# mbhall88/drprg

Hardware: AMD Instinct MI355X
Metric: reads/sec (+ achieved HBM GB/s) predicting on mtb index, 1/2/4/8 GPUs (higher is better)
Workload: dtype u32

## Files before the change

drprg_amd/csrc/candidates.hip:

```cpp
#include "filter_common.h"
#include "verify_lane.h"
#include <algorithm>
#include <cstdint>

namespace drprg {
namespace dev {

constexpr int VS_THREADS = 512;
constexpr int VS_PER = MAX_SLICES / VS_THREADS;
template <int KC, bool PACKED>
__global__ __launch_bounds__(VS_THREADS, 8) void verify_scan_kernel(SketchArgs a, FilterWork fw, ReadClusterArgs rc)
{
    __shared__ uint32_t s_red[3][VS_THREADS / 64];
    __shared__ uint32_t s_w[VS_THREADS / 64 + 1];
    __shared__ uint32_t s_share[2];
    __shared__ __attribute__((aligned(16))) uint32_t s_pre[MAX_SLICES + 4];
    const int tid = threadIdx.x;
    static_assert(VS_PER % 4 == 0 && MAX_SLICES % (VS_THREADS * 4) == 0, "the counts are read 16 bytes at a time");
    auto my_count = [&](int i4) -> uint4 {
        return reinterpret_cast<const uint4*>(fw.super_count + (size_t)tid * VS_PER)[i4];
    };
    uint32_t run = 0;
    uint4 v[VS_PER / 4];
#pragma unroll
    for (int i = 0; i < VS_PER / 4; ++i) v[i] = my_count(i);
#pragma unroll
    for (int i = 0; i < VS_PER / 4; ++i) run += v[i].x + v[i].y + v[i].z + v[i].w;
    uint32_t total;
    const uint32_t before = block_exclusive_scan<VS_THREADS / 64>(run, s_w, &total);
    if (blockIdx.x == 0 && tid == 0) *fw.cand_count = total;
    const uint32_t per_wg = (total + gridDim.x - 1) / gridDim.x;
    const uint64_t b64 = (uint64_t)blockIdx.x * per_wg;
    const uint32_t t_begin = b64 < total ? (uint32_t)b64 : total, t_end = b64 + per_wg < total ? (uint32_t)(b64 + per_wg) : total;
    {
        const uint32_t x0 = t_begin, x1 = t_end - 1u;
        const bool own0 = t_begin < t_end && before <= x0 && x0 < before + run, own1 = t_begin < t_end && before <= x1 && x1 < before + run;
        uint32_t acc = before, n0 = 0, n1 = 0;
        uint4* dst = reinterpret_cast<uint4*>(s_pre + (size_t)tid * VS_PER);
#pragma unroll
        for (int i = 0; i < VS_PER / 4; ++i) {
            uint4 p;
            p.x = acc;
            p.y = p.x + v[i].x;
            p.z = p.y + v[i].y;
            p.w = p.z + v[i].z;
            acc = p.w + v[i].w;
            dst[i] = p;
            n0 += (p.y <= x0 ? 1u : 0u) + (p.z <= x0 ? 1u : 0u) + (p.w <= x0 ? 1u : 0u) + (acc <= x0 ? 1u : 0u);
            n1 += (p.y <= x1 ? 1u : 0u) + (p.z <= x1 ? 1u : 0u) + (p.w <= x1 ? 1u : 0u) + (acc <= x1 ? 1u : 0u);
        }
        if (tid == VS_THREADS - 1) s_pre[MAX_SLICES] = acc;
        if (own0) s_share[0] = (uint32_t)tid * VS_PER + n0;
        if (own1) s_share[1] = (uint32_t)tid * VS_PER + n1;
    }
    __syncthreads();
    const VerifyConsts c(a, fw);
    uint32_t my_hits = 0, my_nmin = 0, my_maxlen = 0;
    auto position_in = [&](uint32_t t, uint32_t lo0, uint32_t hi0, uint32_t step0) -> int64_t {
        uint32_t lo = lo0;
        for (uint32_t step = step0; step >= 1; step >>= 1)
            if (lo + step <= hi0 && s_pre[lo + step] <= t) lo += step;
        static_assert(FT_SUPER == 8, "two uint4 of slice counts per superblock");
        const uint4* __restrict__ c4 = reinterpret_cast<const uint4*>(fw.slice_count) + (size_t)lo * 2;
        const uint4* __restrict__ b4 = reinterpret_cast<const uint4*>(fw.slice_base) + (size_t)lo * 2;
        const uint4 ca = c4[0], cb = c4[1], ba = b4[0], bb = b4[1];
        const uint32_t cnt[7] = { ca.x, ca.y, ca.z, ca.w, cb.x, cb.y, cb.z }, start[8] = { ba.x, ba.y, ba.z, ba.w, bb.x, bb.y, bb.z, bb.w };
        uint32_t rest = t - s_pre[lo], sum = 0, before = 0, at = start[0];
#pragma unroll
        for (int q = 0; q < 7; ++q) {
            sum += cnt[q];
            const bool past = rest >= sum;
            at = past ? start[q + 1] : at;
            before = past ? sum : before;
        }
        return (int64_t)fw.raw_pos[(size_t)at + (rest - before)];
    };
    {
        const uint32_t s_lo = (uint32_t)__builtin_amdgcn_readfirstlane((int)s_share[0]), s_hi = (uint32_t)__builtin_amdgcn_readfirstlane((int)s_share[1]);
        const uint32_t span_step = s_hi > s_lo ? 1u << (31 - __builtin_clz(s_hi - s_lo)) : 1u;
        auto position_of = [&](uint32_t t) -> int64_t { return position_in(t, s_lo, s_hi, span_step); };
        int64_t gp_next = t_begin + tid < t_end ? position_of(t_begin + (uint32_t)tid) : 0;
        for (uint32_t t = t_begin + (uint32_t)tid; t < t_end; t += VS_THREADS) {
            const int64_t gp = gp_next;
            if (t + VS_THREADS < t_end) gp_next = position_of(t + VS_THREADS);
            VerifyOut o;
            verify_one_lane<KC, PACKED>(a, rc, c, gp, o, my_hits, my_nmin, my_maxlen);
            fw.cand_pos1[t] = o.pos1;
            fw.cand_info[t] = ((uint64_t)o.slot << 32) | ((uint64_t)o.strand << 31) | (uint64_t)o.read;
            fw.cand_rec[t] = o.crec;
        }
    }
    const uint32_t wh = wave_inclusive_scan(my_hits), wn = wave_inclusive_scan(my_nmin), wm = wave_max(my_maxlen);
    if ((tid & 63) == 63) {
        s_red[0][tid >> 6] = wh;
        s_red[1][tid >> 6] = wn;
        s_red[2][tid >> 6] = wm;
    }
    __syncthreads();
    if (tid == 0) {
        uint32_t h = 0, n = 0, mx = 0;
        for (int i = 0; i < VS_THREADS / 64; ++i) {
            h += s_red[0][i];
            n += s_red[1][i];
            mx = s_red[2][i] > mx ? s_red[2][i] : mx;
        }
        fw.wg_hits[blockIdx.x] = h;
        fw.wg_nmin[blockIdx.x] = n;
        fw.wg_maxlen[blockIdx.x] = mx;
    }
}



__global__ __launch_bounds__(SCAN_THREADS) void hit_scan_kernel(SketchArgs a, FilterWork fw, int recount, uint32_t n_wg)
{
    __shared__ uint32_t s_w[SCAN_THREADS / 64 + 1];
    __shared__ uint32_t s_n[SCAN_THREADS / 64], s_m[SCAN_THREADS / 64];
    constexpr int PER = MAX_EX_WG / SCAN_THREADS;
    const int tid = threadIdx.x;
    uint32_t v[PER], h[PER], nm[PER], ml[PER], run = 0, nmin = 0, mx = 0;
#pragma unroll
    for (int i = 0; i < PER; ++i) {
        const uint32_t g = (uint32_t)tid * PER + i, gc = g < n_wg ? g : 0u;
        h[i] = fw.wg_hits[gc];
        nm[i] = fw.wg_nmin[gc];
        ml[i] = fw.wg_maxlen[gc];
    }
#pragma unroll
    for (int i = 0; i < PER; ++i) {
        const uint32_t g = (uint32_t)tid * PER + i;
        v[i] = run;
        if (g < n_wg) {
            run += h[i];
            nmin += nm[i];
            mx = ml[i] > mx ? ml[i] : mx;
        }
    }
    uint32_t total;
    const uint32_t before = block_exclusive_scan<SCAN_THREADS / 64>(run, s_w, &total);
#pragma unroll
    for (int i = 0; i < PER; ++i) {
        const uint32_t g = (uint32_t)tid * PER + i;
        if (g < n_wg) fw.wg_base[g] = before + v[i];
    }
    const uint32_t wn = wave_inclusive_scan(nmin), wm = wave_max(mx);
    if ((tid & 63) == 63) {
        s_n[tid >> 6] = wn;
        s_m[tid >> 6] = wm;
    }
    __syncthreads();
    if (tid == 0) {
        uint32_t n = 0, m = 0;
        for (int i = 0; i < SCAN_THREADS / 64; ++i) {
            n += s_n[i];
            m = s_m[i] > m ? s_m[i] : m;
        }
        *a.n_hits = (unsigned long long)total;
        if (n && !recount && !(*reinterpret_cast<volatile uint32_t*>(a.overflow) & 4u)) atomicAdd(a.n_minimizers, (unsigned long long)n);
        *fw.max_len = (unsigned long long)m;
    }
}

__global__ __launch_bounds__(EX_THREADS) void expand_kernel(SketchArgs a, FilterWork fw)
{
    __shared__ uint32_t s_w[EX_THREADS / 64 + 1];
    const int tid = threadIdx.x;
    uint32_t t_begin, t_end;
    candidate_range(fw, blockIdx.x, gridDim.x, t_begin, t_end);
    uint64_t base = fw.wg_base[blockIdx.x];
    for (uint32_t t0 = t_begin; t0 < t_end; t0 += EX_THREADS) {
        const uint32_t t = t0 + tid;
        const uint32_t pos1 = t < t_end ? fw.cand_pos1[t] : 0u;
        uint64_t info = 0;
        uint2 rec = make_uint2(0, 0);
        if (pos1) {
            info = fw.cand_info[t];
            rec = a.slot_rec[(uint32_t)(info >> 32)];
        }
        uint32_t total;
        const uint32_t off = block_exclusive_scan<EX_THREADS / 64>(rec.y, s_w, &total);
        const uint64_t at = base + off;
        if (pos1 && at + rec.y <= a.hit_capacity) {
            const uint32_t read = (uint32_t)info & 0x7FFFFFFFu, strand = ((uint32_t)info >> 31) & 1u;
            for (uint32_t q = 0; q < rec.y; ++q) {
                const uint32_t kn = a.rec_knode[rec.x + q];
                const uint32_t prg = a.rec_prg[rec.x + q];
                const uint32_t rev = ((kn & 1u) == strand) ? 0u : 1u;
                a.hit_key[at + q] = pack_hit_key(read, prg, rev, pos1 - 1);
                a.hit_val[at + q] = kn >> 1;
            }
        }
        base += total;
    }
}

__global__ void read_inversion_kernel(const uint64_t* __restrict__ key, uint32_t n, uint2* __restrict__ list, uint32_t cap,
    unsigned long long* __restrict__ count)
{
    const uint32_t i = blockIdx.x * blockDim.x + threadIdx.x;
    if (i + 1 >= n) return;
    const uint64_t a = key[i], b = key[i + 1];
    const uint32_t read = hit_read(a);
    if (hit_read(b) != read || a <= b) return;
    uint32_t s = i;
    while (s > 0 && hit_read(key[s - 1]) == read) {
        if (key[s - 1] > key[s]) return;
        --s;
    }
    uint32_t e = i + 2;
    while (e < n && hit_read(key[e]) == read) ++e;
    const unsigned long long at = atomicAdd(count, 1ull);
    if (at < cap) list[at] = make_uint2(s, e - s);
}

constexpr int RS_THREADS = 256, RS_MAX = 1024;
__global__ __launch_bounds__(RS_THREADS) void read_fix_kernel(uint64_t* __restrict__ key, uint32_t* __restrict__ val,
    uint64_t* __restrict__ key_tmp, uint32_t* __restrict__ val_tmp, const uint2* __restrict__ list, const unsigned long long* __restrict__ count)
{
    __shared__ uint64_t s_key[RS_MAX];
    __shared__ uint32_t s_val[RS_MAX];
    const uint32_t n_list = (uint32_t)*count;
    for (uint32_t r = blockIdx.x; r < n_list; r += gridDim.x) {
        const uint32_t start = list[r].x, len = list[r].y;
        if (len > RS_MAX) {
            for (uint32_t t0 = 0; t0 < len; t0 += RS_THREADS) {
                const uint32_t t = t0 + threadIdx.x;
                const bool mine = t < len;
                const uint64_t kt = mine ? key[start + t] : 0;
                uint32_t before = 0;
                for (uint32_t j0 = 0; j0 < len; j0 += RS_MAX) {
                    const uint32_t nj = len - j0 < (uint32_t)RS_MAX ? len - j0 : (uint32_t)RS_MAX;
                    __syncthreads();
                    for (uint32_t j = threadIdx.x; j < nj; j += RS_THREADS) s_key[j] = key[start + j0 + j];
                    __syncthreads();
                    if (!mine) continue;
                    if (j0 + nj <= t) {
                        for (uint32_t j = 0; j < nj; ++j) before += s_key[j] <= kt ? 1u : 0u;
                    } else if (j0 > t) {
                        for (uint32_t j = 0; j < nj; ++j) before += s_key[j] < kt ? 1u : 0u;
                    } else {
                        const uint32_t tj = t - j0;
                        for (uint32_t j = 0; j < tj; ++j) before += s_key[j] <= kt ? 1u : 0u;
                        for (uint32_t j = tj + 1; j < nj; ++j) before += s_key[j] < kt ? 1u : 0u;
                    }
                }
                if (mine) {
                    key_tmp[start + before] = kt;
                    val_tmp[start + before] = val[start + t];
                }
            }
            __syncthreads();
            for (uint32_t t = threadIdx.x; t < len; t += RS_THREADS) {
                key[start + t] = key_tmp[start + t];
                val[start + t] = val_tmp[start + t];
            }
            __syncthreads();
            continue;
        }
        for (uint32_t t = threadIdx.x; t < len; t += RS_THREADS) {
            s_key[t] = key[start + t];
            s_val[t] = val[start + t];
        }
        __syncthreads();
        for (uint32_t t = threadIdx.x; t < len; t += RS_THREADS) {
            const uint64_t kt = s_key[t];
            uint32_t before = 0;
            for (uint32_t j = 0; j < t; ++j) before += s_key[j] <= kt ? 1u : 0u;
            for (uint32_t j = t + 1; j < len; ++j) before += s_key[j] < kt ? 1u : 0u;
            key[start + before] = kt;
            val[start + before] = s_val[t];
        }
        __syncthreads();
    }
}

__global__ __launch_bounds__(EX_THREADS) void recount_kernel(SketchArgs a, FilterWork fw)
{
    __shared__ uint32_t s_red[2][EX_THREADS / 64];
    const int tid = threadIdx.x;
    uint32_t t_begin, t_end;
    candidate_range(fw, blockIdx.x, gridDim.x, t_begin, t_end);
    uint32_t my_hits = 0, my_maxlen = 0;
    for (uint32_t t = t_begin + tid; t < t_end; t += EX_THREADS) {
        if (!fw.cand_pos1[t]) continue;
        const uint64_t info = fw.cand_info[t];
        my_hits += a.slot_rec[(uint32_t)(info >> 32)].y;
        const uint32_t read = (uint32_t)info & 0x7FFFFFFFu;
        const uint64_t len64 = a.offsets[read + 1] - a.offsets[read];
        const uint32_t len = len64 > 0xFFFFFFFFull ? 0xFFFFFFFFu : (uint32_t)len64;
        my_maxlen = len > my_maxlen ? len : my_maxlen;
    }
    const uint32_t wh = wave_inclusive_scan(my_hits), wm = wave_max(my_maxlen);
    if ((tid & 63) == 63) {
        s_red[0][tid >> 6] = wh;
        s_red[1][tid >> 6] = wm;
    }
    __syncthreads();
    if (tid == 0) {
        uint32_t h = 0, mx = 0;
        for (int i = 0; i < EX_THREADS / 64; ++i) {
            h += s_red[0][i];
            mx = s_red[1][i] > mx ? s_red[1][i] : mx;
        }
        fw.wg_hits[blockIdx.x] = h;
        fw.wg_nmin[blockIdx.x] = 0;
        fw.wg_maxlen[blockIdx.x] = mx;
    }
}

constexpr int TG_THREADS = 1024, TG_TILES = 64;
__device__ __forceinline__ bool tile_overflow(const SketchArgs& a, const uint32_t* tile_prefix, uint32_t n_tiles, uint64_t dense_capacity)
{
    return (*reinterpret_cast<volatile uint32_t*>(a.overflow) & 4u) != 0 || (uint64_t)tile_prefix[n_tiles] > dense_capacity;
}

__global__ __launch_bounds__(TG_THREADS) void tile_totals_kernel(SketchArgs a, const uint32_t* __restrict__ tile_prefix, uint32_t n_tiles,
    uint64_t dense_capacity, uint32_t* __restrict__ block_first)
{
    __shared__ uint32_t s_w[TG_THREADS / 64 + 1];
    const int tid = threadIdx.x;
    if (tile_overflow(a, tile_prefix, n_tiles, dense_capacity)) {
        if (blockIdx.x == 0 && tid == 0) atomicOr(a.overflow, 4u);
        return;
    }
    uint32_t my_hits = 0, my_nmin = 0;
    for (uint32_t t = blockIdx.x * TG_THREADS + (uint32_t)tid; t < n_tiles; t += gridDim.x * TG_THREADS) {
        my_hits += a.tile_hits[t];
        my_nmin += a.tile_nmin[t];
        if (block_first) {
            const uint32_t lo = tile_prefix[t], hi = tile_prefix[t + 1];
            for (uint32_t m = (lo + 63u) >> 6; lo < hi && (uint64_t)m << 6 < hi; ++m) block_first[m] = t;
        }
    }
    uint32_t hits, nmin;
    (void)block_exclusive_scan<TG_THREADS / 64>(my_hits, s_w, &hits);
    (void)block_exclusive_scan<TG_THREADS / 64>(my_nmin, s_w, &nmin);
    if (tid == 0) {
        if (hits) atomicAdd(a.n_hits, (unsigned long long)hits);
        if (nmin) atomicAdd(a.n_minimizers, (unsigned long long)nmin);
    }
}

__global__ __launch_bounds__(TG_THREADS) void tile_gather_kernel(SketchArgs a, FilterWork fw, const uint32_t* __restrict__ tile_prefix,
    uint32_t n_tiles, uint64_t dense_capacity, uint32_t mark)
{
    const int tid = threadIdx.x, lane = tid & 63, wave = tid >> 6;
    if (tile_overflow(a, tile_prefix, n_tiles, dense_capacity)) return;
    const uint32_t t0 = blockIdx.x * TG_TILES, t1 = t0 + TG_TILES < n_tiles ? t0 + TG_TILES : n_tiles;
    for (uint32_t t = t0 + (uint32_t)wave; t < t1; t += TG_THREADS / 64) {
        const uint32_t n = a.tile_count[t], dst = tile_prefix[t];
        const size_t src = (size_t)t * a.tile_cap;
        for (uint32_t i0 = 0; i0 < n; i0 += 256) {
            uint64_t ci[4];
            uint32_t cp[4];
            uint4 cr[4];
#pragma unroll
            for (int u = 0; u < 4; ++u) {
                const uint32_t i = i0 + 64u * (uint32_t)u + (uint32_t)lane;
                const size_t at = src + (i < n ? i : 0u);
                ci[u] = a.tile_info[at];
                cp[u] = a.tile_pos1[at];
                cr[u] = a.tile_rec[at];
            }
#pragma unroll
            for (int u = 0; u < 4; ++u) {
                const uint32_t i = i0 + 64u * (uint32_t)u + (uint32_t)lane;
                if (i < n) {
                    fw.cand_info[dst + i] = ci[u];
                    fw.cand_pos1[dst + i] = fw.cand_pos1[dst + i] == mark ? 0u : cp[u];
                    fw.cand_rec[dst + i] = cr[u];
                }
            }
        }
    }
}

hipError_t launch_candidate_stage(const SketchArgs& a, FilterWork& fw, const ReadClusterArgs& rc, int n_cus, hipStream_t stream, bool with_totals)
{
    fw.verify_grid = std::min<uint32_t>((uint32_t)n_cus * (uint32_t)(2048 / VS_THREADS), MAX_EX_WG);
    const dim3 grid(fw.verify_grid);
    if (a.packed) {
        if (a.k == 15) hipLaunchKernelGGL((verify_scan_kernel<15, true>), grid, dim3(VS_THREADS), 0, stream, a, fw, rc);
        else hipLaunchKernelGGL((verify_scan_kernel<0, true>), grid, dim3(VS_THREADS), 0, stream, a, fw, rc);
    } else if (a.k == 15) hipLaunchKernelGGL((verify_scan_kernel<15, false>), grid, dim3(VS_THREADS), 0, stream, a, fw, rc);
    else hipLaunchKernelGGL((verify_scan_kernel<0, false>), grid, dim3(VS_THREADS), 0, stream, a, fw, rc);
    if (with_totals) hipLaunchKernelGGL(hit_scan_kernel, dim3(1), dim3(SCAN_THREADS), 0, stream, a, fw, 0, fw.verify_grid);
    return hipGetLastError();
}

bool direct_uses_wave_form(int k, int w, bool wide_hash, bool force_lds) { return !wide_hash && !force_lds && wave_kernel_applies(k, w); }

uint32_t direct_candidate_tiles(uint64_t n_bases, int halo, int k, int w, bool wide_hash, bool force_lds)
{
    return direct_uses_wave_form(k, w, wide_hash, force_lds) ? wave_n_slices(n_bases) : sketch_n_tiles(n_bases, halo);
}

uint32_t direct_first_read_tiles(uint64_t n_bases, int halo, int k, int w, bool wide_hash, bool force_lds)
{
    return direct_uses_wave_form(k, w, wide_hash, force_lds) ? wave_n_tiles(n_bases) : sketch_n_tiles(n_bases, halo);
}

hipError_t launch_direct_candidates(const SketchArgs& a, bool wide_hash, bool force_lds, uint32_t* tile_prefix, void* temp, size_t temp_bytes,
    uint64_t dense_capacity, const ReadClusterArgs& rc, int n_cus, FilterWork& fw, hipStream_t stream, KernelTimer timer, uint32_t slices_mark)
{
    if (a.n_bases == 0 || !a.tile_cap || !slices_mark) return hipErrorInvalidValue;
    const uint32_t n_tiles = direct_candidate_tiles(a.n_bases, a.halo, a.k, a.w, wide_hash, force_lds);
    if (direct_uses_wave_form(a.k, a.w, wide_hash, force_lds)) HIP_TRY(launch_sketch_wave(a, stream, timer));
    else HIP_TRY(launch_sketch_probe(a, wide_hash, stream, timer));
    HIP_TRY(exclusive_scan_u32(temp, temp_bytes, a.tile_count, tile_prefix, n_tiles + 1, stream));
    fw.cand_total = tile_prefix + n_tiles;
    uint32_t* const block_first = dense_capacity ? reinterpret_cast<uint32_t*>(fw.cand_info) : nullptr;
    hipLaunchKernelGGL(tile_totals_kernel, dim3(std::min<uint32_t>((n_tiles + TG_THREADS - 1) / TG_THREADS, (uint32_t)n_cus)), dim3(TG_THREADS), 0, stream, a,
        tile_prefix, n_tiles, dense_capacity, block_first);
    HIP_TRY(hipGetLastError());
    ReadClusterArgs rcs = rc;
    rcs.block_first = block_first;
    rcs.slice_prefix = tile_prefix;
    rcs.n_slices = n_tiles;
    rcs.mark_epoch = slices_mark;
    return launch_read_cluster(a, fw, rcs, n_cus, false, stream);
}

hipError_t launch_tile_gather_marked(const SketchArgs& a, const FilterWork& fw, const uint32_t* tile_prefix, uint32_t n_tiles, uint64_t dense_capacity,
    uint32_t mark, hipStream_t stream)
{
    hipLaunchKernelGGL(tile_gather_kernel, dim3((n_tiles + TG_TILES - 1) / TG_TILES), dim3(TG_THREADS), 0, stream, a, fw, tile_prefix, n_tiles,
        dense_capacity, mark);
    return hipGetLastError();
}

hipError_t launch_filter_recount(const SketchArgs& a, const FilterWork& fw, hipStream_t stream)
{
    hipLaunchKernelGGL(recount_kernel, dim3(fw.ex_grid), dim3(EX_THREADS), 0, stream, a, fw);
    HIP_TRY(hipGetLastError());
    hipLaunchKernelGGL(hit_scan_kernel, dim3(1), dim3(SCAN_THREADS), 0, stream, a, fw, 1, fw.ex_grid);
    return hipGetLastError();
}

hipError_t launch_filter_expand(const SketchArgs& a, const FilterWork& fw, hipStream_t stream)
{
    hipLaunchKernelGGL(expand_kernel, dim3(fw.ex_grid), dim3(EX_THREADS), 0, stream, a, fw);
    return hipGetLastError();
}

hipError_t launch_read_sort(uint64_t* key, uint32_t* val, uint64_t* key_tmp, uint32_t* val_tmp, uint32_t n, uint32_t* scratch, uint64_t scratch_words,
    unsigned long long* count, hipStream_t stream)
{
    if (n < 2) return hipSuccess;
    uint2* list = reinterpret_cast<uint2*>(scratch);
    hipLaunchKernelGGL(read_inversion_kernel, dim3((n + 255) / 256), dim3(256), 0, stream, key, n, list, (uint32_t)(scratch_words / 2), count);
    HIP_TRY(hipGetLastError());
    hipLaunchKernelGGL(read_fix_kernel, dim3(1024), dim3(RS_THREADS), 0, stream, key, val, key_tmp, val_tmp, list, count);
    return hipGetLastError();
}

}
}
```

drprg_amd/csrc/capi.cpp:

```cpp
#include <set>
#include <atomic>
#include <mutex>
#include <thread>
#include <fstream>
#include <cstdio>
#include "../../include/drprg_hip.h"
#include "fastx.h"
#include "genotype.h"
#include "bam.h"
#include "ingest.h"
#include "pgunzip.h"
#include "denovo.h"
#include "mapper.h"
#include "rccl_dyn.h"
#include "pack.h"
#include <algorithm>
#include <cstdlib>
#include <cstring>
#include <fcntl.h>
#include <functional>
#include <sys/mman.h>
#include <sys/stat.h>
#include <unistd.h>
#include <memory>
// ... 1169 lines not shown
    const std::vector<uint32_t> p = find_max_path(kg, std::vector<float>(logp, logp + kg.nodes.size()), thresh, max_kmers_to_average);
    *n_path = p.size();
    for (size_t i = 0; i < p.size() && i < cap; ++i) path[i] = p[i];
    return DRPRG_OK;
}

int drprg_hip_path_base_coverage(const drprg_hip_ctx* ctx, uint32_t prg, const uint32_t* path, uint64_t n_path, const uint32_t* covg2, uint32_t* out,
    uint64_t cap, uint64_t* n_out)
{
    if (!ctx || (n_path && !path) || !covg2 || !n_out || prg >= ctx->index.kgs.size()) return DRPRG_EINVAL;
    const KmerGraph& kg = ctx->index.kgs[prg];
    for (uint64_t i = 0; i < n_path; ++i)
        if (path[i] >= kg.nodes.size()) return DRPRG_EINVAL;
    const std::vector<uint32_t> b = base_coverage_along_path(ctx->index.prgs[prg], kg, std::vector<uint32_t>(path, path + n_path), covg2);
    *n_out = b.size();
    for (size_t i = 0; i < b.size() && i < cap; ++i) out[i] = b[i];
    return DRPRG_OK;
}

int drprg_hip_path_coverage_too_low(const uint32_t* base_covg, uint64_t n, uint32_t global_covg)
{
    if (n && !base_covg) return DRPRG_EINVAL;
    return path_coverage_too_low(std::vector<uint32_t>(base_covg, base_covg + n), global_covg) ? 1 : 0;
}

int drprg_hip_coverage_model(const drprg_hip_ctx* ctx, double out[12])
{
    if (!ctx || !out) return DRPRG_EINVAL;
    const CoverageModel& m = ctx->last_model;
    out[0] = m.exp_depth_covg; out[1] = m.bin ? 1 : 0; out[2] = m.e_rate; out[3] = m.nb_p; out[4] = m.nb_r; out[5] = m.branch;
    out[6] = m.mean; out[7] = m.var; out[8] = m.num_reads; out[9] = m.bin_p; out[10] = m.thresh; out[11] = (double)ctx->last_dropped;
    return DRPRG_OK;
}

int drprg_hip_allele_stats(const uint32_t* fwd, const uint32_t* rev, uint32_t n, uint32_t min_kmer_covg, uint32_t out[6], double* gaps)
{
    if ((n && (!fwd || !rev)) || !out || !gaps) return DRPRG_EINVAL;
    const AlleleStats s = allele_stats(std::vector<uint32_t>(fwd, fwd + n), std::vector<uint32_t>(rev, rev + n), min_kmer_covg);
    out[0] = s.mean_fwd; out[1] = s.mean_rev; out[2] = s.med_fwd; out[3] = s.med_rev; out[4] = s.sum_fwd; out[5] = s.sum_rev;
    *gaps = s.gaps;
    return DRPRG_OK;
}

int drprg_hip_genotype_site(const uint32_t* mean_fwd, const uint32_t* mean_rev, const double* gaps, uint32_t n_alleles, double e,
    double eps, double* likelihood, int32_t* gt, double* gt_conf)
{
    if (!n_alleles || !mean_fwd || !mean_rev || !gaps || !likelihood || !gt || !gt_conf) return DRPRG_EINVAL;
    std::vector<AlleleStats> al(n_alleles);
    for (uint32_t a = 0; a < n_alleles; ++a) {
        al[a].mean_fwd = mean_fwd[a];
        al[a].mean_rev = mean_rev[a];
        al[a].gaps = gaps[a];
    }
    int g = 0;
    genotype_site(al, e, eps, g, *gt_conf);
    *gt = g;
    for (uint32_t a = 0; a < n_alleles; ++a) likelihood[a] = al[a].likelihood;
    return DRPRG_OK;
}

int drprg_hip_genotype_info(const drprg_hip_ctx* ctx, uint32_t out[4])
{
    if (!ctx || !out) return DRPRG_EINVAL;
    std::memcpy(out, ctx->ginfo, sizeof ctx->ginfo);
    return DRPRG_OK;
}

int drprg_hip_filter_selfcheck(const drprg_hip_ctx* ctx, uint64_t out[8])
{
    if (!ctx || !out) return DRPRG_EINVAL;
    ctx->index.filter_selfcheck(out);
    return DRPRG_OK;
}

int drprg_hip_index_sizes(const drprg_hip_ctx* ctx, uint64_t sizes[5])
{
    if (!ctx || !sizes) return DRPRG_EINVAL;
    const FlatIndex& f = ctx->index.flat;
    sizes[0] = f.keys.size();
    sizes[1] = f.rec_prg.size();
    sizes[2] = ctx->index.prgs.size();
    sizes[3] = f.total_knodes();
    sizes[4] = f.slot_key.size();
    return DRPRG_OK;
}

int drprg_hip_index_export(const drprg_hip_ctx* ctx, uint64_t* keys, uint32_t* rec_off, uint32_t* rec_prg, uint32_t* rec_knode,
    uint8_t* rec_strand, uint32_t* prg_min_path_len, uint32_t* prg_knode_base)
{
    if (!ctx) return DRPRG_EINVAL;
    const FlatIndex& f = ctx->index.flat;
    if (keys) std::memcpy(keys, f.keys.data(), f.keys.size() * sizeof(uint64_t));
    if (rec_off) std::memcpy(rec_off, f.rec_off.data(), f.rec_off.size() * sizeof(uint32_t));
    if (rec_prg) std::memcpy(rec_prg, f.rec_prg.data(), f.rec_prg.size() * sizeof(uint32_t));
    if (rec_knode) std::memcpy(rec_knode, f.rec_knode_global.data(), f.rec_knode_global.size() * sizeof(uint32_t));
    if (rec_strand) std::memcpy(rec_strand, f.rec_strand.data(), f.rec_strand.size());
    if (prg_min_path_len) std::memcpy(prg_min_path_len, f.min_path_len.data(), f.min_path_len.size() * sizeof(uint32_t));
    if (prg_knode_base) std::memcpy(prg_knode_base, f.knode_base.data(), f.knode_base.size() * sizeof(uint32_t));
    return DRPRG_OK;
}

int drprg_hip_prg_nodes(const drprg_hip_ctx* ctx, uint32_t prg, uint32_t* starts, uint32_t* ends, uint32_t cap, uint32_t* n_nodes,
    uint32_t* n_sites)
{
    if (!ctx || prg >= ctx->index.prgs.size()) return DRPRG_EINVAL;
    const LocalGraph& g = ctx->index.prgs[prg];
    for (uint32_t i = 0; i < g.nodes.size() && i < cap; ++i) {
        if (starts) starts[i] = g.nodes[i].start;
        if (ends) ends[i] = g.nodes[i].end;
    }
    if (n_nodes) *n_nodes = (uint32_t)g.nodes.size();
    if (n_sites) *n_sites = (uint32_t)g.sites.size();
    return DRPRG_OK;
}

int drprg_hip_device_tables(drprg_hip_ctx* ctx, uint64_t out[6])
{
    API_BEGIN(ctx)
    need_mapper(ctx).device_tables(out);
    API_END(ctx)
}

int drprg_hip_kernel_timing(drprg_hip_ctx* ctx, int enable, int reset, double* ms_total, uint64_t* launches)
{
    API_BEGIN(ctx)
    Mapper& m = need_mapper(ctx);
    m.sync();
    m.enable_kernel_timing(enable != 0);
    if (ms_total) *ms_total = m.sketch_ms_total();
    if (launches) *launches = m.sketch_launches();
    if (reset) m.reset_kernel_timing();
    API_END(ctx)
}

int drprg_hip_filter_schedule(drprg_hip_ctx* ctx, uint64_t out[20])
{
    API_BEGIN(ctx)
    if (!out) throw Error(DRPRG_EINVAL, "null pointer");
    need_mapper(ctx).filter_schedule(out);
    API_END(ctx)
}

int drprg_hip_buffer_info(drprg_hip_ctx* ctx, uint64_t out[6])
{
    API_BEGIN(ctx)
    if (!out) throw Error(DRPRG_EINVAL, "null pointer");
    need_mapper(ctx);
    std::memset(out, 0, 6 * sizeof(uint64_t));
    for (Mapper* m : mappers_of(ctx)) {
        uint64_t v[6];
        m->buffer_info(v);
        for (int i = 0; i < 3; ++i) out[i] += v[i];
        for (int i = 3; i < 5; ++i) out[i] = std::max(out[i], v[i]);
    }
    API_END(ctx)
}

}

#include "report.h"

static int report_guard(char* err, size_t err_len, const std::function<void()>& fn)
{
    auto put = [&](const char* m) {
        if (err && err_len) {
            std::strncpy(err, m, err_len - 1);
            err[err_len - 1] = 0;
        }
    };
    try {
        fn();
    } catch (const Error& e) {
        put(e.what());
        return e.code;
    } catch (const std::exception& e) {
        put(e.what());
        return DRPRG_EIO;
    }
    return DRPRG_OK;
}

extern "C" {

int drprg_hip_annotate(const char* index_dir, const char* pandora_vcf, const char* out_vcf, const drprg_hip_annotate_opts* o,
    char* err, size_t err_len)
{
    if (!index_dir || !pandora_vcf || !out_vcf || !o) return DRPRG_EINVAL;
    return report_guard(err, err_len, [&]() {
        report::AnnotateOpts a;
        a.filter.min_covg = o->min_covg;
        a.filter.max_covg = o->max_covg;
        a.filter.min_strand_bias = o->min_strand_bias;
        a.filter.min_gt_conf = o->min_gt_conf;
        a.filter.min_frs = o->min_frs;
        a.filter.has_max_indel = o->max_indel >= 0;
        a.filter.max_indel = o->max_indel;
        a.minor.maf = o->maf;
        a.minor.max_gaps = o->max_gaps;
        a.minor.max_called_gaps = o->max_called_gaps;
        a.minor.max_gaps_diff = o->max_gaps_diff;
        a.minor.minor_min_covg = o->minor_min_covg;
        a.minor.minor_min_strand_bias = o->minor_min_strand_bias;
        a.ignore_synonymous = o->ignore_synonymous != 0;
        a.id_seed = o->id_seed;
        report::annotate_vcf(report::IndexFiles { index_dir }, pandora_vcf, out_vcf, a);
    });
}

int drprg_hip_report_json(const char* index_dir, const char* annotated_vcf, const char* out_json, const char* sample, int padding,
    const char* index_version, char* err, size_t err_len)
{
    if (!index_dir || !annotated_vcf || !out_json) return DRPRG_EINVAL;
    return report_guard(err, err_len, [&]() {
        report::IndexFiles idx { index_dir };
        std::string version = index_version ? index_version : "";
        if (padding < 0 || !index_version) {
            report::IndexConfig c = report::read_config(idx.config());
            if (padding < 0) padding = c.padding;
            if (!index_version) version = c.version;
        }
        report::vcf_to_json(idx, annotated_vcf, out_json, sample ? sample : "sample", padding, version);
    });
}

}

extern "C" int drprg_hip_vcf_to_bcf(const char* vcf_path, const char* bcf_path, char* err, size_t err_len)
{
    if (!vcf_path || !bcf_path) return DRPRG_EINVAL;
    return report_guard(err, err_len, [&]() { report::vcf_to_bcf(vcf_path, bcf_path); });
}

extern "C" int drprg_hip_gunzip_file(const char* gz_path, int threads, uint64_t chunk_bytes, const char* out_path, uint64_t out[3], char* err, size_t err_len)
{
    if (!gz_path || !out_path || !out) return DRPRG_EINVAL;
    return report_guard(err, err_len, [&]() {
        const int fd = open(gz_path, O_RDONLY);
        if (fd < 0) throw Error(DRPRG_ENOENT, std::string("cannot open ") + gz_path);
        struct stat sb;
        void* map = fstat(fd, &sb) == 0 && sb.st_size > 0 ? mmap(nullptr, (size_t)sb.st_size, PROT_READ, MAP_PRIVATE, fd, 0) : MAP_FAILED;
        close(fd);
        if (map == MAP_FAILED) throw Error(DRPRG_EIO, std::string("cannot map ") + gz_path);
        struct Unmap {
            void* p;
            size_t n;
            ~Unmap() { munmap(p, n); }
        } unmap { map, (size_t)sb.st_size };
        FILE* o = std::fopen(out_path, "wb");
        if (!o) throw Error(DRPRG_EIO, std::string("cannot write ") + out_path);
        struct Close {
            FILE* f;
            ~Close() { std::fclose(f); }
        } close_o { o };
        ParallelGunzip pg((const unsigned char*)map, (size_t)sb.st_size, threads, (size_t)chunk_bytes);
        std::vector<char> buf(size_t(8) << 20);
        uint64_t total = 0;
        for (size_t n; (n = pg.read(buf.data(), buf.size())) > 0; total += n)
            if (std::fwrite(buf.data(), 1, n, o) != n) throw Error(DRPRG_EIO, std::string("cannot write ") + out_path);
        out[0] = total;
        out[1] = pg.chunks_accepted();
        out[2] = pg.chunks_redone();
    });
}

extern "C" int drprg_hip_parse_fastx_ordered(const char* reads_path, int threads, uint64_t max_reads, uint64_t out[6], char* err, size_t err_len)
{
    if (!reads_path || !out) return DRPRG_EINVAL;
    return report_guard(err, err_len, [&]() {
        uint64_t sum = 0, n_reads = 0, n_bases = 0, batches = 0;
        IngestHooks hooks;
        hooks.submit_in_order = [&](const PinnedBatch& b) -> bool {
            const uint64_t n = std::min<uint64_t>(b.n_reads, max_reads - n_reads);
            for (uint64_t i = 0; i < n; ++i) {
                uint64_t h = 1469598103934665603ull;
                for (uint64_t j = b.offsets[i]; j < b.offsets[i + 1]; ++j) h = (h ^ b.bases[j]) * 1099511628211ull;
                sum += (n_reads + i + 1) * h;
            }
            n_reads += n;
            n_bases += b.offsets[n];
            ++batches;
            return n_reads < max_reads;
        };
        const IngestStats st = ingest_fastx(reads_path, threads, hooks);
        out[0] = n_reads; out[1] = n_bases; out[2] = sum; out[3] = batches; out[4] = (uint64_t)st.gz_mode; out[5] = st.discarded_reads;
    });
}

extern "C" int drprg_hip_parse_fastx(const char* reads_path, int threads, uint64_t out[5], char* err, size_t err_len)
{
    if (!reads_path || !out) return DRPRG_EINVAL;
    return report_guard(err, err_len, [&]() {
        uint64_t sum = 0, n_reads = 0, n_bases = 0, batches = 0;
        const bool no_digest = std::getenv("DRPRG_PARSE_NO_DIGEST") != nullptr;
        auto digest = [&](const uint8_t* bases, const uint64_t* offsets, uint64_t n) {
            for (uint64_t i = 0; i < n && !no_digest; ++i) {
                uint64_t h = 1469598103934665603ull;
                for (uint64_t j = offsets[i]; j < offsets[i + 1]; ++j) h = (h ^ bases[j]) * 1099511628211ull;
                sum += h;
            }
            n_reads += n;
            n_bases += offsets[n];
            ++batches;
        };
        const char* fmt = std::getenv("DRPRG_PARSE_FORMAT");
        const bool packed = fmt && std::string(fmt) == "packed", normalized = fmt && std::string(fmt) == "normalized";
        std::vector<uint8_t> tmp;
// ... 37 lines not shown
```

drprg_amd/csrc/device_common.h:

```cpp
#pragma once
#include "kernels.h"
#include <hip/hip_runtime.h>
#include <hip/hip_ext.h>

namespace drprg {
namespace dev {

#define HIP_TRY(x)                                                                                   \
    do {                                                                                             \
        hipError_t e_ = (x);                                                                         \
        if (e_ != hipSuccess) return e_;                                                             \
    } while (0)

constexpr int MAX_HIP_DEVICES = 64;
inline hipError_t ensure_dynamic_lds(const void* kernel, size_t bytes, size_t (&cache)[MAX_HIP_DEVICES])
{
    int dev = 0;
    hipError_t e = hipGetDevice(&dev);
    if (e != hipSuccess) return e;
    if (dev >= 0 && dev < MAX_HIP_DEVICES && bytes <= cache[dev]) return hipSuccess;
    e = hipFuncSetAttribute(kernel, hipFuncAttributeMaxDynamicSharedMemorySize, (int)bytes);
    if (e == hipSuccess && dev >= 0 && dev < MAX_HIP_DEVICES) cache[dev] = bytes;
    return e;
}
// ... 57 lines not shown
    static constexpr uint64_t EMPTY = ~0ULL;
    __device__ static inline uint64_t mix(uint64_t key, uint64_t mask)
    {
        key = (~key + (key << 21)) & mask;
        key = key ^ (key >> 24);
        key = (key + (key << 3) + (key << 8)) & mask;
        key = key ^ (key >> 14);
        key = (key + (key << 2) + (key << 4)) & mask;
        key = key ^ (key >> 28);
        key = (key + (key << 31)) & mask;
        return key;
    }
};

__device__ inline uint32_t table_slot_dev(uint32_t key, uint32_t bits) { return (key * 0x9E3779B1u) >> (32 - bits); }
__device__ inline uint32_t table_slot_dev(uint64_t key, uint32_t bits)
{
    return (uint32_t)((key * 0x9E3779B97F4A7C15ULL) >> (64 - bits));
}

__device__ __forceinline__ bool table_find4(const uint32_t* __restrict__ slot_key, uint32_t tmask, uint32_t h, uint32_t& sl)
{
    constexpr uint32_t EMPTY = HashTraits<uint32_t>::EMPTY;
    uint32_t base = sl & ~3u, from = 0xFu << (sl & 3u);
    while (true) {
        const uint4 q = *reinterpret_cast<const uint4*>(slot_key + base);
        const uint32_t hit = (q.x == h ? 1u : 0u) | (q.y == h ? 2u : 0u) | (q.z == h ? 4u : 0u) | (q.w == h ? 8u : 0u);
        const uint32_t end = hit | (q.x == EMPTY ? 1u : 0u) | (q.y == EMPTY ? 2u : 0u) | (q.z == EMPTY ? 4u : 0u) | (q.w == EMPTY ? 8u : 0u);
        const uint32_t m = end & from;
        if (m) {
            const uint32_t i = (uint32_t)__builtin_ctz(m);
            sl = base + i;
            return (hit >> i) & 1u;
        }
        base = (base + 4u) & tmask;
        from = 0xFu;
    }
}

__device__ inline uint32_t encode_base(uint32_t c)
{
    uint32_t u = c & 0xDFu;
    uint32_t x = (u >> 1) & 3u;
    x ^= x >> 1;
    bool ok = (u == 'A') | (u == 'C') | (u == 'G') | (u == 'T');
    return ok ? x : 4u;
}
__device__ inline uint32_t encode4(uint32_t word)
{
    const uint32_t u = word & 0xDFDFDFDFu;
    const uint32_t sel = (u >> 1) & 0x03030303u;
    const uint32_t code = __builtin_amdgcn_perm(0u, 0x02030100u, sel);
    const uint32_t expect = __builtin_amdgcn_perm(0u, 0x47544341u, sel);
    const uint32_t diff = u ^ expect;
    const uint32_t bad = (((diff & 0x7F7F7F7Fu) + 0x7F7F7F7Fu) | diff) & 0x80808080u;
    return code | (bad >> 5);
}

__device__ inline uint32_t find_read_from(const uint64_t* __restrict__ offsets, uint32_t n_reads, uint32_t lo, uint64_t gp)
{
    uint32_t step = 1, hi = lo + 1;
    while (hi < n_reads && offsets[hi] <= gp) {
        lo = hi;
        step <<= 1;
        hi = (n_reads - lo > step) ? lo + step : n_reads;
    }
    while (hi - lo > 1) {
        uint32_t mid = lo + ((hi - lo) >> 1);
        if (offsets[mid] <= gp) lo = mid; else hi = mid;
    }
    return lo;
}

__device__ inline uint32_t find_read_guess(const uint64_t* __restrict__ offsets, uint32_t n_reads, uint32_t guess, uint32_t lo, uint64_t gp)
{
    if (guess >= n_reads) guess = n_reads - 1;
    if (offsets[guess] <= gp && gp < offsets[guess + 1]) return guess;
    return find_read_from(offsets, n_reads, lo, gp);
}

__device__ inline uint32_t find_read_near(const uint64_t* __restrict__ offsets, uint32_t n_reads, uint32_t guess, uint64_t gp)
{
    uint32_t lo = guess < n_reads ? guess : n_reads - 1, hi;
    if (offsets[lo] <= gp) {
        uint32_t step = 1;
        hi = lo + 1;
        while (hi < n_reads && offsets[hi] <= gp) {
            lo = hi;
            step <<= 1;
            hi = (n_reads - lo > step) ? lo + step : n_reads;
        }
    } else {
        uint32_t step = 1;
        hi = lo;
        while (true) {
            lo = hi > step ? hi - step : 0;
            if (offsets[lo] <= gp) break;
            hi = lo;
            step <<= 1;
        }
    }
    while (hi - lo > 1) {
        uint32_t mid = lo + ((hi - lo) >> 1);
        if (offsets[mid] <= gp) lo = mid; else hi = mid;
    }
    return lo;
}

__device__ inline uint32_t w1_reciprocal(int w) { return (uint32_t)(0x100000000ull / (uint32_t)(w + 1)) + 1u; }
__device__ inline uint64_t expected_minimizers(uint64_t len, int w, uint32_t magic)
{
    if (w < 200 && len < (1ull << 23)) return (uint64_t)__umulhi((uint32_t)len * 2u, magic);
    return len * 2 / (uint64_t)(w + 1);
}

__device__ inline uint32_t wave_inclusive_scan(uint32_t v)
{
    const int lane = threadIdx.x & 63;
#pragma unroll
    for (int off = 1; off < 64; off <<= 1) {
        const uint32_t n = __shfl_up(v, off);
        if (lane >= off) v += n;
    }
    return v;
}
__device__ inline uint32_t wave_max(uint32_t v)
{
#pragma unroll
    for (int off = 32; off > 0; off >>= 1) {
        const uint32_t n = __shfl_xor(v, off);
        v = n > v ? n : v;
    }
    return v;
}

template <int NW> __device__ inline uint32_t block_exclusive_scan(uint32_t v, uint32_t* s_w, uint32_t* total)
{
    const int lane = threadIdx.x & 63, wave = threadIdx.x >> 6;
    const uint32_t incl = wave_inclusive_scan(v);
    __syncthreads();
    if (lane == 63) s_w[wave] = incl;
    __syncthreads();
    uint32_t base = 0, sum = 0;
#pragma unroll
    for (int i = 0; i < NW; ++i) {
        const uint32_t x = s_w[i];
        if (i < wave) base += x;
        sum += x;
    }
    *total = sum;
    return base + incl - v;
}

}
}
```

drprg_amd/csrc/filter_common.h:

```cpp
#pragma once
#include "common.h"
#include "device_common.h"

namespace drprg {
namespace dev {

constexpr int FT_THREADS = 1024;
constexpr int FT_WAVES = FT_THREADS / 64;
constexpr int FT_G = 32;
constexpr int FT_WPOS = 63 * FT_G;
DRPRG_HD constexpr int filter_positions_per_lane(bool level0, bool packed) { return level0 && packed ? 64 : 32; }
constexpr int FT_BLOOM_WORDS = 1 << 14;
constexpr int FT_L0_WORDS = 1 << 15;
constexpr int EX_THREADS = 256;
constexpr int SCAN_THREADS = 1024;
constexpr int MAX_SLICES = SCAN_THREADS * 8;
constexpr int FT_DEPTH = 3;
constexpr int FT_SUPER = 8;
constexpr int MAX_CHUNKS = MAX_SLICES * FT_SUPER;
constexpr int MAX_EX_WG = SCAN_THREADS * 4;

__device__ inline void candidate_range(const FilterWork& fw, uint32_t wg, uint32_t n_wg, uint32_t& t_begin, uint32_t& t_end)
{
    const uint32_t total = *fw.cand_total;
    const uint32_t per_wg = (total + n_wg - 1) / n_wg;
    const uint64_t b = (uint64_t)wg * per_wg;
    t_begin = b < total ? (uint32_t)b : total;
    t_end = b + per_wg < total ? (uint32_t)(b + per_wg) : total;
}

hipError_t launch_candidate_stage(const SketchArgs& a, FilterWork& fw, const ReadClusterArgs& rc, int n_cus, hipStream_t stream, bool with_totals = true);
hipError_t launch_read_cluster(const SketchArgs& a, const FilterWork& fw, const ReadClusterArgs& rc, int n_cus, bool skip, hipStream_t stream);

}
}
```

drprg_amd/csrc/kernels.h:

```cpp
#pragma once
#include <cstddef>
#include <cstdint>
#include <hip/hip_runtime_api.h>
#include "switches.h"

#if defined(__HIPCC__)
#define DRPRG_HD __host__ __device__
#else
#define DRPRG_HD
#endif

namespace drprg {
namespace dev {

constexpr int HIT_POS_BITS = 23;
constexpr int HIT_PRG_BITS = 12;
constexpr int HIT_READ_BITS = 28;
constexpr uint64_t HIT_POS_MASK = (1ull << HIT_POS_BITS) - 1;
constexpr uint32_t MAX_BATCH_READS = 1u << HIT_READ_BITS;
constexpr uint32_t MAX_PRGS = 1u << HIT_PRG_BITS;

DRPRG_HD inline uint64_t pack_hit_key(uint32_t read, uint32_t prg, uint32_t rev, uint32_t pos)
{
    return ((uint64_t)read << (HIT_PRG_BITS + 1 + HIT_POS_BITS)) | ((uint64_t)prg << (1 + HIT_POS_BITS))
        | ((uint64_t)rev << HIT_POS_BITS) | (uint64_t)pos;
}
DRPRG_HD inline uint32_t hit_read(uint64_t k) { return (uint32_t)(k >> (HIT_PRG_BITS + 1 + HIT_POS_BITS)); }
DRPRG_HD inline uint32_t hit_prg(uint64_t k) { return (uint32_t)(k >> (1 + HIT_POS_BITS)) & (MAX_PRGS - 1); }
DRPRG_HD inline uint32_t hit_rev(uint64_t k) { return (uint32_t)(k >> HIT_POS_BITS) & 1u; }

DRPRG_HD inline uint32_t pbloom_mix(uint64_t key) { return ((uint32_t)key ^ (uint32_t)(key >> 32)) * 0x9E3779B1u; }
DRPRG_HD inline uint32_t pbloom_word(uint32_t m, uint32_t wbits) { return m >> (32 - wbits); }
DRPRG_HD inline uint32_t pbloom_bits(uint32_t m) { return (1u << (m & 31)) | (1u << ((m >> 5) & 31)); }

struct SketchArgs {
    const uint8_t* bases;
    const uint64_t* offsets;
    uint64_t n_bases;
    uint32_t n_reads;
    int w, k, halo;
    int packed;
    const uint64_t* npos;
    uint64_t n_npos;
    const uint16_t* nbits;
    const void* slot_key;
    const uint2* slot_rec;
    const uint4* slot_first;
    uint32_t table_bits;
    const uint32_t* rec_knode;
    const uint16_t* rec_prg;
    uint32_t* tile_first_read;
    uint64_t* hit_key;
    uint32_t* hit_val;
    uint64_t hit_capacity;
    unsigned long long* n_hits;
    unsigned long long* n_minimizers;
    const uint32_t* pbloom;
    uint32_t pbloom_wbits;
    uint32_t* overflow;
    uint32_t tile_cap;
    uint64_t* tile_info;
    uint32_t* tile_pos1;
    uint4* tile_rec;
    uint32_t *tile_count, *tile_hits, *tile_nmin;
    const uint32_t* prg_min_path_len;
    const uint32_t* prg_thr;
    double fraction;
    uint32_t min_cluster_size;
};

struct ClusterRec {
    uint32_t read, prg_rev, first_pos, last_pos, n, state;
};

struct ClusterArgs {
    const uint64_t* key;
    const uint32_t* val;
    const uint32_t* scan;
    const uint32_t* cstart;
    const uint32_t* d_n_clusters;
    const uint64_t* offsets;
    const uint32_t* prg_min_path_len;
    ClusterRec* clusters;
    uint32_t* order;
    int w;
    double fraction;
    uint32_t min_cluster_size;
    uint32_t* covg;
    uint32_t* prg_reads;
    unsigned long long* n_clusters_kept;
    unsigned long long* n_hits_kept;
};

struct KernelTimer {
    hipEvent_t begin = nullptr, end = nullptr;
};

uint32_t sketch_tile_eval(int halo);
uint32_t sketch_n_tiles(uint64_t n_bases, int halo);
hipError_t launch_sketch_probe(const SketchArgs& a, bool wide_hash, hipStream_t stream, KernelTimer timer = {});
bool probe_compile_time_window(int k, int w);
hipError_t launch_tile_first_read(const uint64_t* offsets, uint32_t n_reads, int t_eval, int halo, uint32_t n_tiles, uint32_t* out,
    hipStream_t stream);
bool wave_kernel_applies(int k, int w);
uint32_t wave_tile_eval();
uint32_t wave_n_tiles(uint64_t n_bases);
uint32_t wave_n_slices(uint64_t n_bases);
hipError_t launch_sketch_wave(const SketchArgs& a, hipStream_t stream, KernelTimer timer = {});
uint32_t direct_candidate_tiles(uint64_t n_bases, int halo, int k, int w, bool wide_hash, bool force_lds);
bool direct_uses_wave_form(int k, int w, bool wide_hash, bool force_lds);
uint32_t direct_first_read_tiles(uint64_t n_bases, int halo, int k, int w, bool wide_hash, bool force_lds);
uint32_t filter_n_tiles(uint64_t n_bases, int positions_per_lane = 32);
uint32_t filter_grid(bool level0, int n_cus, uint32_t n_tiles, uint32_t cap);
struct BloomTables {
    const uint32_t* bloom;
    uint32_t bloom_wbits;
    const uint32_t* bloom0;
    uint32_t bloom0_wbits;
    const uint32_t* bloomr;
    const uint32_t* bloom0f;
    const uint32_t* mid0 = nullptr;
    const uint32_t* mid_bitmap = nullptr;
    const uint32_t* midc = nullptr;
    uint32_t midc_wbits = 0, mid0_bits = 0;
    const uint32_t* blkc = nullptr;
    uint32_t blkc_wbits = 0;
};
struct FilterBuffers {
    uint64_t* raw_pos;
    uint64_t* cand_info;
    uint32_t* cand_pos1;
    uint4* cand_rec;
    uint64_t raw_capacity;
    uint32_t* small;
    unsigned long long* max_len;
    const uint32_t* wave_share = nullptr;
    unsigned long long* class_clock = nullptr;
};
constexpr int FT_MAX_ROUNDS = 8;
struct FilterSched {
    uint32_t tpw0;
    uint32_t per_wg;
    uint32_t n_tiles;
    uint32_t first_ticket[FT_MAX_ROUNDS], first_tile[FT_MAX_ROUNDS], size[FT_MAX_ROUNDS];
    uint32_t n_rounds;
    uint32_t lds_word;
};
FilterSched make_filter_sched(uint32_t n_tiles, uint32_t n_wg, const uint32_t share[4], const FilterSchedKnobs& knobs);
const uint32_t* filter_builtin_shares(bool mid, bool packed);
struct FilterWork {
    const uint32_t* bloom;
    uint32_t bloom_wbits;
    const uint32_t* bloom0;
    uint32_t bloom0_wbits;
    const uint32_t* mid_bitmap;
    const uint32_t* midc;
    uint32_t midc_wbits;
    uint32_t read_begin, read_end;
    uint32_t n_slices;
    uint32_t slice_budget, slice_cpt, slice_slack;
    uint32_t slice_extra, slice_extra_from;
    uint64_t* raw_pos;
    uint32_t* slice_count;
    uint32_t* slice_base;
    uint32_t* slice_cap;
    uint32_t* super_count;
    FilterSched sched;
    uint32_t* cand_count;
    const uint32_t* cand_total;
    uint64_t* cand_info;
    uint32_t* cand_pos1;
    uint4* cand_rec;
    uint32_t ex_grid;
    uint32_t verify_grid;
    uint32_t *wg_hits, *wg_nmin, *wg_maxlen, *wg_base;
    unsigned long long* max_len;
    unsigned long long* class_clock;
    uint32_t wave_share[4];
};
constexpr uint32_t READ_NONE = 0x7FFFFFFFu;

struct ReadClusterArgs {
    const uint32_t* prg_min_path_len;
    double fraction;
    uint32_t min_cluster_size;
    int max_diff;
    uint32_t n_prgs;
    uint32_t* covg;
    uint32_t* prg_reads;
    unsigned long long* n_clusters_kept;
    unsigned long long* n_hits_kept;
    unsigned long long* n_complex;
    uint32_t* chunk_counter;
    const uint32_t* slice_prefix;
    uint32_t n_slices, mark_epoch;
    const uint32_t* block_first;
    const uint32_t *wg_hits, *wg_nmin, *wg_maxlen;
    uint32_t n_wg;
    unsigned long long *tot_hits, *tot_minimizers, *tot_max_len;
    const uint32_t* overflow_word;
    uint32_t minpath_in_lds;
};
hipError_t launch_counters_home(unsigned long long* from, unsigned long long* to, uint32_t n, hipStream_t stream, uint32_t* zero = nullptr, uint32_t n_zero = 0);
uint32_t* filter_super_counts(uint32_t* small);
uint32_t filter_super_words();
size_t filter_small_words();
void init_candidate_work(FilterWork& fw, const FilterBuffers& b, int n_cus);
hipError_t launch_sketch_filter(const SketchArgs& a, const BloomTables& bt, int n_cus, const FilterBuffers& b, const ReadClusterArgs& rc, FilterWork& fw,
    const Switches& sw, hipStream_t stream, KernelTimer timer = {});
hipError_t launch_filter_recount(const SketchArgs& a, const FilterWork& fw, hipStream_t stream);
hipError_t launch_filter_expand(const SketchArgs& a, const FilterWork& fw, hipStream_t stream);
hipError_t launch_direct_candidates(const SketchArgs& a, bool wide_hash, bool force_lds, uint32_t* tile_prefix, void* temp, size_t temp_bytes,
    uint64_t dense_capacity, const ReadClusterArgs& rc, int n_cus, FilterWork& fw, hipStream_t stream, KernelTimer timer, uint32_t slices_mark);
hipError_t launch_tile_gather_marked(const SketchArgs& a, const FilterWork& fw, const uint32_t* tile_prefix, uint32_t n_tiles, uint64_t dense_capacity,
    uint32_t mark, hipStream_t stream);
hipError_t exclusive_scan_u32(void* temp, size_t temp_bytes, const uint32_t* in, uint32_t* out, uint32_t n, hipStream_t stream);
hipError_t launch_read_sort(uint64_t* key, uint32_t* val, uint64_t* key_tmp, uint32_t* val_tmp, uint32_t n, uint32_t* scratch, uint64_t scratch_words,
    unsigned long long* count, hipStream_t stream);
size_t sort_temp_bytes(uint32_t n);
size_t scan_temp_bytes(uint32_t n);
hipError_t sort_hits(void* temp, size_t temp_bytes, const uint64_t* key_in, uint64_t* key_out, const uint32_t* val_in,
    uint32_t* val_out, uint32_t n, hipStream_t stream);
hipError_t launch_cluster_flags(const uint64_t* key, uint32_t n, int max_diff, uint32_t* head, uint32_t* scan, void* temp,
    size_t temp_bytes, hipStream_t stream);
hipError_t launch_cluster_starts(const uint32_t* head, const uint32_t* scan, uint32_t n, uint32_t* cstart, hipStream_t stream);
hipError_t launch_cluster_pipeline(const ClusterArgs& a, uint32_t n_hits, uint32_t n_prgs, hipStream_t stream);
hipError_t launch_vector_add_u32(uint32_t* dst, const uint32_t* src, uint64_t n, hipStream_t stream);
hipError_t launch_unpack(const uint32_t* words, uint64_t n_bases, const uint64_t* npos, uint64_t n_npos, uint8_t* out, hipStream_t stream);
hipError_t launch_mark_npos(const uint64_t* npos, uint64_t n_npos, uint64_t n_bases, uint16_t* bits, hipStream_t stream);
hipError_t launch_pack(const uint8_t* bases, uint64_t n_bases, uint32_t* words, uint64_t* npos, uint64_t npos_cap, unsigned long long* n_npos,
    hipStream_t stream);

uint32_t bam_pack_chunks(uint64_t n_bases);
hipError_t launch_bam_pack(const uint8_t* seq, const uint64_t* seq_start, const uint64_t* offsets, const uint8_t* reverse, uint64_t n_reads, uint64_t n_bases,
    uint32_t* words, uint64_t* npos, uint64_t npos_cap, bool list, uint32_t* chunk_count, uint32_t* chunk_prefix, void* temp, size_t temp_bytes, hipStream_t stream);

hipError_t launch_covg_cut(const uint64_t* offsets, uint64_t n_reads, uint64_t target, const uint64_t* npos, uint64_t n_npos, unsigned long long* out,
    hipStream_t stream);

struct SelectedRead {
    uint64_t offset;
    uint32_t len, read, batch, pad;
};
hipError_t launch_anchor_scan(const uint8_t* bases, const uint64_t* offsets, uint32_t n_reads, uint64_t n_bases, const uint64_t* anchors,
    uint32_t n_anchors, uint32_t A, const uint32_t* prefilter, uint32_t batch, uint32_t* flags, unsigned long long* count, SelectedRead* list,
    uint64_t list_cap, int n_cus, hipStream_t stream);
struct GatherEntry {
    const uint8_t* src;
    uint64_t dst;
    uint32_t len, pad;
};
hipError_t launch_gather_reads(const GatherEntry* table, uint32_t n, uint8_t* out, hipStream_t stream);

}
}
```

drprg_amd/csrc/mapper.cpp:

```cpp
#include "mapper.h"
#include <algorithm>
#include <cmath>
#include <atomic>
#include <cstdio>
#include <cstdlib>
#include <cstring>
#include <mutex>
#include <set>
#include <hip/hip_runtime.h>
#include <sys/mman.h>

namespace drprg {

enum { C_HITS = 0, C_MINIMIZERS = 1, C_CLUSTERS_KEPT = 2, C_HITS_KEPT = 3, C_OVERFLOW = 4, C_MAXLEN = 5, C_UNSORTED = 6, C_COMPLEX = 7, C_N = 8 };
constexpr uint64_t READ_SORT_MAX_LEN = 512;
constexpr uint64_t FILTER_BASES_PER_ENTRY = 48;

void Mapper::IndexTables::fill(const FlatIndex& idx, bool wide_hash, uint64_t mid_max_records)
{
    const size_t nslot = idx.slot_key.size(), nrec = idx.rec_prg.size();
    if (idx.min_path_len.size() > dev::MAX_PRGS) throw Error(DRPRG_EOVERFLOW, "more than " + std::to_string(dev::MAX_PRGS) + " PRGs");
    for (size_t i = 0; i < nslot; ++i)
        if (idx.slot_cnt[i] && idx.min_path_len[idx.rec_prg[idx.slot_off[i]]] >= (1u << 20))
            throw Error(DRPRG_EOVERFLOW, "a PRG's shortest k-mer path has 2^20 nodes or more");
// ... 152 lines not shown
            (void)hipHostFree(p);
            return;
        }
    }
    (void)hipHostUnregister(p);
    std::free(p);
}

void Mapper::warm_device(int device)
{
    if (hipSetDevice(device) == hipSuccess) (void)hipFree(nullptr);
}

void Mapper::set_params(const MapParams& p)
{
    sync();
    PrgIndex::check_wk(p.w, p.k);
    const bool filter_ok = (tables_.bloom_wbits != 0 || tables_.midc_wbits != 0) && p.k <= 15 && p.w <= 16;
    if (p.kernel_mode < 0 || p.kernel_mode > 3) throw Error(DRPRG_EINVAL, "kernel must be 0 (auto), 1, 2 or 3");
    if (p.kernel_mode == 2 && !filter_ok)
        throw Error(DRPRG_EINVAL, "the Bloom-prefiltered kernel needs k <= 15, w <= 16 and an index small enough for its filter tiers");
    params_ = p;
    wide_hash_ = p.k > 15;
    halo_ = std::max(16, ((p.w - 1 + 15) / 16) * 16);
    {
        std::vector<uint32_t> thr(n_prgs_);
        const double fraction = params_.cluster_fraction();
        for (uint32_t i = 0; i < n_prgs_; ++i) thr[i] = (uint32_t)((double)tables_.h_min_path_len[i] * fraction);
        HIPCHK(hipSetDevice(device_));
        HIPCHK(hipMemcpy(tables_.prg_thr.data(), thr.data(), n_prgs_ * sizeof(uint32_t), hipMemcpyHostToDevice));
        HIPCHK(hipStreamSynchronize(nullptr));
    }
    use_filter_ = p.kernel_mode == 2 || (p.kernel_mode == 0 && filter_ok);
    use_mid_ = use_filter_ && tables_.bloom_wbits == 0;
    use_direct_cands_ = p.kernel_mode == 3 || (p.kernel_mode == 0 && !filter_ok);
}

void Mapper::reset_coverage(bool new_sample)
{
    sync();
    HIPCHK(hipSetDevice(device_));
    HIPCHK(hipMemsetAsync(d_covg_.data(), 0, d_covg_.bytes(), stream_));
    HIPCHK(hipMemsetAsync(d_counters_.data(), 0, d_counters_.bytes(), stream_));
    HIPCHK(hipStreamSynchronize(stream_));
    tot_reads_ = tot_bases_ = tot_hits_ = tot_leftover_ = tot_minimizers_ = 0;
    bam_blocks_ = 0;
    for (auto& sh : ft_share_)
        for (uint32_t& v : sh) v = 0;
    sw_ = read_switches();
    if (new_sample) drop_kept();
}

void Mapper::ensure_workspace(uint64_t cap)
{
    if (cap <= hit_capacity()) return;
    if (cap >= (1ull << 31)) throw Error(DRPRG_EOVERFLOW, "more than 2^31 minimizer hits in one batch; map smaller batches");
    d_key_a_.alloc(cap); d_key_b_.alloc(cap); d_val_a_.alloc(cap); d_val_b_.alloc(cap);
    d_head_.alloc(cap); d_scan_.alloc(cap); d_cstart_.alloc(cap + 1); d_order_.alloc(cap);
    d_clusters_.alloc(cap);
    d_temp_.alloc(std::max(dev::sort_temp_bytes((uint32_t)cap), dev::scan_temp_bytes((uint32_t)cap)));
}

void Mapper::grow_lane(Lane& lane, uint64_t cap)
{
    if (cap <= lane.capacity()) return;
    if (cap >= (1ull << 31)) throw Error(DRPRG_EOVERFLOW, "more than 2^31 candidate k-mers in one batch; map smaller batches");
    lane.raw_pos.alloc(cap); lane.cand_info.alloc(cap); lane.cand_pos1.alloc(cap); lane.cand_rec.alloc(cap);
    zero_now(lane.cand_pos1.data(), lane.cand_pos1.bytes());
}

void Mapper::ensure_lanes()
{
    for (Lane& lane : lanes_) {
        if (lane.h_scratch) continue;
        lane.done.create(false);
        lane.t0.create(true);
        lane.t1.create(true);
        lane.small.alloc(dev::filter_small_words());
        zero_now(lane.small.data(), lane.small.bytes());
        lane.d_scratch.alloc(L_N);
        zero_now(lane.d_scratch.data(), lane.d_scratch.bytes());
        lane.scratch_zero = true;
        lane.h_scratch.alloc(L_N);
    }
}

Mapper::Batch Mapper::make_batch(int lane, const DeviceBatch& batch, uint32_t* covg, uint32_t* prg_reads, hipStream_t stream) const
{
    Batch b;
    b.batch = batch;
    b.active = true;
    b.direct = !use_filter_;
    b.lane = lane;
    b.covg = covg;
    b.prg_reads = prg_reads;
    b.stream = stream;
    return b;
}

void Mapper::launch(const Batch& b)
{
    ensure_lanes();
    if (b.direct) direct_launch(b);
    else filter_launch(b);
    HIPCHK(hipEventRecord(lanes_[b.lane].done, b.stream));
}

void Mapper::count_on_lane(dev::SketchArgs& a, const Lane& lane) const
{
    a.n_hits = lane.d_scratch.data() + L_HITS;
    a.n_minimizers = lane.d_scratch.data() + L_MINIMIZERS;
    a.overflow = reinterpret_cast<uint32_t*>(lane.d_scratch.data() + L_OVERFLOW);
}

dev::FilterBuffers Mapper::filter_buffers(const Lane& lane) const
{
    return dev::FilterBuffers { lane.raw_pos.data(), lane.cand_info.data(), lane.cand_pos1.data(), lane.cand_rec.data(), lane.capacity(), lane.small.data(),
        lane.d_scratch.data() + L_MAXLEN };
}

dev::ReadClusterArgs Mapper::read_cluster_args(const Batch& b) const
{
    const Lane& lane = lanes_[b.lane];
    dev::ReadClusterArgs rc {};
    rc.prg_min_path_len = tables_.min_path_len.data();
    rc.fraction = params_.cluster_fraction();
    rc.min_cluster_size = params_.min_cluster_size;
    rc.max_diff = params_.max_diff;
    rc.n_prgs = n_prgs_;
    rc.covg = b.covg;
    rc.prg_reads = b.prg_reads;
    rc.n_clusters_kept = d_counters_.data() + C_CLUSTERS_KEPT;
    rc.n_hits_kept = d_counters_.data() + C_HITS_KEPT;
    rc.n_complex = lane.d_scratch.data() + L_COMPLEX;
    rc.chunk_counter = reinterpret_cast<uint32_t*>(lane.d_scratch.data() + L_CHUNK);
    return rc;
}

dev::KernelTimer Mapper::kernel_timer(hipEvent_t t0, hipEvent_t t1) const
{
    dev::KernelTimer timer;
    if (timing_) {
        timer.begin = t0;
        timer.end = t1;
    }
    return timer;
}

void Mapper::filter_launch(const Batch& b)
{
    Lane& lane = lanes_[b.lane];
    grow_lane(lane, std::max<uint64_t>(min_capacity_, b.batch.n_bases / FILTER_BASES_PER_ENTRY));
    if (!lane.scratch_zero) HIPCHK(hipMemsetAsync(lane.d_scratch.data(), 0, lane.d_scratch.bytes(), b.stream));
    lane.scratch_zero = false;
    dev::SketchArgs a = sketch_args(b.batch, nullptr);
    count_on_lane(a, lane);
    dev::FilterBuffers fb = filter_buffers(lane);
    fb.class_clock = lane.d_scratch.data() + L_FT_CLOCK;
    if (ft_share_[b.batch.packed ? 1 : 0][0]) fb.wave_share = ft_share_[b.batch.packed ? 1 : 0];
    HIPCHK(dev::launch_sketch_filter(a, tables_.bloom_tables(use_mid_), n_cus_, fb, read_cluster_args(b), lane.fw, sw_, b.stream, kernel_timer(lane.t0, lane.t1)));
    HIPCHK(dev::launch_counters_home(lane.d_scratch.data(), lane.h_scratch.device_ptr(), L_N, b.stream, dev::filter_super_counts(lane.small.data()), dev::filter_super_words()));
    lane.scratch_zero = true;
}

static void wait_stream(hipStream_t stream, hipEvent_t event = nullptr)
{
    for (int spins = 0; spins < 2048; ++spins) {
        const hipError_t e = event ? hipEventQuery(event) : hipStreamQuery(stream);
        if (e == hipSuccess) return;
        if (e != hipErrorNotReady) HIPCHK(e);
    }
    HIPCHK(event ? hipEventSynchronize(event) : hipStreamSynchronize(stream));
}

void Mapper::cluster_hits(const uint64_t* d_offsets, uint32_t n_hits, bool ordered, unsigned long long* d_unsorted, uint32_t* covg,
    uint32_t* prg_reads, hipStream_t stream)
{
    if (n_hits == 0) return;
    const uint64_t* s_key = d_key_b_.data();
    const uint32_t* s_val = d_val_b_.data();
    if (ordered) {
        HIPCHK(dev::launch_read_sort(d_key_a_.data(), d_val_a_.data(), d_key_b_.data(), d_val_b_.data(), n_hits, d_order_.data(), hit_capacity(), d_unsorted, stream));
        s_key = d_key_a_.data();
        s_val = d_val_a_.data();
    } else HIPCHK(dev::sort_hits(d_temp_.data(), d_temp_.size(), d_key_a_.data(), d_key_b_.data(), d_val_a_.data(), d_val_b_.data(), n_hits, stream));
    HIPCHK(dev::launch_cluster_flags(s_key, n_hits, params_.max_diff, d_head_.data(), d_scan_.data(), d_temp_.data(), d_temp_.size(), stream));
    HIPCHK(dev::launch_cluster_starts(d_head_.data(), d_scan_.data(), n_hits, d_cstart_.data(), stream));
    dev::ClusterArgs c {};
    c.key = s_key;
    c.val = s_val;
    c.scan = d_scan_.data();
    c.cstart = d_cstart_.data();
    c.d_n_clusters = d_scan_.data() + (n_hits - 1);
    c.offsets = d_offsets;
    c.prg_min_path_len = tables_.min_path_len.data();
    c.clusters = d_clusters_.data();
    c.order = d_order_.data();
    c.w = params_.w;
    c.fraction = params_.cluster_fraction();
    c.min_cluster_size = params_.min_cluster_size;
    c.covg = covg;
    c.prg_reads = prg_reads;
    c.n_clusters_kept = d_counters_.data() + C_CLUSTERS_KEPT;
    c.n_hits_kept = d_counters_.data() + C_HITS_KEPT;
    HIPCHK(dev::launch_cluster_pipeline(c, n_hits, n_prgs_, stream));
}

dev::SketchArgs Mapper::sketch_args(const DeviceBatch& batch, const TileSet* tiles) const
{
    dev::SketchArgs a {};
    a.bases = batch.d_bases;
    a.offsets = batch.d_offsets;
    a.n_bases = batch.n_bases;
    a.n_reads = (uint32_t)batch.n_reads;
    a.w = params_.w;
    a.k = params_.k;
    a.halo = halo_;
    a.slot_key = tables_.slot_key.data();
    a.slot_rec = tables_.slot_rec.data();
    a.slot_first = tables_.slot_first.data();
    a.table_bits = tables_.table_bits;
    a.rec_knode = tables_.rec_knode.data();
    a.rec_prg = tables_.rec_prg.data();
    a.tile_first_read = tiles ? tiles->d_tile_first.data() : nullptr;
    a.pbloom = tables_.pbloom.data();
    a.pbloom_wbits = tables_.pbloom_wbits;
    a.hit_key = d_key_a_.data();
    a.hit_val = d_val_a_.data();
    a.hit_capacity = hit_capacity();
    a.n_hits = d_counters_.data() + C_HITS;
    a.n_minimizers = d_counters_.data() + C_MINIMIZERS;
    a.overflow = reinterpret_cast<uint32_t*>(d_counters_.data() + C_OVERFLOW);
    a.packed = batch.packed ? 1 : 0;
    a.npos = batch.d_npos;
    a.n_npos = batch.n_npos;
    return a;
}

Mapper::DeviceBatch Mapper::ascii_view(int slot, const DeviceBatch& batch, hipStream_t stream)
{
    if (!batch.packed) return batch;
    const uint64_t need = (batch.n_bases + 15) / 16 * 16 + 64;
    if (need > d_unpacked_[slot].size()) {
        sync();
        HIPCHK(hipStreamSynchronize(stream));
        d_unpacked_[slot].alloc(need + need / 4);
    }
    HIPCHK(dev::launch_unpack(reinterpret_cast<const uint32_t*>(batch.d_bases), batch.n_bases, batch.d_npos, batch.n_npos, d_unpacked_[slot].data(), stream));
    DeviceBatch ascii;
    ascii.d_bases = d_unpacked_[slot].data();
    ascii.d_offsets = batch.d_offsets;
    ascii.n_reads = batch.n_reads;
    ascii.n_bases = batch.n_bases;
    return ascii;
}

void Mapper::read_counters(hipStream_t stream)
{
    HIPCHK(hipMemcpyAsync(h_counters_.data(), d_counters_.data(), d_counters_.bytes(), hipMemcpyDeviceToHost, stream));
    wait_stream(stream);
}

void Mapper::note_kernel_time(hipEvent_t t0, hipEvent_t t1)
{
    if (!timing_) return;
    float ms = 0;
    HIPCHK(hipEventElapsedTime(&ms, t0, t1));
    sketch_ms_ += ms;
    sketch_launches_ += 1;
}

void Mapper::leftovers(const Batch& b)
{
    Lane& lane = lanes_[b.lane];
    if (lane.h_scratch[L_COMPLEX] == 0) return;
    const hipStream_t stream = b.stream;
    dev::SketchArgs a = sketch_args(b.batch, b.direct ? &tsets_[b.lane] : nullptr);
    count_on_lane(a, lane);
    lane.scratch_zero = false;
    HIPCHK(dev::launch_filter_recount(a, lane.fw, stream));
    HIPCHK(hipMemcpyAsync(lane.h_scratch.data(), lane.d_scratch.data(), lane.d_scratch.bytes(), hipMemcpyDeviceToHost, stream));
    wait_stream(stream);
    const uint64_t n_left = lane.h_scratch[L_HITS];
    if (n_left == 0) return;
    ensure_workspace(std::max<uint64_t>(min_capacity_, n_left + n_left / 8));
    a.hit_key = d_key_a_.data();
    a.hit_val = d_val_a_.data();
    a.hit_capacity = hit_capacity();
    HIPCHK(dev::launch_filter_expand(a, lane.fw, stream));
    cluster_hits(b.batch.d_offsets, (uint32_t)n_left, lane.h_scratch[L_MAXLEN] <= READ_SORT_MAX_LEN, lane.d_scratch.data() + L_UNSORTED, b.covg, b.prg_reads, stream);
}

void Mapper::ensure_tile_workspace(TileSet& t, uint32_t n_tiles, uint32_t tile_cap)
{
    if (n_tiles <= t.ws_tiles && tile_cap <= t.ws_cap) return;
    const uint32_t ws_tiles = std::max(t.ws_tiles, n_tiles + n_tiles / 8 + 32), ws_cap = std::max(t.ws_cap, tile_cap);
    const size_t n = (size_t)ws_tiles * ws_cap, per_tile = (size_t)ws_tiles + 1;
    t.d_tile_info.alloc(n); t.d_tile_pos1.alloc(n); t.d_tile_rec.alloc(n);
    t.d_tile_count.alloc(per_tile); t.d_tile_hits.alloc(per_tile); t.d_tile_nmin.alloc(per_tile); t.d_tile_prefix.alloc(per_tile);
    t.d_tile_temp.alloc(dev::scan_temp_bytes(ws_tiles + 1));
    t.ws_tiles = ws_tiles;
    t.ws_cap = ws_cap;
}

void Mapper::reserve_tile_first(TileSet& t, uint32_t n_tiles)
{
    t.d_tile_first.reserve(n_tiles, n_tiles + n_tiles / 4 + 16);
}

void Mapper::direct_launch(const Batch& b)
{
    const int set = b.lane;
    const uint64_t n_bases = b.batch.n_bases;
    const hipStream_t stream = b.stream;
    TileSet& t = tsets_[set];
    const uint32_t n_tiles = dev::direct_candidate_tiles(n_bases, halo_, params_.k, params_.w, wide_hash_, sw_.direct_lds);
    reserve_tile_first(t, dev::direct_first_read_tiles(n_bases, halo_, params_.k, params_.w, wide_hash_, sw_.direct_lds));
    Lane& lane = lanes_[set];
    grow_lane(lane, std::min<uint64_t>(std::max<uint64_t>(min_capacity_, n_bases / 16), (1ull << 31) - 1));
    static std::atomic<uint32_t> process_epoch { 0x80000000u };
    slices_epoch_ = process_epoch.fetch_add(1) + 1;
    if (slices_epoch_ < 0x80000000u) {
        HIPCHK(hipMemsetAsync(lane.cand_pos1.data(), 0, lane.cand_pos1.bytes(), stream));
        process_epoch.store(0x80000001u);
        slices_epoch_ = 0x80000001u;
    }
    const uint32_t mark = slices_epoch_;
    ensure_tile_workspace(t, n_tiles, t.slice_cap);
    if (!lane.scratch_zero) HIPCHK(hipMemsetAsync(lane.d_scratch.data(), 0, lane.d_scratch.bytes(), stream));
    lane.scratch_zero = false;
    HIPCHK(hipMemsetAsync(t.d_tile_count.data() + n_tiles, 0, sizeof(uint32_t), stream));
    const bool native_packed = b.batch.packed && dev::direct_uses_wave_form(params_.k, params_.w, wide_hash_, sw_.direct_lds);
    dev::SketchArgs a = sketch_args(native_packed ? b.batch : ascii_view(set, b.batch, stream), &t);
    if (native_packed && a.n_npos) {
        const uint64_t words16 = ((n_bases + 15) / 16 + 1) & ~1ull;
        const uint64_t grown = words16 + words16 / 4;
        if (t.d_nbits.reserve(words16, grown + (grown & 1))) t.nbits_dirty = true;
        if (t.nbits_dirty) HIPCHK(hipMemsetAsync(t.d_nbits.data(), 0, t.d_nbits.bytes(), stream));
        HIPCHK(dev::launch_mark_npos(a.npos, a.n_npos, n_bases, t.d_nbits.data(), stream));
        t.nbits_dirty = true;
        a.nbits = t.d_nbits.data();
    }
    count_on_lane(a, lane);
    a.tile_cap = t.ws_cap;
    a.tile_info = t.d_tile_info.data();
    a.tile_pos1 = t.d_tile_pos1.data();
    a.tile_rec = t.d_tile_rec.data();
    a.tile_count = t.d_tile_count.data();
    a.tile_hits = t.d_tile_hits.data();
    a.tile_nmin = t.d_tile_nmin.data();
    a.prg_min_path_len = tables_.min_path_len.data();
    a.prg_thr = tables_.prg_thr.data();
    a.fraction = params_.cluster_fraction();
    a.min_cluster_size = params_.min_cluster_size;
    lane.fw = dev::FilterWork {};
    lane.fw.read_begin = 0;
    lane.fw.read_end = (uint32_t)b.batch.n_reads;
    dev::init_candidate_work(lane.fw, filter_buffers(lane), n_cus_);
    HIPCHK(dev::launch_direct_candidates(a, wide_hash_, sw_.direct_lds, t.d_tile_prefix.data(), t.d_tile_temp.data(), t.d_tile_temp.size(), lane.capacity(),
        read_cluster_args(b), n_cus_, lane.fw, stream, kernel_timer(lane.t0, lane.t1), mark));
    t.a_done = a;
    t.mark = mark;
    t.n_tiles = n_tiles;
    HIPCHK(hipMemcpyAsync(lane.h_scratch.data(), lane.d_scratch.data(), lane.d_scratch.bytes(), hipMemcpyDeviceToHost, stream));
    HIPCHK(hipMemsetAsync(lane.d_scratch.data(), 0, lane.d_scratch.bytes(), stream));
    lane.scratch_zero = true;
}

bool Mapper::direct_finish(const Batch& b, int attempt)
{
    TileSet& t = tsets_[b.lane];
    Lane& lane = lanes_[b.lane];
    const uint32_t ovf = (uint32_t)lane.h_scratch[L_OVERFLOW];
    if (ovf & 2u) throw Error(DRPRG_EOVERFLOW, "a read is longer than 2^" + std::to_string(dev::HIT_POS_BITS) + " bases");
    if (ovf & 4u) {
        if (attempt > 6) throw Error(DRPRG_EOVERFLOW, "candidate buffer overflow after regrow");
        HIPCHK(hipStreamSynchronize(b.stream));
        ++reruns_direct_;
        t.slice_cap = std::min<uint32_t>(t.slice_cap * 2, 4096);
        grow_lane(lane, std::min<uint64_t>(lane.capacity() * 2, (1ull << 31) - 1));
        return false;
    }
    tot_minimizers_ += lane.h_scratch[L_MINIMIZERS];
    tot_hits_ += lane.h_scratch[L_HITS];
    tot_leftover_ += lane.h_scratch[L_COMPLEX];
    if (lane.h_scratch[L_COMPLEX])
        HIPCHK(dev::launch_tile_gather_marked(t.a_done, lane.fw, t.d_tile_prefix.data(), t.n_tiles, lane.capacity(), t.mark, b.stream));
    leftovers(b);
    return true;
}

bool Mapper::filter_finish(const Batch& b, int attempt)
{
    Lane& lane = lanes_[b.lane];
    const uint32_t ovf = (uint32_t)lane.h_scratch[L_OVERFLOW];
    if (ovf & 8u) throw Error(DRPRG_EIO, "sketch_filter_kernel: dynamic LDS does not start at address 0");
    if (ovf & 16u) throw Error(DRPRG_EIO, "sketch_filter_kernel: a chunk of its schedule holds too few whole tiles");
    if (ovf & 32u) throw Error(DRPRG_EINVAL, "the batch's read offsets do not span its bases: offsets[0] must be 0 and offsets[n_reads] must be n_bases");
    if (ovf & 2u) throw Error(DRPRG_EOVERFLOW, "a read is longer than 2^" + std::to_string(dev::HIT_POS_BITS) + " bases");
    if (ovf & 4u) {
        if (attempt > 8) throw Error(DRPRG_EOVERFLOW, "candidate buffer overflow after regrow");
        grow_lane(lane, lane.capacity() * 4);
        ++reruns_filter_;
        return false;
    }
    tot_minimizers_ += lane.h_scratch[L_MINIMIZERS];
    tot_hits_ += lane.h_scratch[L_HITS];
    tot_leftover_ += lane.h_scratch[L_COMPLEX];
    tune_filter_shares(lane, b.batch.packed, b.batch.n_bases);
    leftovers(b);
    return true;
}

void Mapper::filter_schedule(uint64_t out[20])
{
    sync();
    for (int i = 0; i < 20; ++i) out[i] = ft_last_[i];
}

void Mapper::buffer_info(uint64_t out[6])
{
    sync();
    uint64_t raw = 0;
    for (const Lane& lane : lanes_) raw = std::max(raw, lane.capacity());
    out[0] = reruns_filter_;
    out[1] = reruns_direct_;
    out[2] = regrows_hits_;
    out[3] = raw;
    out[4] = hit_capacity();
    out[5] = sketch_form();
}

int Mapper::sketch_form() const
{
    if (use_filter_) return use_mid_ ? 12 : (tables_.bloom0_wbits ? 10 : 11);
    if (use_direct_cands_ && dev::direct_uses_wave_form(params_.k, params_.w, wide_hash_, sw_.direct_lds)) return 1;
    return wide_hash_ ? 4 : (dev::probe_compile_time_window(params_.k, params_.w) ? 2 : 3);
}

void Mapper::tune_filter_shares(const Lane& lane, bool packed, uint64_t n_bases)
{
    {
        const dev::FilterSched& sc = lane.fw.sched;
        const unsigned long long* ck = &lane.h_scratch[L_FT_CLOCK];
        ft_last_[0] = sc.n_rounds;
        ft_last_[1] = lane.fw.n_slices;
        ft_last_[2] = sc.tpw0;
        for (int c = 0; c < 4; ++c) {
            ft_last_[3 + c] = lane.fw.wave_share[c];
            ft_last_[7 + c] = ck[0] && ck[1 + c] > ~ck[0] ? ck[1 + c] - ~ck[0] : 0;
        }
        ft_last_[11] = sc.per_wg;
        for (int r = 0; r < dev::FT_MAX_ROUNDS; ++r) ft_last_[12 + r] = r && r < (int)sc.n_rounds ? sc.size[r] : 0;
    }
    if (lane.fw.sched.n_rounds > 1) return;
    if (n_bases < (64ull << 20)) return;
    const unsigned long long* ck = &lane.h_scratch[L_FT_CLOCK];
    if (!ck[0] || !ck[1] || !ck[2] || !ck[3] || !ck[4]) return;
    const unsigned long long t0 = ~ck[0];
    double end[4], mean = 0;
    for (int c = 0; c < 4; ++c) {
        if (ck[1 + c] <= t0) return;
        end[c] = (double)(ck[1 + c] - t0);
        mean += end[c] / 4;
    }
    uint32_t* s = ft_share_[packed ? 1 : 0];
    if (!s[0]) {
        const uint32_t* from = dev::filter_builtin_shares(use_mid_, packed);
        for (int c = 0; c < 4; ++c) s[c] = from[c];
    }
    double v[4], sum = 0;
    for (int c = 0; c < 4; ++c) {
        v[c] = (double)s[c] * std::pow(mean / end[c], 0.6);
        v[c] = std::min(std::max(v[c], 0.35 * 256), 2.2 * 256);
        sum += v[c];
    }
    uint32_t acc = 0;
    for (int c = 0; c < 3; ++c) acc += s[c] = (uint32_t)(1024.0 * v[c] / sum + 0.5);
    s[3] = 1024u - acc;
}

void Mapper::check(const DeviceBatch& b)
{
    if (b.n_npos && !b.d_npos) throw Error(DRPRG_EINVAL, "n_npos > 0 without the positions");
    if (b.n_reads == 0) return;
    if (!b.d_bases || !b.d_offsets) throw Error(DRPRG_EINVAL, "null device pointer");
    if ((reinterpret_cast<uintptr_t>(b.d_bases) & 15u) != 0)
        throw Error(DRPRG_EINVAL, std::string(b.packed ? "d_words" : "d_bases") + " must be 16-byte aligned");
    if (b.n_reads > dev::MAX_BATCH_READS) throw Error(DRPRG_EOVERFLOW, "at most " + std::to_string(dev::MAX_BATCH_READS) + " reads per batch");
}

void Mapper::map(const DeviceBatch& batch, uint32_t* covg, uint32_t* prg_reads, hipStream_t stream, bool deferred)
{
    check(batch);
    if (batch.n_reads == 0) return;
    HIPCHK(hipSetDevice(device_));
    if (kept_cap_ && !in_keep_call_) kept_broken_ = true;
    if (!covg) covg = d_covg();
    if (!prg_reads) prg_reads = d_prg_reads();
    if (!stream) stream = stream_;
    if (!deferred || (!use_filter_ && !use_direct_cands_) || batch.n_bases == 0) {
        complete_pending();
        run_batch(batch, covg, prg_reads, stream);
        tot_reads_ += batch.n_reads;
        tot_bases_ += batch.n_bases;
        if (deferred) wait_stream(stream);
        return;
    }
    const Batch cur = make_batch(pipe_next_, batch, covg, prg_reads, stream);
    launch(cur);
    const Batch prev = pending_;
    pending_ = cur;
    pipe_next_ ^= 1;
    tot_reads_ += batch.n_reads;
    tot_bases_ += batch.n_bases;
    if (prev.active) complete_batch(prev);
}

void Mapper::complete_pending()
{
    if (!pending_.active) return;
    const Batch b = pending_;
    pending_.active = false;
    complete_batch(b);
}

void Mapper::complete_batch(const Batch& b)
{
    HIPCHK(hipSetDevice(device_));
    const Lane& lane = lanes_[b.lane];
    const uint64_t leftover_before = tot_leftover_;
    for (int attempt = 0;; ++attempt) {
        if (attempt) launch(b);
        wait_stream(b.stream, lane.done);
        if (attempt == 0) note_kernel_time(lane.t0, lane.t1);
        if (b.direct ? direct_finish(b, attempt) : filter_finish(b, attempt)) {
            if (attempt || tot_leftover_ != leftover_before) wait_stream(b.stream);
            return;
        }
    }
}

void Mapper::sync()
{
    const hipStream_t last = pending_.active ? pending_.stream : nullptr;
    complete_pending();
    if (last) HIPCHK(hipStreamSynchronize(last));
}

void Mapper::run_batch(const DeviceBatch& batch, uint32_t* covg, uint32_t* prg_reads, hipStream_t stream)
{
    const uint64_t n_bases = batch.n_bases;
    if (n_bases == 0) return;
    if (use_filter_ || use_direct_cands_) {
        const Batch b = make_batch(0, batch, covg, prg_reads, stream);
        launch(b);
        complete_batch(b);
        return;
    }
    ensure_workspace(std::max<uint64_t>(min_capacity_, n_bases / 64));
    reserve_tile_first(tsets_[0], dev::sketch_n_tiles(n_bases, halo_));
// ... 457 lines not shown
```

drprg_amd/csrc/mapper.h:

```cpp
#pragma once
#include "device_mem.h"
#include "index.h"
#include "kernels.h"
#include <vector>

namespace drprg {

struct MapCounters {
    uint64_t reads = 0, bases = 0, minimizers = 0, hits = 0, clusters_kept = 0, hits_kept = 0;
    uint64_t kernel = 0;
    uint64_t leftover_reads = 0;
};

class Mapper {
public:
    Mapper(const FlatIndex& idx, const MapParams& p, int device);
    ~Mapper();
    Mapper(const Mapper&) = delete;
    Mapper& operator=(const Mapper&) = delete;

    int device() const { return device_; }
    uint32_t n_knodes() const { return n_knodes_; }
    uint32_t n_prgs() const { return n_prgs_; }
    hipStream_t stream() const { return stream_; }
    void set_params(const MapParams& p);

    struct DeviceBatch {
        const uint8_t* d_bases = nullptr;
        const uint64_t* d_offsets = nullptr;
        uint64_t n_reads = 0, n_bases = 0;
        bool packed = false;
        const uint64_t* d_npos = nullptr;
        uint64_t n_npos = 0;
    };
    void map(const DeviceBatch& b, uint32_t* d_covg, uint32_t* d_prg_reads, hipStream_t stream, bool deferred);
    void sync();
    static void check(const DeviceBatch& b);

    struct CutPoint {
        uint64_t n_reads, n_bases, n_npos;
    };
    CutPoint find_cut(const DeviceBatch& b, uint64_t target, hipStream_t stream);

    uint64_t pack_on_device(const uint8_t* d_bases, uint64_t n_bases, uint32_t* d_words, uint64_t* d_npos, uint64_t npos_cap, hipStream_t stream);
    uint64_t pack_bam_on_device(const uint8_t* d_seq, const uint64_t* d_seq_start, const uint64_t* d_offsets, const uint8_t* d_reverse, uint64_t n_reads,
        uint64_t n_bases, uint32_t* d_words, uint64_t* d_npos, uint64_t npos_cap, hipStream_t stream);
    struct HostBatch {
        const uint8_t* bases = nullptr;
        const uint64_t* offsets = nullptr;
        uint64_t n_reads = 0;
        bool packed = false;
        const uint64_t* npos = nullptr;
        uint64_t n_npos = 0;
        bool bam = false;
        const uint64_t* seq_start = nullptr;
        const uint8_t* reverse = nullptr;
        uint64_t seq_bytes = 0;
        uint64_t n_bases() const { return offsets[n_reads]; }
        uint64_t payload_bytes() const { return packed || bam ? ((n_bases() + 15) / 16) * 4 : n_bases(); }
    };
    uint64_t bam_blocks() const { return bam_blocks_; }
    void map_host(const HostBatch& b);
    void map_host_async(const HostBatch& b);
    void keep_reads(uint64_t max_bytes);
    bool kept_complete() const { return kept_cap_ > 0 && !kept_broken_; }
    const std::vector<DeviceBatch>& kept() const { return kept_; }
    uint64_t kept_bytes() const { return kept_bytes_; }
    void drop_kept();
    static constexpr uint64_t SELECT_WINDOW_BYTES = 1ull << 30;
    void select_reads_with_anchors(std::vector<uint64_t> anchors, uint32_t A, std::vector<uint8_t>& bases, std::vector<uint64_t>& offsets,
        std::vector<uint64_t>* ids = nullptr, uint64_t window_bytes = 0);
    uint64_t map_kept_from(const Mapper& other);

    void add_vectors_from(Mapper& other);

    static void* pinned_alloc(size_t bytes);
    static void pinned_free(void* p);
    static void warm_device(int device);

    void reset_coverage(bool new_sample = true);
    uint32_t* d_covg() const { return d_covg_.data(); }
    uint32_t* d_prg_reads() const { return d_covg_.data() + 2 * (size_t)n_knodes_; }
    void download(std::vector<uint32_t>& covg, std::vector<uint32_t>& prg_reads);
    void upload(const std::vector<uint32_t>& covg, const std::vector<uint32_t>& prg_reads);
    MapCounters counters();
    void device_tables(uint64_t out[6]) const;

    bool pending_writes_to(const uint32_t* covg, const uint32_t* prg_reads) const
    {
        return pending_.active && ((covg && pending_.covg == covg) || (prg_reads && pending_.prg_reads == prg_reads));
    }
    void filter_schedule(uint64_t out[20]);
    void buffer_info(uint64_t out[6]);
    void enable_kernel_timing(bool on) { timing_ = on; }
    double sketch_ms_total() const { return sketch_ms_; }
    uint64_t sketch_launches() const { return sketch_launches_; }
    void reset_kernel_timing() { sketch_ms_ = 0; sketch_launches_ = 0; }

private:
    Stream stream_, copy_stream_;
    void zero_now(void* p, size_t bytes);
    void ensure_workspace(uint64_t hit_capacity);
    struct Lane {
        Event done, t0, t1;
        DeviceBuffer<uint64_t> raw_pos, cand_info;
        DeviceBuffer<uint4> cand_rec;
        DeviceBuffer<uint32_t> cand_pos1, small;
        DeviceBuffer<unsigned long long> d_scratch;
        PinnedBuffer<unsigned long long> h_scratch;
        bool scratch_zero = false;
        dev::FilterWork fw {};
        uint64_t capacity() const { return raw_pos.size(); }
    };
    enum { L_HITS = 0, L_OVERFLOW = 1, L_MAXLEN = 2, L_UNSORTED = 3, L_COMPLEX = 4, L_CHUNK = 5, L_MINIMIZERS = 6, L_FT_CLOCK = 7 , L_N = 12 };
    struct Batch {
        DeviceBatch batch;
        bool active = false;
        bool direct = false;
        int lane = 0;
        uint32_t *covg = nullptr, *prg_reads = nullptr;
        hipStream_t stream = nullptr;
    };
    Batch make_batch(int lane, const DeviceBatch& batch, uint32_t* covg, uint32_t* prg_reads, hipStream_t stream) const;
    void ensure_lanes();
    void grow_lane(Lane& lane, uint64_t capacity);
    void launch(const Batch& b);
    void filter_launch(const Batch& b);
    bool filter_finish(const Batch& b, int attempt);
    void direct_launch(const Batch& b);
    bool direct_finish(const Batch& b, int attempt);
    void leftovers(const Batch& b);
    void run_batch(const DeviceBatch& batch, uint32_t* d_covg, uint32_t* d_prg_reads, hipStream_t stream);
    void cluster_hits(const uint64_t* d_offsets, uint32_t n_hits, bool ordered, unsigned long long* d_unsorted, uint32_t* d_covg,
        uint32_t* d_prg_reads, hipStream_t stream);
    void count_on_lane(dev::SketchArgs& a, const Lane& lane) const;
    dev::FilterBuffers filter_buffers(const Lane& lane) const;
    dev::ReadClusterArgs read_cluster_args(const Batch& b) const;
    dev::KernelTimer kernel_timer(hipEvent_t t0, hipEvent_t t1) const;
    DeviceBatch ascii_view(int slot, const DeviceBatch& batch, hipStream_t stream);
    DeviceBuffer<uint8_t> d_unpacked_[3];
    DeviceBuffer<unsigned long long> d_pack_count_;
    PinnedBuffer<unsigned long long> h_cut_;
    void read_counters(hipStream_t stream);
    void note_kernel_time(hipEvent_t t0, hipEvent_t t1);
    void complete_pending();
    void complete_batch(const Batch& b);
    Batch pending_;
    int pipe_next_ = 0;

    int device_ = 0;
    Switches sw_ = read_switches();
    MapParams params_;
    bool wide_hash_ = false;
    int halo_ = 16;
    uint32_t n_knodes_ = 0, n_prgs_ = 0;
    struct IndexTables {
        uint32_t table_bits = 0;
        DeviceBuffer<unsigned char> slot_key;
        DeviceBuffer<uint2> slot_rec;
        DeviceBuffer<uint4> slot_first;
        DeviceBuffer<uint32_t> rec_knode;
        DeviceBuffer<uint16_t> rec_prg;
        DeviceBuffer<uint32_t> min_path_len;
        DeviceBuffer<uint32_t> prg_thr;
        std::vector<uint32_t> h_min_path_len;
        DeviceBuffer<uint32_t> bloom;
        uint32_t bloom_wbits = 0;
        DeviceBuffer<uint32_t> pbloom;
        uint32_t pbloom_wbits = 0;
        DeviceBuffer<uint32_t> bloom0;
        DeviceBuffer<uint32_t> bloom0f;
        uint32_t bloom0_wbits = 0;
        DeviceBuffer<uint32_t> bloomr;
        DeviceBuffer<uint32_t> mid0, mid_bitmap, midc;
        uint32_t midc_wbits = 0, mid0_bits = 0;
        DeviceBuffer<uint32_t> blkc;
        uint32_t blkc_wbits = 0;
        void fill(const FlatIndex& idx, bool wide_hash, uint64_t mid_max_records);
        dev::BloomTables bloom_tables(bool mid) const;
    };
    IndexTables tables_;
    bool use_mid_ = false;
    int n_cus_ = 256;
    bool use_filter_ = false;
    bool use_direct_cands_ = false;
    int sketch_form() const;
    DeviceBuffer<uint32_t> d_covg_;
    DeviceBuffer<unsigned long long> d_counters_;
    PinnedBuffer<unsigned long long> h_counters_;
    uint64_t tot_reads_ = 0, tot_bases_ = 0, tot_hits_ = 0, tot_leftover_ = 0, tot_minimizers_ = 0;
    DeviceBuffer<uint64_t> d_key_a_, d_key_b_;
    DeviceBuffer<uint32_t> d_val_a_, d_val_b_;
    DeviceBuffer<uint32_t> d_head_, d_scan_, d_cstart_, d_order_;
    DeviceBuffer<dev::ClusterRec> d_clusters_;
    DeviceBuffer<unsigned char> d_temp_;
    uint64_t hit_capacity() const { return d_key_a_.size(); }
    Lane lanes_[2];
    static constexpr uint64_t MIN_CAPACITY_CLAMP = 4096;
    uint64_t min_capacity_ = 1u << 20;
    uint64_t reruns_filter_ = 0, reruns_direct_ = 0, regrows_hits_ = 0;
    struct TileSet {
        uint32_t slice_cap = 256, ws_tiles = 0, ws_cap = 0;
        DeviceBuffer<uint64_t> d_tile_info;
        DeviceBuffer<uint32_t> d_tile_pos1, d_tile_count, d_tile_hits, d_tile_nmin, d_tile_prefix;
        DeviceBuffer<uint4> d_tile_rec;
        DeviceBuffer<unsigned char> d_tile_temp;
        DeviceBuffer<uint32_t> d_tile_first;
        DeviceBuffer<uint16_t> d_nbits;
        bool nbits_dirty = false;
        uint32_t mark = 0, n_tiles = 0;
        dev::SketchArgs a_done {};
    };
    TileSet tsets_[2];
    dev::SketchArgs sketch_args(const DeviceBatch& batch, const TileSet* tiles) const;
    uint32_t slices_epoch_ = 0x80000000u;
    void ensure_tile_workspace(TileSet& t, uint32_t n_tiles, uint32_t tile_cap);
    void reserve_tile_first(TileSet& t, uint32_t n_tiles);
    struct BamScratch {
        DeviceBuffer<uint32_t> d_count, d_prefix;
        DeviceBuffer<unsigned char> d_temp;
    };
    struct Stage {
        DeviceBuffer<uint8_t> d_bases;
        DeviceBuffer<uint64_t> d_offsets, d_npos;
        Event copied;
        DeviceBuffer<uint8_t> d_seq, d_reverse;
        DeviceBuffer<uint64_t> d_seq_start;
        BamScratch bam;
    };
    void ensure_bam_scratch(BamScratch& s, uint64_t n_bases);
    DeviceBatch copy_in_bam(const HostBatch& hb, Stage& st, uint8_t* d_words, uint64_t* d_offsets, uint64_t* d_npos, hipStream_t copy_stream, hipStream_t stream);
    BamScratch bam_api_;
    uint64_t bam_blocks_ = 0;
    void ensure_stage(Stage& st, uint64_t payload_bytes, uint64_t n_reads, uint64_t n_npos);
    Stage stage_[2], stage_sync_;
    DeviceBatch copy_in(const HostBatch& hb, uint8_t* d_bases, uint64_t* d_offsets, uint64_t* d_npos, hipStream_t stream);
    int stage_next_ = 0;
    uint32_t ft_share_[2][4] = { { 0, 0, 0, 0 }, { 0, 0, 0, 0 } };
    uint64_t ft_last_[20] = {};
    void tune_filter_shares(const Lane& lane, bool packed, uint64_t n_bases);
    std::vector<DeviceBuffer<uint8_t>> kept_arenas_;
    uint8_t* arena_at_ = nullptr;
    size_t arena_left_ = 0;
    std::vector<DeviceBatch> kept_;
    uint64_t kept_cap_ = 0, kept_bytes_ = 0;
    bool kept_broken_ = false, in_keep_call_ = false;
    Event kept_copied_;
    void* arena_take(size_t bytes);
    DeviceBuffer<uint32_t> d_peer_tmp_;
    bool timing_ = false;
    double sketch_ms_ = 0;
    uint64_t sketch_launches_ = 0;
    Event ev0_, ev1_;
};

}
```

drprg_amd/csrc/read_cluster.hip:

```cpp
#include "filter_common.h"
#include <algorithm>
#include <cstdint>

namespace drprg {
namespace dev {

constexpr int RC_THREADS = 1024;
constexpr int RC_WAVES = RC_THREADS / 64;
constexpr int RC_PER = 2;
constexpr int RC_WG_PER_CU = 2;
constexpr int RC_SLOTS = RC_THREADS * RC_PER;
constexpr int RC_HCAP = 3072;
constexpr int RC_POOL = 512;
constexpr uint32_t RC_IRREGULAR = 2u, RC_COMPLEX = 1u;

__device__ __forceinline__ uint32_t pack_max(uint32_t earlier, uint32_t later)
{
    const uint32_t lead = (later >> 16) > (earlier >> 16) ? (later >> 16) : (earlier >> 16);
    const uint32_t seg = (later & 0xFFFFu) > (earlier & 0xFFFFu) ? (later & 0xFFFFu) : (earlier & 0xFFFFu);
    return (lead << 16) | seg;
}
__device__ __forceinline__ void lds_barrier() { asm volatile("s_waitcnt lgkmcnt(0)\n\ts_barrier" ::: "memory"); }
__device__ __forceinline__ void lds_barrier(int& t) { asm volatile("s_waitcnt lgkmcnt(0)\n\ts_barrier" : "+v"(t) : : "memory"); }

template <bool SLICES, int AHEAD>
__global__ __launch_bounds__(RC_THREADS, 4 * RC_WG_PER_CU) void read_cluster_kernel(SketchArgs a, FilterWork fw, ReadClusterArgs rc)
{
    constexpr int RC_AHEAD = AHEAD, RC_OWN = RC_SLOTS - AHEAD;
    static_assert(RC_OWN % 64 == 0, "the slices form locates 64 entries from a multiple of 64 per wave");
    (void)RC_AHEAD;
    extern __shared__ uint32_t s_hist[];
    __shared__ uint32_t s_read[RC_SLOTS + 1], s_hstart[RC_SLOTS + 1];
    __shared__ uint16_t s_pos1[RC_SLOTS];
    __shared__ uint32_t s_gt[RC_SLOTS];
    __shared__ uint16_t s_lead[RC_SLOTS];
    __shared__ uint16_t s_seg[RC_SLOTS];
    __shared__ uint16_t s_end[RC_SLOTS];
    __shared__ uint16_t s_g0[RC_SLOTS];
    __shared__ uint8_t s_dec[RC_SLOTS];
    __shared__ uint8_t s_cplx[RC_SLOTS], s_irrf[RC_SLOTS];
    __shared__ uint16_t s_grp[RC_HCAP];
    __shared__ uint16_t s_hpos[RC_HCAP];
    __shared__ uint32_t s_cov[RC_HCAP];
    __shared__ uint32_t s_w[2][RC_WAVES];
    __shared__ uint32_t s_irr[RC_POOL];
    __shared__ uint32_t s_prev_read, s_n_irr, s_chunk;
    __shared__ unsigned long long s_tot[3];

    int tid = threadIdx.x;
#define lane (tid & 63)
#define wave (tid >> 6)
    if (rc.n_wg && blockIdx.x == 0) {
        uint32_t h = 0, nm = 0, ml = 0;
        for (uint32_t g = (uint32_t)tid; g < rc.n_wg; g += RC_THREADS) {
            h += rc.wg_hits[g];
            nm += rc.wg_nmin[g];
            const uint32_t m = rc.wg_maxlen[g];
            ml = m > ml ? m : ml;
        }
        const uint32_t wh = wave_inclusive_scan(h), wn = wave_inclusive_scan(nm), wm = wave_max(ml);
        if (lane == 63) {
            s_w[0][wave] = wh;
            s_w[1][wave] = wn;
            s_irr[wave] = wm;
        }
        __syncthreads();
        if (tid == 0) {
            unsigned long long th = 0, tn = 0;
            uint32_t tm = 0;
            for (int i = 0; i < RC_WAVES; ++i) {
                th += s_w[0][i];
                tn += s_w[1][i];
                tm = s_irr[i] > tm ? s_irr[i] : tm;
            }
            *rc.tot_hits = th;
            if (tn && !(*reinterpret_cast<volatile const uint32_t*>(rc.overflow_word) & 4u)) atomicAdd(rc.tot_minimizers, tn);
            *rc.tot_max_len = (unsigned long long)tm;
        }
        __syncthreads();
    }
    if (*reinterpret_cast<volatile uint32_t*>(a.overflow) & 4u) return;
    const uint32_t total = SLICES ? rc.slice_prefix[rc.n_slices] : *fw.cand_total;
    const uint32_t handled_mark = SLICES ? rc.mark_epoch : 0u;
    uint16_t* const s_minpath = reinterpret_cast<uint16_t*>(s_hist + rc.n_prgs);
    for (uint32_t i = tid; i < rc.n_prgs; i += RC_THREADS) {
        s_hist[i] = 0;
        if (rc.minpath_in_lds) {
            const uint32_t m = rc.prg_min_path_len[i];
            s_minpath[i] = (uint16_t)(m < 0xFFFFu ? m : 0xFFFFu);
        }
    }
    if (tid < 3) s_tot[tid] = 0;
    unsigned long long my_kept_hits = 0;
    uint32_t my_kept = 0, my_complex = 0;
    const uint32_t w1_magic = w1_reciprocal(a.w);

    struct Staged {
        uint4 rec[RC_PER];
        uint32_t info[RC_PER], pos1[RC_PER], edge_prev, edge_next;
    };
    auto request = [&](uint32_t chunk) {
        Staged st;
        const uint64_t b64 = (uint64_t)chunk * RC_OWN;
        const bool live = b64 < total;
        const uint32_t b = live ? (uint32_t)b64 : 0u;
        const uint32_t n_in = total - b < (uint32_t)RC_SLOTS ? total - b : (uint32_t)RC_SLOTS;
        if constexpr (!SLICES) {
#pragma unroll
            for (int q = 0; q < RC_PER; ++q) {
                const uint32_t i = (uint32_t)tid + (uint32_t)q * RC_THREADS;
                const uint32_t src = b + (i < n_in ? i : 0u);
                st.info[q] = live ? (uint32_t)fw.cand_info[src] : 0u;
                st.pos1[q] = live ? fw.cand_pos1[src] : 0u;
                st.rec[q] = live ? fw.cand_rec[src] : make_uint4(0, 0, 0, 0);
            }
            const bool nxt = n_in == (uint32_t)RC_SLOTS && b + n_in < total;
            st.edge_prev = live ? (uint32_t)fw.cand_info[b ? b - 1 : 0u] : 0u;
            st.edge_next = live ? (uint32_t)fw.cand_info[nxt ? b + n_in : b] : 0u;
        } else {
            const uint32_t* __restrict__ P = rc.slice_prefix;
            uint32_t* const s_mine = s_gt + (wave << 6);
            const uint32_t d_last = b + n_in - 1;
            const bool nxt = n_in == (uint32_t)RC_SLOTS && b + n_in < total;
            uint32_t d0[RC_PER + 1], s0[RC_PER + 1], pj[RC_PER + 1], p0[RC_PER + 1], sn = 0, pn0 = 0;
            bool some[RC_PER + 1];
#pragma unroll
            for (int q = 0; q <= RC_PER; ++q) {
                d0[q] = q < RC_PER ? b + ((uint32_t)(wave << 6) + (uint32_t)q * RC_THREADS) : b - 64u;
                some[q] = q < RC_PER ? live && d0[q] <= d_last : live && b && wave == 0;
                s0[q] = some[q] ? rc.block_first[__builtin_amdgcn_readfirstlane(d0[q] >> 6)] : 0u;
            }
            const bool edge_n = live && nxt && wave == 0;
            if (edge_n) sn = rc.block_first[__builtin_amdgcn_readfirstlane((b + n_in) >> 6)];
#pragma unroll
            for (int q = 0; q <= RC_PER; ++q) {
                s0[q] = __builtin_amdgcn_readfirstlane(s0[q]);
                const uint32_t j1 = s0[q] + 1u + (uint32_t)lane;
                pj[q] = some[q] ? P[j1 < rc.n_slices ? j1 : rc.n_slices] : 0u;
                p0[q] = some[q] ? P[s0[q]] : 0u;
            }
            if (edge_n) pn0 = P[sn];
            auto locate = [&](int q, uint32_t d_hi) -> size_t {
                const uint32_t x = d0[q] + (uint32_t)lane <= d_hi ? (uint32_t)lane : d_hi - d0[q];
                if (__builtin_amdgcn_readlane(pj[q], 63) > d_hi) {
                    s_mine[lane] = 0;
                    const uint32_t pn = __shfl_down(pj[q], 1);
                    const uint32_t rel = pj[q] - d0[q];
                    if ((lane == 63 || pn != pj[q]) && rel < 64u) s_mine[rel] = (uint32_t)lane + 1u;
                    __builtin_amdgcn_wave_barrier();
                    uint32_t c = s_mine[lane];
                    __builtin_amdgcn_wave_barrier();
#pragma unroll
                    for (int off = 1; off < 64; off <<= 1) {
                        const uint32_t n = __shfl_up(c, off);
                        if (lane >= off) c = n > c ? n : c;
                    }
                    c = __shfl(c, (int)x);
                    const uint32_t before = __shfl(pj[q], (int)(c ? c - 1u : 0u));
                    return (size_t)(s0[q] + c) * a.tile_cap + (d0[q] + x - (c ? before : p0[q]));
                }
                const uint32_t d = d0[q] + x;
                uint32_t lo = s0[q], hi = rc.n_slices;
                while (hi - lo > 1) {
                    const uint32_t mid = (lo + hi) >> 1;
                    if (P[mid] <= d) lo = mid;
                    else hi = mid;
                }
                return (size_t)lo * a.tile_cap + (d - P[lo]);
            };
#pragma unroll
            for (int q = 0; q < RC_PER; ++q) {
                const size_t src = some[q] ? locate(q, d_last) : 0;
                st.info[q] = live ? (uint32_t)a.tile_info[src] : 0u;
                st.pos1[q] = live ? a.tile_pos1[src] : 0u;
                st.rec[q] = live ? a.tile_rec[src] : make_uint4(0, 0, 0, 0);
            }
            st.edge_prev = 0u;
            st.edge_next = 0u;
            if (wave == 0) {
                size_t e_prev = 0;
                if (some[RC_PER]) e_prev = (size_t)__shfl((unsigned long long)locate(RC_PER, b - 1u), 63);
                const size_t e_next = edge_n ? (size_t)sn * a.tile_cap + (b + n_in - pn0) : 0;
                st.edge_prev = some[RC_PER] ? (uint32_t)a.tile_info[e_prev] : 0u;
                st.edge_next = edge_n ? (uint32_t)a.tile_info[e_next] : 0u;
            }
        }
        return st;
    };
    auto take_ticket = [&]() -> uint32_t { return atomicAdd(rc.chunk_counter, 1u) + gridDim.x; };
    uint32_t cur = blockIdx.x;
    Staged nx = request(cur);
    for (;;) {
        lds_barrier(tid);
        const uint64_t base64 = (uint64_t)cur * RC_OWN;
        if (base64 >= total) break;
        const uint32_t base = (uint32_t)base64;
        const uint32_t n_loaded = total - base < (uint32_t)RC_SLOTS ? total - base : (uint32_t)RC_SLOTS;
        const uint32_t n_own = total - base < (uint32_t)RC_OWN ? total - base : (uint32_t)RC_OWN;
        uint32_t ticket = 0;
        if (tid == 0) ticket = take_ticket();
        uint4 crec[RC_PER];
        uint32_t st_read[RC_PER], st_pos1[RC_PER];
#pragma unroll
        for (int q = 0; q < RC_PER; ++q) {
            st_read[q] = nx.info[q];
            st_pos1[q] = nx.pos1[q];
            crec[q] = nx.rec[q];
        }
        const bool has_next = n_loaded == (uint32_t)RC_SLOTS && base + n_loaded < total;
        const uint32_t edge_prev = nx.edge_prev, edge_next = nx.edge_next;
#pragma unroll
        for (int q = 0; q < RC_PER; ++q) {
            const uint32_t i = (uint32_t)tid + (uint32_t)q * RC_THREADS;
            const bool in = i < n_loaded;
            st_read[q] = in ? st_read[q] & 0x7FFFFFFFu : READ_NONE;
            st_pos1[q] = in ? st_pos1[q] : 0u;
            if (!in) crec[q] = make_uint4(0, 0, 0, 0);
        }
#pragma unroll
        for (int q = 0; q < RC_PER; ++q) {
            const uint32_t i = (uint32_t)tid + (uint32_t)q * RC_THREADS;
            const uint32_t read = st_read[q], pos1 = st_pos1[q];
            if (!pos1) crec[q].y = 0;
            s_read[i] = read;
            s_pos1[i] = (uint16_t)(pos1 < 0xFFFFu ? pos1 : 0xFFFFu);
            s_hstart[i] = crec[q].y;
            s_g0[i] = (uint16_t)((crec[q].z >> 16) & 0x7FFFu);
            s_cplx[i] = 0;
            s_irrf[i] = 0;
        }
        if (tid == 0) {
            s_prev_read = base ? (edge_prev & 0x7FFFFFFFu) : 0xFFFFFFFFu;
            s_read[RC_SLOTS] = has_next ? (edge_next & 0x7FFFFFFFu) : 0xFFFFFFFFu;
            s_n_irr = 0;
// ... 153 lines not shown
                const uint32_t decision = s_dec[(uint32_t)s_seg[i] - 1];
                if (!decision) continue;
                fw.cand_pos1[base + i] = handled_mark;
                if (decision == 2) {
                    atomicAdd(&rc.covg[crec[q].w], 1u);
                    const uint32_t h0 = s_hstart[i];
                    for (uint32_t r = 1; r < cnt; ++r) atomicAdd(&rc.covg[s_cov[h0 + r]], 1u);
                }
            }
        }
        cur = s_chunk;
        nx = request(cur);
        const uint32_t n_irr = s_n_irr < (uint32_t)RC_POOL ? s_n_irr : (uint32_t)RC_POOL;
        for (uint32_t r = wave; r < n_irr; r += RC_WAVES) {
            const uint32_t i = s_irr[r] & 0xFFFFu, e = s_irr[r] >> 16;
            const uint32_t read = s_read[i], hb = s_hstart[i], he = s_hstart[e];
            const uint64_t len = a.offsets[read + 1] - a.offsets[read];
            uint32_t cl_g = 0, cl_n = 0, cl_first = 0, cl_last = 0;
            int nc = 0;
            bool complex = false;
            for (uint32_t b = hb; b < he && !complex; b += 64) {
                const uint32_t h = b + lane;
                const uint32_t hg = h < he ? s_grp[h] : 0u, hp = h < he ? s_hpos[h] : 0u;
                const bool valid = h < he;
                const uint64_t lt = (1ull << lane) - 1ull;
                uint64_t todo = __ballot(valid);
                while (todo) {
                    const uint32_t G = (uint32_t)__builtin_amdgcn_readlane((int)hg, __ffsll((long long)todo) - 1);
                    const uint64_t m = __ballot(valid && hg == G);
                    todo &= ~m;
                    const uint64_t open = __ballot(lane < nc && cl_g == G);
                    const int fo = open ? 63 - __clzll((long long)open) : -1;
                    const uint32_t open_last = fo >= 0 ? (uint32_t)__builtin_amdgcn_readlane((int)cl_last, fo) : 0u;
                    const uint64_t below = m & lt;
                    const int prev = below ? 63 - __clzll((long long)below) : -1;
                    const uint32_t prev_pos = __shfl(hp, prev < 0 ? lane : prev);
                    const bool member = ((m >> lane) & 1ull) != 0;
                    const bool start = member
                        && (prev >= 0 ? (int)(hp - prev_pos) > rc.max_diff : (fo < 0 || (int)(hp - open_last) > rc.max_diff));
                    const uint64_t starts = __ballot(start);
                    const int n_new = __popcll(starts);
                    if (nc + n_new > 64) {
                        complex = true;
                        break;
                    }
                    const uint64_t cont = m & (starts ? (1ull << (__ffsll((long long)starts) - 1)) - 1ull : ~0ull);
                    if (cont) {
                        const uint32_t lp = (uint32_t)__builtin_amdgcn_readlane((int)hp, 63 - __clzll((long long)cont));
                        if (lane == fo) {
                            cl_n += (uint32_t)__popcll(cont);
                            cl_last = lp;
                        }
                    }
                    const int c = lane - nc;
                    const bool mine = c >= 0 && c < n_new;
                    int first_lane = lane, last_lane = lane;
                    uint32_t span_n = 0;
                    if (mine) {
                        uint64_t mm = starts;
                        for (int k = 0; k < c; ++k) mm &= mm - 1;
                        first_lane = __ffsll((long long)mm) - 1;
                        const uint64_t rest = mm & (mm - 1);
                        const uint64_t upto = rest ? (1ull << (__ffsll((long long)rest) - 1)) - 1ull : ~0ull;
                        const uint64_t span = m & upto & ~((1ull << first_lane) - 1ull);
                        last_lane = 63 - __clzll((long long)span);
                        span_n = (uint32_t)__popcll(span);
                    }
                    const uint32_t fpos = __shfl(hp, first_lane), lpos = __shfl(hp, last_lane);
                    if (mine) {
                        cl_g = G;
                        cl_n = span_n;
                        cl_first = fpos;
                        cl_last = lpos;
                    }
                    nc += n_new;
                }
            }
            if (complex) {
                if (lane == 0) ++my_complex;
                continue;
            }
            const uint64_t expected = expected_minimizers(len, a.w, w1_magic);
            bool kept = false;
            if (lane < nc) {
                uint64_t m = rc.minpath_in_lds ? s_minpath[cl_g >> 1] : 0xFFFFu;
                if (m == 0xFFFFu) m = rc.prg_min_path_len[cl_g >> 1];
                if (expected < m) m = expected;
                const uint32_t length_based = (uint32_t)((double)m * rc.fraction);
                const uint32_t thr = length_based > rc.min_cluster_size ? length_based : rc.min_cluster_size;
                kept = cl_n > thr;
            }
            uint64_t alive = __ballot(kept);
            if (alive & (alive - 1)) {
                uint32_t rank = 0;
                for (uint64_t mm = alive; mm; mm &= mm - 1) {
                    const int o = __ffsll((long long)mm) - 1;
                    const uint32_t of = (uint32_t)__builtin_amdgcn_readlane((int)cl_first, o), on = (uint32_t)__builtin_amdgcn_readlane((int)cl_n, o),
                                   og = (uint32_t)__builtin_amdgcn_readlane((int)cl_g, o);
                    rank += (of < cl_first || (of == cl_first && (on > cl_n || (on == cl_n && og < cl_g)))) ? 1u : 0u;
                }
                const int nk = __popcll(alive);
                int prev = -1;
                uint32_t pg = 0, pn = 0, p_last = 0;
                for (int o = 0; o < nk; ++o) {
                    const int cur = __ffsll((long long)__ballot(kept && rank == (uint32_t)o)) - 1;
                    const uint32_t cg = (uint32_t)__builtin_amdgcn_readlane((int)cl_g, cur), cn = (uint32_t)__builtin_amdgcn_readlane((int)cl_n, cur),
                                   c_last = (uint32_t)__builtin_amdgcn_readlane((int)cl_last, cur);
                    if (prev >= 0) {
                        const bool same_prg_other_strand = (pg >> 1) == (cg >> 1) && (pg & 1u) != (cg & 1u);
                        if (same_prg_other_strand || c_last <= p_last) {
                            if (pn >= cn) {
                                alive &= ~(1ull << cur);
                                continue;
                            }
                            alive &= ~(1ull << prev);
                        }
                    }
                    prev = cur;
                    pg = cg;
                    pn = cn;
                    p_last = c_last;
                }
            }
            if ((alive >> lane) & 1ull) {
                atomicAdd(&s_hist[cl_g >> 1], 1u);
                ++my_kept;
                my_kept_hits += cl_n;
            }
            for (uint32_t b = hb; b < he; b += 64) {
                const uint32_t h = b + lane;
                const uint32_t hg = h < he ? s_grp[h] : 0xFFFFFFFFu, hp = h < he ? s_hpos[h] : 0u;
                for (uint64_t mm = alive; mm; mm &= mm - 1) {
                    const int o = __ffsll((long long)mm) - 1;
                    const uint32_t og = (uint32_t)__builtin_amdgcn_readlane((int)cl_g, o), of = (uint32_t)__builtin_amdgcn_readlane((int)cl_first, o),
                                   ol = (uint32_t)__builtin_amdgcn_readlane((int)cl_last, o);
                    if (hg == og && hp >= of && hp <= ol) atomicAdd(&rc.covg[s_cov[h]], 1u);
                }
            }
            for (uint32_t c = i + lane; c < e; c += 64)
                if (s_pos1[c]) fw.cand_pos1[base + c] = handled_mark;
        }
    }
    if (my_kept) atomicAdd(&s_tot[0], (unsigned long long)my_kept);
    if (my_kept_hits) atomicAdd(&s_tot[1], my_kept_hits);
    if (my_complex) atomicAdd(&s_tot[2], (unsigned long long)my_complex);
    __syncthreads();
    for (uint32_t i = tid; i < rc.n_prgs; i += RC_THREADS)
        if (s_hist[i]) atomicAdd(&rc.prg_reads[i], s_hist[i]);
    if (tid == 0) {
        if (s_tot[0]) atomicAdd(rc.n_clusters_kept, s_tot[0]);
        if (s_tot[1]) atomicAdd(rc.n_hits_kept, s_tot[1]);
        if (s_tot[2]) atomicAdd(rc.n_complex, s_tot[2]);
    }
}
#undef lane
#undef wave

constexpr int CH_THREADS = 256;
__global__ __launch_bounds__(CH_THREADS) void counters_home_kernel(unsigned long long* from, unsigned long long* to, uint32_t n, uint4* zero, uint32_t n_zero4)
{
    const uint32_t i = threadIdx.x;
    if (i < n) {
        to[i] = from[i];
        from[i] = 0;
    }
    for (uint32_t j = i; j < n_zero4; j += CH_THREADS) zero[j] = make_uint4(0, 0, 0, 0);
}
hipError_t launch_counters_home(unsigned long long* from, unsigned long long* to, uint32_t n, hipStream_t stream, uint32_t* zero, uint32_t n_zero)
{
    if (n > CH_THREADS || (n_zero & 3u) || (reinterpret_cast<uintptr_t>(zero) & 15u)) return hipErrorInvalidValue;
    hipLaunchKernelGGL(counters_home_kernel, dim3(1), dim3(CH_THREADS), 0, stream, from, to, n, reinterpret_cast<uint4*>(zero), zero ? n_zero / 4 : 0u);
    return hipGetLastError();
}

__global__ void flag_complex_kernel(const unsigned long long* n_hits, unsigned long long* n_complex)
{
    if (*n_hits) *n_complex = 1;
}

hipError_t launch_read_cluster(const SketchArgs& a, const FilterWork& fw, const ReadClusterArgs& rc, int n_cus, bool skip, hipStream_t stream)
{
    if (skip) {
        hipLaunchKernelGGL(flag_complex_kernel, dim3(1), dim3(1), 0, stream, a.n_hits, rc.n_complex);
        return hipGetLastError();
    }
    ReadClusterArgs rcd = rc;
    size_t dyn = (size_t)rc.n_prgs * sizeof(uint32_t);
    {
        static size_t static_lds = 0;
        if (!static_lds) {
            size_t most = 0;
            for (const void* k : { reinterpret_cast<const void*>(&read_cluster_kernel<false, 128>), reinterpret_cast<const void*>(&read_cluster_kernel<false, 256>),
                     reinterpret_cast<const void*>(&read_cluster_kernel<false, 512>), reinterpret_cast<const void*>(&read_cluster_kernel<true, 128>),
                     reinterpret_cast<const void*>(&read_cluster_kernel<true, 256>), reinterpret_cast<const void*>(&read_cluster_kernel<true, 512>) }) {
                hipFuncAttributes at {};
                HIP_TRY(hipFuncGetAttributes(&at, k));
                most = std::max<size_t>(most, at.sharedSizeBytes);
            }
            static_lds = most;
        }
        const size_t lds_cu = 160 * 1024, with = dyn + (size_t)rc.n_prgs * sizeof(uint16_t);
        const size_t fit_without = std::min<size_t>(lds_cu / (static_lds + dyn), RC_WG_PER_CU), fit_with = std::min<size_t>(lds_cu / (static_lds + with), RC_WG_PER_CU);
        rcd.minpath_in_lds = fit_with == fit_without ? 1u : 0u;
        if (rcd.minpath_in_lds) dyn = with;
    }
    const uint64_t mean_len = a.n_bases / (a.n_reads ? a.n_reads : 1u);
    const int ahead = mean_len <= 300 ? 128 : mean_len <= 600 ? 256 : 512;
    static size_t configured[6][MAX_HIP_DEVICES] = {};
    auto launch = [&](auto kernel, size_t (&conf)[MAX_HIP_DEVICES]) -> hipError_t {
        HIP_TRY(ensure_dynamic_lds(reinterpret_cast<const void*>(kernel), dyn, conf));
        hipLaunchKernelGGL(kernel, dim3((uint32_t)n_cus * RC_WG_PER_CU), dim3(RC_THREADS), dyn, stream, a, fw, rcd);
        return hipGetLastError();
    };
    if (rcd.slice_prefix) {
        if (ahead == 128) HIP_TRY(launch(&read_cluster_kernel<true, 128>, configured[0]));
        else if (ahead == 256) HIP_TRY(launch(&read_cluster_kernel<true, 256>, configured[1]));
        else HIP_TRY(launch(&read_cluster_kernel<true, 512>, configured[2]));
    } else {
        if (ahead == 128) HIP_TRY(launch(&read_cluster_kernel<false, 128>, configured[3]));
        else if (ahead == 256) HIP_TRY(launch(&read_cluster_kernel<false, 256>, configured[4]));
        else HIP_TRY(launch(&read_cluster_kernel<false, 512>, configured[5]));
    }
    return hipGetLastError();
}

}
}
```

drprg_amd/csrc/sketch_filter.hip:

```cpp
#include "filter_common.h"
#include <algorithm>
#include <cstdint>
#include <type_traits>

namespace drprg {
namespace dev {

__device__ inline uint32_t pack16le(const uint4& in)
{
    constexpr uint32_t W = 0x40100401u;
    const uint32_t p0 = __builtin_amdgcn_udot4(in.x & 0x06060606u, W, 0u, false), p1 = __builtin_amdgcn_udot4(in.y & 0x06060606u, W, 0u, false);
    const uint32_t p2 = __builtin_amdgcn_udot4(in.z & 0x06060606u, W, 0u, false), p3 = __builtin_amdgcn_udot4(in.w & 0x06060606u, W, 0u, false);
    return ((p0 | (p1 << 8) | (p2 << 16)) >> 1) | (p3 << 23);
}


typedef __attribute__((address_space(3))) const uint32_t lds_cu32;
__device__ __forceinline__ uint32_t lds_at(uint32_t byte_addr) { return *(lds_cu32*)(uintptr_t)byte_addr; }
__device__ __forceinline__ uint32_t bloom_test(uint32_t word, uint32_t h, uint32_t x)
{
    uint32_t t2;
    asm("v_lshlrev_b32_sdwa %0, %1, %2 dst_sel:DWORD dst_unused:UNUSED_PAD src0_sel:BYTE_1 src1_sel:DWORD" : "=v"(t2) : "v"(h), "v"(word));
    return (word << (h & 31)) & t2 & (word << ((x >> 16) & 0xFF));
}

__device__ __forceinline__ uint32_t canon12_dev(uint32_t x)
{
    const uint32_t m = x & 0xFFFFFFu;
    const uint32_t r = __builtin_bitreverse32(x);
    const uint32_t rc = ((r >> 9) & 0x555555u) | (~(r >> 7) & 0xAAAAAAu);
    return m < rc ? m : rc;
}

template <bool SHORT_K, bool LEVEL0, bool FUSED = false, int MID = 0, bool PACKED = false>
__global__ __launch_bounds__(FT_THREADS) void sketch_filter_kernel(SketchArgs a, FilterWork fw)
{
    static_assert(FUSED == LEVEL0, "the level-0 form runs its second stage in this kernel");
    static_assert(MID == 0 || (LEVEL0 && FUSED), "the middle tier is a variant of the level-0 form with the second stage inside");
    extern __shared__ uint32_t s_dyn[];
    constexpr int G = filter_positions_per_lane(LEVEL0, PACKED), WPOS = 63 * G, NW = G / 16, NG = G / 4;
    constexpr uint32_t L12_BASE = LEVEL0 ? FT_L0_WORDS * 4u : 0u;
    constexpr bool CANON = MID == 1 || MID == 3;
    auto group_key = [](uint32_t x) -> uint32_t {
        if constexpr (CANON) return canon12_dev(x);
        else return x;
    };
    (void)group_key;
    constexpr uint32_t STAGE_RECORDS = 128, STAGE_CAP = STAGE_RECORDS - 1, STAGE_BASE_WORDS = FT_L0_WORDS;

    const int tid = threadIdx.x, lane = tid & 63;
    const int k = a.k;
    const int64_t n_bases = (int64_t)a.n_bases;
    const uint32_t n_words = 1u << fw.bloom_wbits;
    const uint32_t amask = (n_words - 1) << 2;
    const uint32_t amask0 = ((1u << fw.bloom0_wbits) - 1) << 2;
    const uint32_t kmask = (k < 16) ? ((1u << (2 * k)) - 1) : 0xFFFFFFFFu;
    const uint32_t kmask24 = kmask & 0xFFFFFFu;
    const int sh_w = 32 - (int)fw.bloom_wbits;
    const uint32_t sh_c = 32u - fw.midc_wbits;
    (void)sh_c;

    auto fill = [&](uint32_t lds_word0, const uint32_t* __restrict__ from, uint32_t n) {
        const uint4* __restrict__ src = reinterpret_cast<const uint4*>(from);
        uint4* dst = reinterpret_cast<uint4*>(s_dyn + lds_word0);
        for (uint32_t i = tid; i < n / 4; i += FT_THREADS) dst[i] = src[i];
    };
    if constexpr (LEVEL0) {
        constexpr int ROUNDS = FT_L0_WORDS / 4 / FT_THREADS;
        const uint4* __restrict__ src = reinterpret_cast<const uint4*>(fw.bloom0);
        uint4* dst = reinterpret_cast<uint4*>(s_dyn);
        uint4 v[ROUNDS];
#pragma unroll
        for (int r = 0; r < ROUNDS; ++r) v[r] = src[tid + r * FT_THREADS];
#pragma unroll
        for (int r = 0; r < ROUNDS; ++r) dst[tid + r * FT_THREADS] = v[r];
    }
    if (!LEVEL0) fill(L12_BASE / 4, fw.bloom, n_words);
    if (tid == 0 && (uint32_t)(uintptr_t)(__attribute__((address_space(3))) uint32_t*)s_dyn != 0u) atomicOr(a.overflow, 8u);

    const uint32_t wv = (uint32_t)(tid >> 6);
    const uint64_t win_lo = a.offsets[fw.read_begin], win_hi = a.offsets[fw.read_end];
    const uint32_t t_lo = (uint32_t)(win_lo / WPOS), t_hi = (uint32_t)((win_hi + WPOS - 1) / WPOS);
    const uint32_t n_waves = gridDim.x * FT_WAVES;
    const uint32_t per_wg = fw.sched.per_wg;
    const bool dynamic = per_wg > FT_WAVES;
    if (dynamic && (t_lo != 0 || t_hi != fw.sched.n_tiles)) {
        if (tid == 0) atomicOr(a.overflow, 32u);
        return;
    }
    const uint32_t tiles_per_wave = fw.sched.tpw0 ? fw.sched.tpw0 : (t_hi - t_lo + n_waves - 1) / n_waves;
    const uint32_t wg_lo = dynamic ? t_lo + (uint32_t)((uint64_t)blockIdx.x * (t_hi - t_lo) / gridDim.x) : (uint32_t)std::min<uint64_t>((uint64_t)t_lo + (uint64_t)blockIdx.x * FT_WAVES * tiles_per_wave, t_hi);
    const uint32_t wg_hi = dynamic ? t_lo + (uint32_t)((uint64_t)(blockIdx.x + 1) * (t_hi - t_lo) / gridDim.x) : (uint32_t)std::min<uint64_t>((uint64_t)wg_lo + (uint64_t)FT_WAVES * tiles_per_wave, t_hi);
    if (fw.class_clock && tid == 0) atomicMax(&fw.class_clock[0], ~(unsigned long long)wall_clock64());
    auto bound = [&](uint32_t i) -> uint32_t {
        uint32_t cum = (i & 3u) * fw.wave_share[(i >> 2) & 3u];
        for (uint32_t c = 0; c < (i >> 2); ++c) cum += 4u * fw.wave_share[c];
        const uint64_t t = (uint64_t)wg_lo + ((uint64_t)tiles_per_wave * FT_WAVES * cum) / 4096u;
        return t < (uint64_t)wg_hi ? (uint32_t)t : wg_hi;
    };
    auto chunk_of_ticket = [&](uint32_t kt, uint32_t& b, uint32_t& e) {
        uint32_t ft = fw.sched.first_ticket[1], tl = fw.sched.first_tile[1], sz = fw.sched.size[1];
#pragma unroll
        for (int q = 2; q < FT_MAX_ROUNDS; ++q)
            if (kt >= fw.sched.first_ticket[q]) {
                ft = fw.sched.first_ticket[q];
                tl = fw.sched.first_tile[q];
                sz = fw.sched.size[q];
            }
        b = wg_lo + tl + (kt - ft) * sz;
        e = kt + 1u == per_wg ? wg_hi : b + sz;
    };
    uint32_t tile = (uint32_t)__builtin_amdgcn_readfirstlane((int)bound(wv));
    uint32_t c_all = (uint32_t)__builtin_amdgcn_readfirstlane((int)bound(wv + 1));
    const uint32_t slice0 = blockIdx.x * per_wg;
    uint32_t slice = (uint32_t)__builtin_amdgcn_readfirstlane((int)(slice0 + wv));
    bool decoded = !dynamic, has_next = false;
    uint32_t n_k = 0, n_begin = 0, n_all = 0;
    auto slice_geometry = [&](uint32_t kt, uint32_t b, uint32_t e, uint32_t& base, uint32_t& cap) {
        base = blockIdx.x * fw.slice_budget + (b - wg_lo) * fw.slice_cpt + kt * fw.slice_slack;
        cap = (e - b) * fw.slice_cpt + fw.slice_slack;
        if (kt >= fw.slice_extra_from) {
            base += (kt - fw.slice_extra_from) * fw.slice_extra;
            cap += fw.slice_extra;
        }
    };
    uint32_t base_cur, cap_cur;
    slice_geometry(wv, tile, c_all, base_cur, cap_cur);
    base_cur = (uint32_t)__builtin_amdgcn_readfirstlane((int)base_cur);
    cap_cur = (uint32_t)__builtin_amdgcn_readfirstlane((int)cap_cur);
    if (tid == 0) s_dyn[fw.sched.lds_word] = 0;

    auto load16 = [&](int64_t g) -> uint4 {
        if (g + 16 <= n_bases) return *reinterpret_cast<const uint4*>(a.bases + g);
        uint32_t t4[4];
        for (int q = 0; q < 4; ++q) {
            uint32_t wd = 0;
            for (int b = 0; b < 4; ++b) {
                const int64_t gg = g + q * 4 + b;
                wd |= (uint32_t)(gg < n_bases ? a.bases[gg] : (uint8_t)'N') << (8 * b);
            }
            t4[q] = wd;
        }
        return make_uint4(t4[0], t4[1], t4[2], t4[3]);
    };
    (void)load16;
    struct PairAscii {
        uint4 a, b;
    };
    using Pair = typename std::conditional<PACKED, typename std::conditional<NW == 4, uint4, uint2>::type, PairAscii>::type;
    const uint32_t* const words = reinterpret_cast<const uint32_t*>(a.bases);
    const int64_t n_pwords = (n_bases + 15) >> 4;
    (void)words; (void)n_pwords;
    const uint32_t n_full = PACKED ? (n_pwords >= NW * 64 ? (uint32_t)((n_pwords - NW * 64) / (WPOS / 16)) + 1 : 0u)
                                   : (n_bases >= 64 * G ? (uint32_t)((n_bases - 64 * G) / WPOS) + 1 : 0u);
    uint32_t c_end = c_all < n_full ? c_all : n_full;
    auto fetch = [&](uint32_t t, Pair& p) {
        if constexpr (PACKED) {
            p = *reinterpret_cast<const Pair*>(words + (int64_t)t * (WPOS / 16) + (int64_t)lane * NW);
        } else {
            const uint8_t* g = a.bases + (int64_t)t * WPOS + (int64_t)lane * G;
            p.a = *reinterpret_cast<const uint4*>(g);
            p.b = *reinterpret_cast<const uint4*>(g + 16);
        }
    };
    uint64_t* out = fw.raw_pos + base_cur;
    uint32_t lane_keep = lane == 63 ? 0u : 0xFFFFFFFFu;
    asm volatile("" : "+v"(lane_keep));
    uint32_t wcur = 0;
    uint4* const stage = FUSED ? reinterpret_cast<uint4*>(s_dyn + STAGE_BASE_WORDS) + (tid >> 6) * STAGE_RECORDS : nullptr;
    uint32_t lcnt = 0;
    (void)stage;
    auto mb_below = [](uint64_t m) { return __builtin_amdgcn_mbcnt_hi((uint32_t)(m >> 32), __builtin_amdgcn_mbcnt_lo((uint32_t)m, 0u)); };
    (void)mb_below;
#define DRPRG_STAGE2_APPEND(r, cand2_in)                                                                                              \
    do {                                                                                                                              \
        uint32_t cand2 = (cand2_in);                                                                                                  \
                                               \
        const uint32_t c2 = (uint32_t)__popc(cand2);                                                                                  \
        const uint64_t e0 = __ballot(c2 & 1u), e1 = __ballot(c2 & 2u), e2 = __ballot(c2 & 4u);                                        \
        if (e0 | e1 | e2) {                                                                                                           \
            uint32_t at2 = wcur + mb_below(e0) + 2u * mb_below(e1) + 4u * mb_below(e2);                                               \
            const uint64_t pos2 = ((uint64_t)(r).y << 32) | (r).x;                                                                    \
            while (cand2) {                                                                                                           \
                const int q2 = __ffs(cand2) - 1;                                                                                      \
                cand2 &= cand2 - 1;                                                                                                   \
                if (at2 < cap_cur) out[at2] = pos2 + (uint64_t)q2;                                                                    \
                ++at2;                                                                                                                \
            }                                                                                                                         \
            wcur += (uint32_t)(__popcll(e0) + 2 * __popcll(e1) + 4 * __popcll(e2));                                                   \
        }                                                                                                                             \
    } while (0)
#define DRPRG_BLOCK_TEST(r, b, dst)                                                                                                   \
    do {                                                                                                                              \
        _Pragma("unroll") for (int q = 0; q < 4; ++q) {                                                                               \
            const uint32_t f = (q ? __funnelshift_r((r).z, (r).w, 2 * q) : (r).z) & kmask;                                            \
            const uint32_t h = f * BLOOM_CR;                                                                                          \
            dst |= (((b).x >> (h >> 27)) & ((b).y >> ((h >> 22) & 31)) & ((b).z >> ((h >> 17) & 31)) & ((b).w >> ((h >> 12) & 31)) & 1u) << q; \
        }                                                                                                                             \
    } while (0)
#define DRPRG_SECOND_STAGE()                                                                                                          \
    do {                                                                                                                              \
        if (lcnt) {                                                                                                                   \
            __builtin_amdgcn_wave_barrier();                  \
            if constexpr (MID != 0) {                                                                                                 \
                                             \
                for (uint32_t c0 = 0; c0 < lcnt; c0 += 128) {                                                                         \
                    const uint32_t ia = c0 + (uint32_t)lane, ib = ia + 64;                                                            \
                    uint4 ra = make_uint4(0, 0, 0, 0), rb = ra, ba = ra, bb = ra;                                                     \
                    if (ia < lcnt) {                                                                                                  \
                        ra = stage[ia];                                                                                               \
                        ba = reinterpret_cast<const uint4*>(fw.midc)[(uint32_t)__umul24(group_key(__funnelshift_r(ra.z, ra.w, 6)), BLOOM_C0) >> sh_c];  \
                    }                                                                                                                 \
                    if (ib < lcnt) {                                                                                                  \
                        rb = stage[ib];                                                                                               \
                        bb = reinterpret_cast<const uint4*>(fw.midc)[(uint32_t)__umul24(group_key(__funnelshift_r(rb.z, rb.w, 6)), BLOOM_C0) >> sh_c]; \
                    }                                                                                                                 \
                    uint32_t ca = 0, cb = 0;                                                                                          \
                    DRPRG_BLOCK_TEST(ra, ba, ca);                            \
                    DRPRG_STAGE2_APPEND(ra, ca);                                                                                      \
                    if (c0 + 64 < lcnt) {                                                                           \
                        DRPRG_BLOCK_TEST(rb, bb, cb);                                                                                 \
                        DRPRG_STAGE2_APPEND(rb, cb);                                                                                  \
                    }                                                                                                                 \
                }                                                                                                                     \
            } else {                                                                                                                  \
                for (uint32_t c0 = 0; c0 < lcnt; c0 += 64) {                                                                          \
                    const uint32_t ri = c0 + (uint32_t)lane;                                                                          \
                    uint32_t cs = 0;                                                                                                  \
                    uint4 r = make_uint4(0, 0, 0, 0);                                                                                 \
                    if (ri < lcnt) {                                                                                                  \
                        r = stage[ri];                                                                                                \
                                                                     \
                        uint32_t hq[4], h2q[4], wq[4];                                                                                \
                        _Pragma("unroll") for (int q = 0; q < 4; ++q) {                                                               \
                            const uint32_t f = (q ? __funnelshift_r(r.z, r.w, 2 * q) : r.z) & kmask;                                  \
                            hq[q] = f * BLOOM_CR;                                                                                     \
                            h2q[q] = f * BLOOM_C2;                                                                                    \
                            wq[q] = lds_at((hq[q] >> 17) << 2);                                                                       \
                        }                                                                                                             \
                        __builtin_amdgcn_sched_barrier(0);      \
// ... 84 lines not shown
                    return make_uint4((uint32_t)pos, (uint32_t)(pos >> 32), __funnelshift_r(lo, hi, sh), hi >> sh);
                };
                if (lcnt + total > STAGE_CAP) DRPRG_SECOND_STAGE();
                if (total <= STAGE_CAP) {
                    uint32_t at = lcnt + lanes_below();
                    while (grp) {
                        const int g = __ffs(grp) - 1;
                        grp &= grp - 1;
                        stage[at++] = record(g);
                    }
                    lcnt += total;
                } else {
                    constexpr int PART_LANES = (int)STAGE_CAP / NG;
                    for (int part = 0; part < (64 + PART_LANES - 1) / PART_LANES; ++part) {
                        uint32_t gq = (lane / PART_LANES) == part ? grp : 0u;
                        const uint32_t cq = (uint32_t)__popc(gq);
                        const uint64_t q0 = __ballot(cq & 1u), q1 = __ballot(cq & 2u), q2 = __ballot(cq & 4u), q3 = __ballot(cq & 8u);
                        const uint64_t q4 = NG > 8 ? __ballot(cq & 16u) : 0ull;
                        uint32_t at = below(q0) + 2u * below(q1) + 4u * below(q2) + 8u * below(q3) + (NG > 8 ? 16u * below(q4) : 0u);
                        while (gq) {
                            const int g = __ffs(gq) - 1;
                            gq &= gq - 1;
                            stage[at++] = record(g);
                        }
                        lcnt = (uint32_t)(__popcll(q0) + 2 * __popcll(q1) + 4 * __popcll(q2) + 8 * __popcll(q3) + (NG > 8 ? 16 * __popcll(q4) : 0));
                        DRPRG_SECOND_STAGE();
                    }
                }
            }
            return;
        }
        uint32_t cand = 0;
        uint32_t c1 = 0;
        {
#pragma unroll
            for (int j = FT_G - 1; j >= 0; --j) {
                const uint32_t lo = j < 16 ? wa : wb, hi = j < 16 ? wb : wc;
                uint32_t x = (j & 15) ? __builtin_amdgcn_alignbit(hi, lo, 2 * (j & 15)) : lo;
                if (SHORT_K) x &= kmask24;
                const uint32_t h = __umul24(x, BLOOM_C1);
                c1 = __builtin_amdgcn_alignbit(c1, bloom_test(lds_at(L12_BASE + ((h >> 16) & amask)), h, x), 31);
            }
            if (lane == 63) c1 = 0;
        }
        while (c1) {
            const int j = __ffs(c1) - 1;
            c1 &= c1 - 1;
            const uint32_t lo = j < 16 ? wa : wb, hi = j < 16 ? wb : wc;
            const uint32_t f = __funnelshift_r(lo, hi, 2 * (j & 15)) & kmask;
            const uint32_t h2 = f * BLOOM_C2;
            const uint32_t word = lds_at(L12_BASE + ((h2 >> sh_w) << 2));
            cand |= ((word >> (h2 & 31)) & (word >> ((h2 >> 5) & 31)) & (word >> ((h2 >> 10) & 31)) & 1u) << j;
        }
        uint64_t m = __ballot(cand != 0);
        while (m) {
            const int l = __ffsll((unsigned long long)m) - 1;
            m &= m - 1;
            const uint32_t c = (uint32_t)__builtin_amdgcn_readlane((int)cand, l);
            if (lane == l) {
                const uint64_t base = (uint64_t)t * WPOS + (uint64_t)lane * G;
                uint32_t cc = c, at = wcur;
                while (cc) {
                    const int j = __ffs(cc) - 1;
                    cc &= cc - 1;
                    if (at < cap_cur) out[at] = base + (uint64_t)j;
                    ++at;
                }
            }
            wcur += (uint32_t)__popc(c);
        }
    };

    auto decode_next = [&]() {
        uint32_t drawn = 0;
        if (lane == 0) drawn = atomicAdd(&s_dyn[fw.sched.lds_word], 1u);
        const uint32_t kt = (uint32_t)FT_WAVES + (uint32_t)__builtin_amdgcn_readfirstlane((int)drawn);
        has_next = kt < per_wg;
        if (has_next) {
            n_k = kt;
            chunk_of_ticket(kt, n_begin, n_all);
            if (lane == 0 && n_begin + FT_DEPTH > (n_all < n_full ? n_all : n_full)) atomicOr(a.overflow, 16u);
        }
        decoded = true;
    };
    auto ahead2 = [&]() -> uint32_t {
        uint32_t ft = tile + FT_DEPTH;
        if (ft >= c_end) {
            if (!decoded) decode_next();
            ft = has_next ? n_begin + (ft - c_end) : c_end - 1;
        }
        return ft;
    };
    auto advance = [&]() {
        ++tile;
        if (tile >= c_end && has_next) {
            close_slice();
            slice = slice0 + n_k;
            slice_geometry(n_k, n_begin, n_all, base_cur, cap_cur);
            out = fw.raw_pos + base_cur;
            wcur = 0;
            tile = n_begin;
            c_all = n_all;
            c_end = n_all < n_full ? n_all : n_full;
            has_next = false;
            decoded = false;
        }
    };
    Pair r0 {}, r1 {}, r2 {}, r3 {};
    const bool pipelined = tile < c_end;
    if (pipelined) {
        fetch(tile, r0);
        fetch(tile + 1 < c_end ? tile + 1 : tile, r1);
        fetch(tile + 2 < c_end ? tile + 2 : tile, r2);
    }
    __syncthreads();
    if (pipelined)
        for (;;) {
            fetch(ahead2(), r3);
            process(tile, r0);
            advance();
            if (tile >= c_end) break;
            fetch(ahead2(), r0);
            process(tile, r1);
            advance();
            if (tile >= c_end) break;
            fetch(ahead2(), r1);
            process(tile, r2);
            advance();
            if (tile >= c_end) break;
            fetch(ahead2(), r2);
            process(tile, r3);
            advance();
            if (tile >= c_end) break;
        }
    for (; tile < c_all; ++tile) {
        const int64_t g = (int64_t)tile * WPOS + (int64_t)lane * G;
        Pair p;
        if constexpr (PACKED) {
            const int64_t wi = g >> 4;
            p.x = wi < n_pwords ? words[wi] : 0u;
            p.y = wi + 1 < n_pwords ? words[wi + 1] : 0u;
            if constexpr (NW == 4) {
                p.z = wi + 2 < n_pwords ? words[wi + 2] : 0u;
                p.w = wi + 3 < n_pwords ? words[wi + 3] : 0u;
            }
        } else {
            p.a = load16(g);
            p.b = load16(g + 16);
        }
        process(tile, p);
    }
    close_slice();
    if (fw.class_clock && (tid & 255) == 0) atomicMax(&fw.class_clock[1 + (tid >> 8)], (unsigned long long)wall_clock64());
}
#undef DRPRG_SECOND_STAGE
#undef DRPRG_BLOCK_TEST
#undef DRPRG_STAGE2_APPEND

uint32_t filter_n_tiles(uint64_t n_bases, int positions_per_lane)
{
    const uint64_t wpos = 63ull * (uint64_t)positions_per_lane;
    return (uint32_t)((n_bases + wpos - 1) / wpos);
}

uint32_t filter_grid(bool level0, int n_cus, uint32_t n_tiles, uint32_t cap)
{
    uint32_t grid = (uint32_t)n_cus * (level0 ? 1 : 2);
    const uint32_t need = (n_tiles + FT_WAVES - 1) / FT_WAVES;
    if (grid > need) grid = need;
    if (grid > (uint32_t)(MAX_SLICES / FT_WAVES)) grid = MAX_SLICES / FT_WAVES;
    if (cap && grid > cap) grid = cap;
    return grid ? grid : 1;
}

constexpr size_t FT_SMALL_HEAD = (size_t)MAX_CHUNKS * 3 + MAX_SLICES;
size_t filter_small_words() { return FT_SMALL_HEAD + 4 + 4 * (size_t)MAX_EX_WG; }
uint32_t* filter_super_counts(uint32_t* small) { return small + MAX_CHUNKS; }
uint32_t filter_super_words() { return (uint32_t)MAX_SLICES; }

FilterSched make_filter_sched(uint32_t n_tiles, uint32_t n_wg, const uint32_t share[4], const FilterSchedKnobs& knobs)
{
    FilterSched s {};
    for (int r = 0; r < FT_MAX_ROUNDS; ++r) s.first_ticket[r] = 0xFFFFFFFFu;
    s.n_rounds = 1;
    s.per_wg = FT_WAVES;
    s.n_tiles = n_tiles;
    s.tpw0 = (n_tiles + n_wg * FT_WAVES - 1) / (n_wg * FT_WAVES);
    uint32_t min_share = share[0];
    for (int c = 1; c < 4; ++c) min_share = std::min(min_share, share[c]);
    const uint64_t wg_tiles = n_tiles / n_wg, avg = wg_tiles / FT_WAVES;
    const uint32_t tpw0 = (uint32_t)(avg * knobs.f / 256);
    if (knobs.is_static || avg < knobs.min_avg || (uint64_t)tpw0 * min_share / 256 < FT_DEPTH + 2) return s;
    const uint32_t max_per_wg = (uint32_t)MAX_CHUNKS / n_wg;
    uint64_t done = (uint64_t)FT_WAVES * tpw0, rest = wg_tiles - done;
    if (rest < FT_DEPTH + 2) return s;
    uint32_t tk = FT_WAVES;
    int r = 1;
    for (; r < FT_MAX_ROUNDS - 1 && tk + 2 * FT_WAVES <= max_per_wg; ++r) {
        const uint32_t sz = (uint32_t)(rest * 16 / ((uint64_t)FT_WAVES * knobs.d));
        if (sz < 2 * knobs.m) break;
        s.first_ticket[r] = tk;
        s.first_tile[r] = (uint32_t)done;
        s.size[r] = sz;
        done += (uint64_t)FT_WAVES * sz;
        rest -= (uint64_t)FT_WAVES * sz;
        tk += FT_WAVES;
    }
    const uint32_t left = max_per_wg - tk;
    const uint32_t sz = (uint32_t)std::max<uint64_t>(knobs.m, (rest + left - 1) / left);
    const uint32_t cnt = (uint32_t)std::max<uint64_t>(1, (rest - (FT_DEPTH - 2)) / sz);
    s.first_ticket[r] = tk;
    s.first_tile[r] = (uint32_t)done;
    s.size[r] = sz;
    s.n_rounds = (uint32_t)r + 1;
    s.per_wg = tk + cnt;
    s.tpw0 = tpw0;
    return s;
}

void init_candidate_work(FilterWork& fw, const FilterBuffers& b, int n_cus)
{
    fw.cand_info = b.cand_info;
    fw.cand_pos1 = b.cand_pos1;
    fw.cand_rec = b.cand_rec;
    fw.wg_hits = b.small + FT_SMALL_HEAD + 4;
    fw.wg_nmin = fw.wg_hits + MAX_EX_WG;
    fw.wg_maxlen = fw.wg_nmin + MAX_EX_WG;
    fw.wg_base = fw.wg_maxlen + MAX_EX_WG;
    fw.ex_grid = std::min<uint32_t>((uint32_t)n_cus * 8, MAX_EX_WG);
    fw.verify_grid = fw.ex_grid;
    fw.max_len = b.max_len;
}

const uint32_t* filter_builtin_shares(bool mid, bool packed)
{
    static const uint32_t ascii_l0[4] = { 397, 294, 200, 133 }, packed_l0[4] = { 422, 292, 184, 126 }, mid_l0[4] = { 356, 292, 220, 156 };
    return mid ? mid_l0 : packed ? packed_l0 : ascii_l0;
}

hipError_t launch_sketch_filter(const SketchArgs& a, const BloomTables& bt, int n_cus, const FilterBuffers& b, const ReadClusterArgs& rc, FilterWork& fw,
    const Switches& sw, hipStream_t stream, KernelTimer timer)
{
    fw = FilterWork {};
    fw.read_begin = 0;
    fw.read_end = a.n_reads;
    if (a.n_bases == 0) return hipSuccess;
    const bool mid = bt.mid_bitmap != nullptr;
    if (mid && (a.k != 15 || !bt.mid0 || !bt.midc || bt.midc_wbits < 1 || bt.midc_wbits > MID_C_MAX_WBITS || (bt.mid0_bits != 1 && bt.mid0_bits != 3)))
        return hipErrorInvalidValue;
    if (!mid && (1u << bt.bloom_wbits) > (uint32_t)FT_BLOOM_WORDS) return hipErrorInvalidValue;
    if (!mid && bt.bloom0 && (1u << bt.bloom0_wbits) != (uint32_t)FT_L0_WORDS) return hipErrorInvalidValue;
    if (!mid && bt.bloom0 && (!bt.bloomr || !bt.bloom0f)) return hipErrorInvalidValue;
    const bool level0 = mid || (bt.bloom0 != nullptr && a.k == 15 && ((size_t)4 << bt.bloom_wbits) + (size_t)FT_L0_WORDS * 4 <= 160 * 1024);
    const bool want_l2 = sw.stage2 == Stage2::by_format ? a.packed != 0 : sw.stage2 == Stage2::l2;
    const bool blk = !mid && level0 && want_l2 && bt.blkc != nullptr && bt.blkc_wbits >= 1 && bt.blkc_wbits <= MID_C_MAX_WBITS;
    fw.bloom = bt.bloom;
    fw.bloom_wbits = bt.bloom_wbits;
    fw.bloom0 = mid ? bt.mid0 : (level0 ? (blk ? bt.bloom0 : bt.bloom0f) : nullptr);
    fw.bloom0_wbits = mid ? 15 : (level0 ? bt.bloom0_wbits : 0);
    fw.mid_bitmap = bt.mid_bitmap;
    fw.midc = blk ? bt.blkc : bt.midc;
    fw.midc_wbits = blk ? bt.blkc_wbits : bt.midc_wbits;
    const uint32_t grid = filter_grid(level0, n_cus, filter_n_tiles(a.n_bases, filter_positions_per_lane(level0, a.packed != 0)), sw.ft_grid);
    {
        static const uint32_t even[4] = { 256, 256, 256, 256 };
        const uint32_t* share = sw.ft_share_pinned ? sw.ft_share : !level0 ? even : b.wave_share ? b.wave_share : filter_builtin_shares(mid, a.packed != 0);
        fw.class_clock = level0 && !sw.ft_share_pinned ? b.class_clock : nullptr;
        for (int c = 0; c < 4; ++c) fw.wave_share[c] = share[c];
    }
    fw.sched = make_filter_sched(filter_n_tiles(a.n_bases, filter_positions_per_lane(level0, a.packed != 0)), grid, fw.wave_share, sw.ft_sched);
    fw.n_slices = grid * fw.sched.per_wg;
    {
        const uint32_t n_tiles = filter_n_tiles(a.n_bases, filter_positions_per_lane(level0, a.packed != 0));
        const uint64_t budget = std::min<uint64_t>(b.raw_capacity, 0x7FFFFFFFull) / grid;
        const uint64_t wg_tiles = fw.sched.per_wg > (uint32_t)FT_WAVES ? (n_tiles + grid - 1) / grid : (uint64_t)FT_WAVES * ((n_tiles + grid * FT_WAVES - 1) / (grid * FT_WAVES));
        fw.slice_budget = (uint32_t)budget;
        fw.slice_extra = 0;
        fw.slice_extra_from = 0xFFFFFFFFu;
        const bool last_round = fw.sched.n_rounds > 1;
        const uint64_t reserve = last_round ? budget / 4 : 0, main = budget - reserve;
        fw.slice_slack = (uint32_t)std::min<uint64_t>(256, main / (4ull * fw.sched.per_wg));
        const uint64_t tiles = std::max<uint64_t>(wg_tiles, 1);
        fw.slice_cpt = (uint32_t)((main - (uint64_t)fw.slice_slack * fw.sched.per_wg) / tiles);
        if (last_round) {
            const uint32_t last = fw.sched.n_rounds - 1, from = fw.sched.first_ticket[last], n_last = fw.sched.per_wg - from;
            const uint64_t tile_pos = 63ull * (uint64_t)filter_positions_per_lane(level0, a.packed != 0);
            const uint64_t sz = fw.sched.size[last], want = sz * tile_pos * 2 / (uint64_t)(a.w + 1);
            const uint64_t have = sz * fw.slice_cpt + fw.slice_slack;
            if (n_last && want > have) {
                fw.slice_extra = (uint32_t)std::min<uint64_t>(want - have, reserve / n_last);
                fw.slice_extra_from = from;
            }
        }
    }
    fw.raw_pos = b.raw_pos;
    fw.cand_info = b.cand_info;
    fw.cand_pos1 = b.cand_pos1;
    fw.cand_rec = b.cand_rec;
    init_candidate_work(fw, b, n_cus);
    fw.slice_count = b.small;
    fw.super_count = filter_super_counts(b.small);
    fw.slice_base = b.small + MAX_CHUNKS + MAX_SLICES;
    fw.slice_cap = fw.slice_base + MAX_CHUNKS;
    fw.cand_count = b.small + FT_SMALL_HEAD;
    fw.cand_total = fw.cand_count;
    {
        using Kernel = void (*)(SketchArgs, FilterWork);
        const int which = mid ? (bt.mid0_bits == 3 ? 3 : 4) : blk ? 5 : level0 ? 2 : (a.k < 12 ? 1 : 0);
        const Kernel ascii = which == 5 ? &sketch_filter_kernel<false, true, true, 2>
            : which == 4                ? &sketch_filter_kernel<false, true, true, 1>
            : which == 3                ? &sketch_filter_kernel<false, true, true, 3>
            : which == 2                ? &sketch_filter_kernel<false, true, true>
            : which == 1                ? &sketch_filter_kernel<true, false>
                                        : &sketch_filter_kernel<false, false>;
        const Kernel packed = which == 5 ? &sketch_filter_kernel<false, true, true, 2, true>
            : which == 4                 ? &sketch_filter_kernel<false, true, true, 1, true>
            : which == 3                 ? &sketch_filter_kernel<false, true, true, 3, true>
            : which == 2                 ? &sketch_filter_kernel<false, true, true, 0, true>
            : which == 1                 ? &sketch_filter_kernel<true, false, false, 0, true>
                                         : &sketch_filter_kernel<false, false, false, 0, true>;
        const Kernel kernel = a.packed ? packed : ascii;
        const size_t dyn = level0 ? (size_t)FT_L0_WORDS * 4 + (size_t)FT_WAVES * 2048 : ((size_t)4 << bt.bloom_wbits) + 16;
        fw.sched.lds_word = (uint32_t)(dyn / 4 - 4);
        static size_t configured[12][MAX_HIP_DEVICES] = {};
        HIP_TRY(ensure_dynamic_lds(reinterpret_cast<const void*>(kernel), dyn, configured[which + (a.packed ? 6 : 0)]));
        launch_timed(timer, kernel, dim3(grid), dim3(FT_THREADS), dyn, stream, a, fw);
    }
    HIP_TRY(hipGetLastError());
    const bool skip_rc = sw.skip_read_cluster;
    HIP_TRY(launch_candidate_stage(a, fw, rc, n_cus, stream, skip_rc));
    ReadClusterArgs rct = rc;
    if (!skip_rc) {
        rct.wg_hits = fw.wg_hits;
        rct.wg_nmin = fw.wg_nmin;
        rct.wg_maxlen = fw.wg_maxlen;
        rct.n_wg = fw.verify_grid;
        rct.tot_hits = a.n_hits;
        rct.tot_minimizers = a.n_minimizers;
        rct.tot_max_len = fw.max_len;
        rct.overflow_word = a.overflow;
    }
    return launch_read_cluster(a, fw, rct, n_cus, skip_rc, stream);
}

}
}
```

drprg_amd/pandora.py:

```python
import ctypes as C
import os
import re

import numpy as np

from ._lib import MapOpts, lib

MTB_GENOME_SIZE = 4411532


class DependencyError(RuntimeError):

    def __init__(self, kind, message, code=0):
        super().__init__(f"{kind}: {message}")
        self.kind = kind
        self.code = code


def _check(rc, ctx=None):
    if rc != 0:
        msg = lib.drprg_hip_last_error(ctx)
        raise DependencyError("ProcessError", (msg or b"").decode() or f"error {rc}", code=-rc)


# ... 120 lines not shown
        _check(lib.drprg_hip_max_covg_info(self._h, out), self._h)
        return dict(reached=bool(out[0]), reads=int(out[1]), bases=int(out[2]), dropped=int(out[3]))

    def keep_reads(self, max_bytes):
        _check(lib.drprg_hip_keep_reads(self._h, int(max_bytes)), self._h)

    def map_resident(self, other):
        _check(lib.drprg_hip_map_resident(self._h, other._h), self._h)

    def resident_info(self):
        out = (C.c_uint64 * 4)()
        _check(lib.drprg_hip_resident_info(self._h, out), self._h)
        return dict(complete=bool(out[0]), bytes=int(out[1]), blocks=int(out[2]), last_discover_from_hbm=bool(out[3]))

    def select_reads(self, anchors, A, window_bytes=0):
        anchors = np.ascontiguousarray(anchors, dtype=np.uint64)
        out = (C.c_uint64 * 2)()
        offsets = np.zeros(1, np.uint64)
        rc = lib.drprg_hip_select_reads(self._h, _ptr(anchors), anchors.size, int(A), int(window_bytes), None, 0, _ptr(offsets), None, 0, out)
        if rc == 0:
            return np.zeros(0, np.uint8), offsets, np.zeros(0, np.uint64)
        if rc != -75:
            _check(rc, self._h)
        n_reads, n_bases = int(out[0]), int(out[1])
        bases, offsets, ids = np.zeros(n_bases, np.uint8), np.zeros(n_reads + 1, np.uint64), np.zeros(n_reads, np.uint64)
        _check(lib.drprg_hip_select_reads(self._h, _ptr(anchors), anchors.size, int(A), int(window_bytes), _ptr(bases), n_bases, _ptr(offsets),
                                          _ptr(ids), n_reads, out), self._h)
        return bases, offsets, ids

    def counters(self):
        out = (C.c_uint64 * 8)()
        _check(lib.drprg_hip_counters(self._h, out), self._h)
        names = ("reads", "bases", "minimizers", "hits", "clusters_kept", "hits_kept", "kernel", "leftover_reads")
        return dict(zip(names, (int(x) for x in out)))

    def genotype(self, vcf_refs, out_vcf, sample="sample"):
        _check(lib.drprg_hip_genotype(self._h, os.fsencode(vcf_refs) if vcf_refs else None, os.fsencode(out_vcf),
                                      sample.encode()), self._h)
        gi = (C.c_uint32 * 4)()
        lib.drprg_hip_genotype_info(self._h, gi)
        return dict(exp_depth_covg=int(gi[0]), min_kmer_covg=int(gi[1]), loci_present=int(gi[2]), records=int(gi[3]))

    def coverage_model(self):
        out = (C.c_double * 12)()
        _check(lib.drprg_hip_coverage_model(self._h, out), self._h)
        names = ("exp_depth_covg", "binomial", "e_rate", "nb_p", "nb_r", "branch", "mean", "var", "reads_per_locus", "bin_p", "thresh",
                 "dropped_low_coverage")
        d = dict(zip(names, (float(x) for x in out)))
        for key in ("exp_depth_covg", "binomial", "branch", "reads_per_locus", "thresh", "dropped_low_coverage"):
            d[key] = int(d[key])
        return d

    def discover(self, vcf_refs, out_dir, sample="sample"):
        n = C.c_uint32()
        _check(lib.drprg_hip_discover(self._h, os.fsencode(vcf_refs) if vcf_refs else None, os.fsencode(out_dir), sample.encode(),
                                      C.byref(n)), self._h)
        regions = []
        for line in open(os.path.join(out_dir, "candidate_regions.tsv")):
            if not line.startswith("#"):
                f = line.rstrip("\n").split("\t")
                regions.append(dict(locus=f[0], start=int(f[1]), end=int(f[2]), low_start=int(f[3]), low_end=int(f[4]),
                                    max_covg=int(f[5]), seq=f[6]))
        assert len(regions) == n.value
        return regions

    def discover_reads(self, reads, vcf_refs, out_dir, sample="sample", list_loci=True):
        out = (C.c_uint32 * 3)()
        _check(lib.drprg_hip_discover_reads(self._h, os.fsencode(reads), os.fsencode(vcf_refs) if vcf_refs else None, os.fsencode(out_dir),
                                            sample.encode(), 1 if list_loci else 0, out), self._h)
        variants = []
        for line in open(os.path.join(out_dir, "denovo_variants.tsv")):
            if not line.startswith("#"):
                f = line.rstrip("\n").split("\t")
                variants.append((f[0], int(f[1]), "" if f[2] == "." else f[2], "" if f[3] == "." else f[3], int(f[4]), int(f[5])))
        assert len(variants) == out[1]
        return variants

    def update_prg(self, out_prg):
        n = C.c_uint32()
        _check(lib.drprg_hip_update_prg(self._h, os.fsencode(out_prg), C.byref(n)), self._h)
        return int(n.value)

    def update_prg_from_paths(self, denovo_paths, out_prg):
        n = C.c_uint32()
        _check(lib.drprg_hip_update_prg_from_paths(self._h, os.fsencode(denovo_paths), os.fsencode(out_prg), C.byref(n)), self._h)
        return int(n.value)

    def save_coverage(self, path, tag):
        _check(lib.drprg_hip_save_coverage(self._h, os.fsencode(path), tag.encode()), self._h)

    def load_coverage(self, path, tag):
        rc = lib.drprg_hip_load_coverage(self._h, os.fsencode(path), tag.encode(), None)
        if rc == -2:
            return False
        _check(rc, self._h)
        return True

    def genotype_alleles(self, out_tsv):
        _check(lib.drprg_hip_genotype_alleles(self._h, os.fsencode(out_tsv)), self._h)
        out = {}
        for line in open(out_tsv):
            if line.startswith("#"):
                continue
            chrom, pos, a, n, nodes = line.rstrip("\n").split("\t")
            out[(chrom, int(pos), int(a))] = np.array([int(x) for x in nodes.split(",") if x], dtype=np.int64)
        return out

    def filter_selfcheck(self):
        out = (C.c_uint64 * 8)()
        _check(lib.drprg_hip_filter_selfcheck(self._h, out), self._h)
        names = ("codes", "level0_false_negatives", "level12_false_negatives", "stage2_false_negatives", "level0_fill_permille",
                 "level12_fill_permille", "stage2_fill_permille", "shared_array_false_negatives")
        return dict(zip(names, (int(x) for x in out)))

    def table_tier(self):
        out = (C.c_uint64 * 6)()
        _check(lib.drprg_hip_device_tables(self._h, out), self._h)
        return dict(pbloom_words=int(out[0]), table_bytes=int(out[1]), lds_filter_bytes=int(out[2]), kernel=int(out[3]),
                    l2_filter_bytes=int(out[4]), sketch_form=int(out[5]))

    def export_index(self):
        keys = np.zeros(self.n_keys, dtype=np.uint64)
        rec_off = np.zeros(self.n_keys + 1, dtype=np.uint32)
        rec_prg = np.zeros(self.n_records, dtype=np.uint32)
        rec_knode = np.zeros(self.n_records, dtype=np.uint32)
        rec_strand = np.zeros(self.n_records, dtype=np.uint8)
        min_path_len = np.zeros(self.n_prgs, dtype=np.uint32)
        knode_base = np.zeros(self.n_prgs + 1, dtype=np.uint32)
        _check(lib.drprg_hip_index_export(self._h, _ptr(keys), _ptr(rec_off), _ptr(rec_prg), _ptr(rec_knode), _ptr(rec_strand),
                                          _ptr(min_path_len), _ptr(knode_base)), self._h)
        return dict(keys=keys, rec_off=rec_off, rec_prg=rec_prg, rec_knode=rec_knode, rec_strand=rec_strand,
                    min_path_len=min_path_len, knode_base=knode_base)

    def prg_nodes(self, prg):
        n, ns = C.c_uint32(), C.c_uint32()
        _check(lib.drprg_hip_prg_nodes(self._h, prg, None, None, 0, C.byref(n), C.byref(ns)), self._h)
        starts = np.zeros(n.value, dtype=np.uint32)
        ends = np.zeros(n.value, dtype=np.uint32)
        _check(lib.drprg_hip_prg_nodes(self._h, prg, _ptr(starts), _ptr(ends), n.value, C.byref(n), C.byref(ns)), self._h)
        return starts, ends, int(ns.value)

    def filter_schedule(self):
        out = (C.c_uint64 * 20)()
        _check(lib.drprg_hip_filter_schedule(self._h, out), self._h)
        v = [int(x) for x in out]
        return {"form": "dynamic" if v[0] > 1 else "static", "rounds": v[0], "slices": v[1], "slices_per_workgroup": v[11], "round0_tiles_per_wave": v[2],
                "round0_class_shares_per_256": v[3:7], "chunk_tiles_per_round": [x for x in v[13:20] if x],
                "class_end_us": [round(x / 100.0, 1) for x in v[7:11]]}

    def buffer_info(self):
        out = (C.c_uint64 * 6)()
        _check(lib.drprg_hip_buffer_info(self._h, out), self._h)
        return dict(filter_reruns=int(out[0]), direct_reruns=int(out[1]), hit_regrows=int(out[2]), lane_capacity=int(out[3]),
                    hit_capacity=int(out[4]))

    def kernel_timing(self, enable=True, reset=False):
        ms, n = C.c_double(), C.c_uint64()
        _check(lib.drprg_hip_kernel_timing(self._h, 1 if enable else 0, 1 if reset else 0, C.byref(ms), C.byref(n)), self._h)
        return ms.value, int(n.value)


def allele_stats(fwd, rev, min_kmer_covg):
    fwd = np.ascontiguousarray(fwd, dtype=np.uint32)
    rev = np.ascontiguousarray(rev, dtype=np.uint32)
    out = np.zeros(6, np.uint32)
    gaps = C.c_double()
    _check(lib.drprg_hip_allele_stats(_ptr(fwd), _ptr(rev), len(fwd), min_kmer_covg, _ptr(out), C.byref(gaps)))
    return [int(x) for x in out], gaps.value


def genotype_site(mean_fwd, mean_rev, gaps, e, eps=0.01):
    mf = np.ascontiguousarray(mean_fwd, dtype=np.uint32)
    mr = np.ascontiguousarray(mean_rev, dtype=np.uint32)
    g = np.ascontiguousarray(gaps, dtype=np.float64)
    lik = np.zeros(len(mf), np.float64)
    gt, conf = C.c_int32(), C.c_double()
    _check(lib.drprg_hip_genotype_site(_ptr(mf), _ptr(mr), _ptr(g), len(mf), e, eps, _ptr(lik), C.byref(gt), C.byref(conf)))
    return lik, gt.value, conf.value


class Pandora:

    def __init__(self, device=0):
        self.device = device

    @staticmethod
    def _parse_args(args):
        o = dict(threads=1, w=14, k=15, c=10, illumina=False, max_covg=300)
        it = iter([str(a) for a in args])
        for a in it:
            if a == "-t":
                o["threads"] = int(next(it))
            elif a == "-w":
                o["w"] = int(next(it))
            elif a == "-k":
                o["k"] = int(next(it))
            elif a == "-c":
                o["c"] = int(next(it))
            elif a == "-I":
                o["illumina"] = True
            elif a == "--max-covg":
                o["max_covg"] = int(next(it))
            elif a == "-K":
                pass
            else:
                raise DependencyError("ProcessError", f"unknown pandora option {a}", code=2)
        return o

    @staticmethod
    def _struct_args(args):
        return ["--max-covg", "4294967295"] + [str(a) for a in args]

    def index_with(self, prg_path, args=()):
        o = self._parse_args(args)
        _check(lib.drprg_hip_index(os.fsencode(prg_path), o["w"], o["k"], o["threads"]))

    def _mapped_context(self, prg, reads, args):
        o = self._parse_args(args)
        ctx = Context(prg, o["w"], o["k"], device=self.device)
        ctx.set_opts(illumina=o["illumina"], min_cluster_size=o["c"], genome_size=MTB_GENOME_SIZE)
        ctx.set_max_covg(o["max_covg"])
        ctx.map_fastx(reads)
        return ctx

    @staticmethod
    def _run_tag(prg, reads, args):
        def stamp(p):
            st = os.stat(p)
            return f"{os.path.realpath(p)}:{st.st_size}:{st.st_mtime_ns}"
        rest, it = [], iter(str(a) for a in args)
        for a in it:
            if a == "--max-covg":
                next(it, None)
            elif a != "-K":
                rest.append(a)
        return "|".join([stamp(prg), stamp(reads)] + rest + [f"M{Pandora._parse_args(args)['max_covg']}"])

    COVERAGE_CACHE = ".drprg_hip_coverage"

    def discover_with(self, prg, query_idx, outdir, args=(), list_loci=False):
        import warnings
        os.makedirs(outdir, exist_ok=True)
        args = self._struct_args(args)
        with open(query_idx) as fh:
            sample, reads = fh.readline().split()[:2]
        with self._mapped_context(prg, reads, args) as ctx:
            ctx.set_threads(self._parse_args(args)["threads"])
            self.novel_variants = ctx.discover_reads(reads, None, outdir, sample, list_loci=list_loci)
            ctx.save_coverage(os.path.join(outdir, self.COVERAGE_CACHE), self._run_tag(prg, reads, args))
        if self.novel_variants and not list_loci:
            warnings.warn(f"discover: {len(self.novel_variants)} novel variant(s) found (denovo_variants.tsv) but not listed in "
                          "denovo_paths.txt: the PRG will not be updated")
        path = os.path.join(outdir, "denovo_paths.txt")
        if not os.path.exists(path):
            raise DependencyError("MissingExpectedOutput", path)
        return path

    def genotype_with(self, prg, vcf_ref, reads, outdir, args=()):
        os.makedirs(outdir, exist_ok=True)
        args = self._struct_args(args)
        o = self._parse_args(args)
        cache = os.path.join(outdir, "discover", self.COVERAGE_CACHE)
        ctx = Context(prg, o["w"], o["k"], device=self.device)
        with ctx:
            ctx.set_opts(illumina=o["illumina"], min_cluster_size=o["c"], genome_size=MTB_GENOME_SIZE)
            ctx.set_max_covg(o["max_covg"])
            self.reused_discover_coverage = os.path.exists(cache) and ctx.load_coverage(cache, self._run_tag(prg, reads, args))
            if not self.reused_discover_coverage:
                ctx.map_fastx(reads)
            ctx.genotype(vcf_ref, os.path.join(outdir, self.vcf_filename()))

    @staticmethod
    def vcf_filename():
        return "pandora_genotyped.vcf"

    @staticmethod
    def list_prgs_with_novel_variants(denovo_file):
        try:
            contents = open(denovo_file).read()
        except OSError:
            raise DependencyError("NovelVariantParsingError", f"Unable to read {denovo_file!r}")
        m = re.search(r"\n(?P<num>\d+) loci with denovo variants\n", contents)
        if not m:
            raise DependencyError("NovelVariantParsingError", "Unable to find line describing the number of novel variants")
        expected = int(m.group("num"))
        genes, prev = [], ""
        for line in contents.splitlines():
            if line.endswith("nodes"):
                genes.append(prev)
            prev = line
        if len(genes) != expected:
            raise DependencyError("NovelVariantParsingError",
                                  f"Expected {expected} genes with novel variants, but found {len(genes)}")
        return genes


def pack_reads(bases):
    bases = np.ascontiguousarray(bases, dtype=np.uint8)
    words = np.zeros((bases.size + 15) // 16, dtype=np.uint32)
    cap = 1024
    while True:
        npos = np.zeros(cap, dtype=np.uint64)
        n = C.c_uint64()
        rc = lib.drprg_hip_pack_reads(_ptr(bases), bases.size, _ptr(words), _ptr(npos), cap, C.byref(n))
        if rc == 0:
            return words, npos[:n.value].copy()
        if rc != -75:
# ... 3 lines not shown
```

Before: 20.91 billion.

## Compute superblock prefix and share bounds once in filter epilogue, fuse totals/home into tails

```diff
diff --git a/drprg_amd/csrc/candidates.hip b/drprg_amd/csrc/candidates.hip
--- a/drprg_amd/csrc/candidates.hip
+++ b/drprg_amd/csrc/candidates.hip
@@ -1,4 +1,5 @@
 #include "filter_common.h"
+#include "share_bounds.h"
 #include "verify_lane.h"
 #include <algorithm>
 #include <cstdint>
@@ -7,65 +8,41 @@
 namespace dev {
 
 constexpr int VS_THREADS = 512;
-constexpr int VS_PER = MAX_SLICES / VS_THREADS;
+static_assert(VS_WINDOW <= VS_THREADS, "one prefix per thread fills the window");
 template <int KC, bool PACKED>
 __global__ __launch_bounds__(VS_THREADS, 8) void verify_scan_kernel(SketchArgs a, FilterWork fw, ReadClusterArgs rc)
 {
     __shared__ uint32_t s_red[3][VS_THREADS / 64];
-    __shared__ uint32_t s_w[VS_THREADS / 64 + 1];
-    __shared__ uint32_t s_share[2];
-    __shared__ __attribute__((aligned(16))) uint32_t s_pre[MAX_SLICES + 4];
+    __shared__ uint32_t s_flag;
+    __shared__ uint32_t s_pre[VS_WINDOW];
     const int tid = threadIdx.x;
-    static_assert(VS_PER % 4 == 0 && MAX_SLICES % (VS_THREADS * 4) == 0, "the counts are read 16 bytes at a time");
-    auto my_count = [&](int i4) -> uint4 {
-        return reinterpret_cast<const uint4*>(fw.super_count + (size_t)tid * VS_PER)[i4];
-    };
-    uint32_t run = 0;
-    uint4 v[VS_PER / 4];
-#pragma unroll
-    for (int i = 0; i < VS_PER / 4; ++i) v[i] = my_count(i);
-#pragma unroll
-    for (int i = 0; i < VS_PER / 4; ++i) run += v[i].x + v[i].y + v[i].z + v[i].w;
-    uint32_t total;
-    const uint32_t before = block_exclusive_scan<VS_THREADS / 64>(run, s_w, &total);
-    if (blockIdx.x == 0 && tid == 0) *fw.cand_count = total;
-    const uint32_t per_wg = (total + gridDim.x - 1) / gridDim.x;
-    const uint64_t b64 = (uint64_t)blockIdx.x * per_wg;
-    const uint32_t t_begin = b64 < total ? (uint32_t)b64 : total, t_end = b64 + per_wg < total ? (uint32_t)(b64 + per_wg) : total;
-    {
-        const uint32_t x0 = t_begin, x1 = t_end - 1u;
-        const bool own0 = t_begin < t_end && before <= x0 && x0 < before + run, own1 = t_begin < t_end && before <= x1 && x1 < before + run;
-        uint32_t acc = before, n0 = 0, n1 = 0;
-        uint4* dst = reinterpret_cast<uint4*>(s_pre + (size_t)tid * VS_PER);
-#pragma unroll
-        for (int i = 0; i < VS_PER / 4; ++i) {
-            uint4 p;
-            p.x = acc;
-            p.y = p.x + v[i].x;
-            p.z = p.y + v[i].y;
-            p.w = p.z + v[i].z;
-            acc = p.w + v[i].w;
-            dst[i] = p;
-            n0 += (p.y <= x0 ? 1u : 0u) + (p.z <= x0 ? 1u : 0u) + (p.w <= x0 ? 1u : 0u) + (acc <= x0 ? 1u : 0u);
-            n1 += (p.y <= x1 ? 1u : 0u) + (p.z <= x1 ? 1u : 0u) + (p.w <= x1 ? 1u : 0u) + (acc <= x1 ? 1u : 0u);
-        }
-        if (tid == VS_THREADS - 1) s_pre[MAX_SLICES] = acc;
-        if (own0) s_share[0] = (uint32_t)tid * VS_PER + n0;
-        if (own1) s_share[1] = (uint32_t)tid * VS_PER + n1;
-    }
+    const uint4 share = fw.share_bounds[blockIdx.x];
+    const uint32_t t_begin = (uint32_t)__builtin_amdgcn_readfirstlane((int)share.x), t_end = (uint32_t)__builtin_amdgcn_readfirstlane((int)share.y);
+    const uint32_t s_lo = (uint32_t)__builtin_amdgcn_readfirstlane((int)share.z), s_hi = (uint32_t)__builtin_amdgcn_readfirstlane((int)share.w);
+    const bool wide = s_hi - s_lo + 2u > VS_WINDOW;
+    if (!wide && (uint32_t)tid < s_hi - s_lo + 2u) s_pre[tid] = fw.super_prefix[s_lo + (uint32_t)tid];
+    if (wide && tid == 0 && fw.wide_shares) atomicAdd(fw.wide_shares, 1u);
     __syncthreads();
     const VerifyConsts c(a, fw);
     uint32_t my_hits = 0, my_nmin = 0, my_maxlen = 0;
     auto position_in = [&](uint32_t t, uint32_t lo0, uint32_t hi0, uint32_t step0) -> int64_t {
-        uint32_t lo = lo0;
-        for (uint32_t step = step0; step >= 1; step >>= 1)
-            if (lo + step <= hi0 && s_pre[lo + step] <= t) lo += step;
+        uint32_t lo = lo0, pre_lo;
+        if (wide) {
+            const uint32_t* __restrict__ gp = fw.super_prefix;
+            for (uint32_t step = step0; step >= 1; step >>= 1)
+                if (lo + step <= hi0 && gp[lo + step] <= t) lo += step;
+            pre_lo = gp[lo];
+        } else {
+            for (uint32_t step = step0; step >= 1; step >>= 1)
+                if (lo + step <= hi0 && s_pre[lo + step - lo0] <= t) lo += step;
+            pre_lo = s_pre[lo - lo0];
+        }
         static_assert(FT_SUPER == 8, "two uint4 of slice counts per superblock");
         const uint4* __restrict__ c4 = reinterpret_cast<const uint4*>(fw.slice_count) + (size_t)lo * 2;
         const uint4* __restrict__ b4 = reinterpret_cast<const uint4*>(fw.slice_base) + (size_t)lo * 2;
         const uint4 ca = c4[0], cb = c4[1], ba = b4[0], bb = b4[1];
         const uint32_t cnt[7] = { ca.x, ca.y, ca.z, ca.w, cb.x, cb.y, cb.z }, start[8] = { ba.x, ba.y, ba.z, ba.w, bb.x, bb.y, bb.z, bb.w };
-        uint32_t rest = t - s_pre[lo], sum = 0, before = 0, at = start[0];
+        uint32_t rest = t - pre_lo, sum = 0, before = 0, at = start[0];
 #pragma unroll
         for (int q = 0; q < 7; ++q) {
             sum += cnt[q];
@@ -76,7 +53,6 @@
         return (int64_t)fw.raw_pos[(size_t)at + (rest - before)];
     };
     {
-        const uint32_t s_lo = (uint32_t)__builtin_amdgcn_readfirstlane((int)s_share[0]), s_hi = (uint32_t)__builtin_amdgcn_readfirstlane((int)s_share[1]);
         const uint32_t span_step = s_hi > s_lo ? 1u << (31 - __builtin_clz(s_hi - s_lo)) : 1u;
         auto position_of = [&](uint32_t t) -> int64_t { return position_in(t, s_lo, s_hi, span_step); };
         int64_t gp_next = t_begin + tid < t_end ? position_of(t_begin + (uint32_t)tid) : 0;
@@ -104,9 +80,43 @@
             n += s_red[1][i];
             mx = s_red[2][i] > mx ? s_red[2][i] : mx;
         }
-        fw.wg_hits[blockIdx.x] = h;
-        fw.wg_nmin[blockIdx.x] = n;
-        fw.wg_maxlen[blockIdx.x] = mx;
+        store_device(fw.wg_hits + blockIdx.x, h);
+        store_device(fw.wg_nmin + blockIdx.x, n);
+        store_device(fw.wg_maxlen + blockIdx.x, mx);
+    }
+    if (!rc.n_wg) return;
+    if (!last_workgroup_out(rc.done, &s_flag)) return;
+    {
+        uint32_t h = 0, nm = 0, ml = 0;
+        for (uint32_t g = (uint32_t)tid; g < gridDim.x; g += VS_THREADS) {
+            h += load_device(fw.wg_hits + g);
+            nm += load_device(fw.wg_nmin + g);
+            const uint32_t m = load_device(fw.wg_maxlen + g);
+            ml = m > ml ? m : ml;
+        }
+        const uint32_t wn = wave_inclusive_scan(nm), wm = wave_max(ml);
+        unsigned long long wh = h;
+#pragma unroll
+        for (int off = 32; off > 0; off >>= 1) wh += __shfl_xor(wh, off);
+        __shared__ unsigned long long s_h[VS_THREADS / 64];
+        if ((tid & 63) == 63) {
+            s_h[tid >> 6] = wh;
+            s_red[1][tid >> 6] = wn;
+            s_red[2][tid >> 6] = wm;
+        }
+        __syncthreads();
+        if (tid == 0) {
+            unsigned long long th = 0, tn = 0;
+            uint32_t tm = 0;
+            for (int i = 0; i < VS_THREADS / 64; ++i) {
+                th += s_h[i];
+                tn += s_red[1][i];
+                tm = s_red[2][i] > tm ? s_red[2][i] : tm;
+            }
+            *rc.tot_hits = th;
+            if (tn && !(load_device(rc.overflow_word) & 4u)) atomicAdd(rc.tot_minimizers, tn);
+            *rc.tot_max_len = (unsigned long long)tm;
+        }
     }
 }
 
@@ -375,9 +385,11 @@
     }
 }
 
+uint32_t candidate_stage_grid(int n_cus) { return std::min<uint32_t>((uint32_t)n_cus * (uint32_t)(2048 / VS_THREADS), MAX_EX_WG); }
+
 hipError_t launch_candidate_stage(const SketchArgs& a, FilterWork& fw, const ReadClusterArgs& rc, int n_cus, hipStream_t stream, bool with_totals)
 {
-    fw.verify_grid = std::min<uint32_t>((uint32_t)n_cus * (uint32_t)(2048 / VS_THREADS), MAX_EX_WG);
+    if (fw.verify_grid != candidate_stage_grid(n_cus)) return hipErrorInvalidValue;
     const dim3 grid(fw.verify_grid);
     if (a.packed) {
         if (a.k == 15) hipLaunchKernelGGL((verify_scan_kernel<15, true>), grid, dim3(VS_THREADS), 0, stream, a, fw, rc);
diff --git a/drprg_amd/csrc/capi.cpp b/drprg_amd/csrc/capi.cpp
--- a/drprg_amd/csrc/capi.cpp
+++ b/drprg_amd/csrc/capi.cpp
@@ -1345,6 +1345,7 @@
         m->buffer_info(v);
         for (int i = 0; i < 3; ++i) out[i] += v[i];
         for (int i = 3; i < 5; ++i) out[i] = std::max(out[i], v[i]);
+        out[5] += m->wide_shares();
     }
     API_END(ctx)
 }
diff --git a/drprg_amd/csrc/device_common.h b/drprg_amd/csrc/device_common.h
--- a/drprg_amd/csrc/device_common.h
+++ b/drprg_amd/csrc/device_common.h
@@ -233,5 +233,22 @@
     return base + incl - v;
 }
 
-}
-}
+__device__ __forceinline__ uint32_t load_device(const uint32_t* p) { return __hip_atomic_load(p, __ATOMIC_RELAXED, __HIP_MEMORY_SCOPE_AGENT); }
+__device__ __forceinline__ unsigned long long load_device(const unsigned long long* p) { return __hip_atomic_load(p, __ATOMIC_RELAXED, __HIP_MEMORY_SCOPE_AGENT); }
+__device__ __forceinline__ void store_device(uint32_t* p, uint32_t v) { __hip_atomic_store(p, v, __ATOMIC_RELAXED, __HIP_MEMORY_SCOPE_AGENT); }
+__device__ __forceinline__ bool last_workgroup_out(uint32_t* done, uint32_t* s_flag)
+{
+    asm volatile("s_waitcnt vmcnt(0)" ::: "memory");
+    __syncthreads();
+    if (threadIdx.x == 0) {
+        const uint32_t drawn = __hip_atomic_fetch_add(done, 1u, __ATOMIC_RELAXED, __HIP_MEMORY_SCOPE_AGENT);
+        const bool last = drawn == gridDim.x - 1u;
+        if (last) store_device(done, 0u);
+        *s_flag = last ? 1u : 0u;
+    }
+    __syncthreads();
+    return *s_flag != 0u;
+}
+
+}
+}
diff --git a/drprg_amd/csrc/filter_common.h b/drprg_amd/csrc/filter_common.h
--- a/drprg_amd/csrc/filter_common.h
+++ b/drprg_amd/csrc/filter_common.h
@@ -29,6 +29,7 @@
     t_end = b + per_wg < total ? (uint32_t)(b + per_wg) : total;
 }
 
+uint32_t candidate_stage_grid(int n_cus);
 hipError_t launch_candidate_stage(const SketchArgs& a, FilterWork& fw, const ReadClusterArgs& rc, int n_cus, hipStream_t stream, bool with_totals = true);
 hipError_t launch_read_cluster(const SketchArgs& a, const FilterWork& fw, const ReadClusterArgs& rc, int n_cus, bool skip, hipStream_t stream);
 
diff --git a/drprg_amd/csrc/kernels.h b/drprg_amd/csrc/kernels.h
--- a/drprg_amd/csrc/kernels.h
+++ b/drprg_amd/csrc/kernels.h
@@ -136,6 +136,11 @@
     unsigned long long* max_len;
     const uint32_t* wave_share = nullptr;
     unsigned long long* class_clock = nullptr;
+    unsigned long long* counters = nullptr;
+    unsigned long long* counters_mirror = nullptr;
+    uint32_t n_counters = 0;
+    uint32_t* done = nullptr;
+    uint32_t* wide_shares = nullptr;
 };
 constexpr int FT_MAX_ROUNDS = 8;
 struct FilterSched {
@@ -165,6 +170,11 @@
     uint32_t* slice_base;
     uint32_t* slice_cap;
     uint32_t* super_count;
+    uint32_t* super_prefix;
+    uint4* share_bounds;
+    uint32_t* done;
+    uint32_t* wide_shares;
+    uint32_t counters_home;
     FilterSched sched;
     uint32_t* cand_count;
     const uint32_t* cand_total;
@@ -195,15 +205,22 @@
     const uint32_t* slice_prefix;
     uint32_t n_slices, mark_epoch;
     const uint32_t* block_first;
-    const uint32_t *wg_hits, *wg_nmin, *wg_maxlen;
     uint32_t n_wg;
     unsigned long long *tot_hits, *tot_minimizers, *tot_max_len;
     const uint32_t* overflow_word;
+    unsigned long long* home_from;
+    unsigned long long* home_to;
+    uint32_t home_n;
+    uint32_t* done;
+    uint4 *zero_a, *zero_b;
+    uint32_t n_zero_a4, n_zero_b4;
     uint32_t minpath_in_lds;
 };
 hipError_t launch_counters_home(unsigned long long* from, unsigned long long* to, uint32_t n, hipStream_t stream, uint32_t* zero = nullptr, uint32_t n_zero = 0);
 uint32_t* filter_super_counts(uint32_t* small);
 uint32_t filter_super_words();
+uint32_t* filter_share_words(uint32_t* small);
+uint32_t filter_share_word_count();
 size_t filter_small_words();
 void init_candidate_work(FilterWork& fw, const FilterBuffers& b, int n_cus);
 hipError_t launch_sketch_filter(const SketchArgs& a, const BloomTables& bt, int n_cus, const FilterBuffers& b, const ReadClusterArgs& rc, FilterWork& fw,
diff --git a/drprg_amd/csrc/mapper.cpp b/drprg_amd/csrc/mapper.cpp
--- a/drprg_amd/csrc/mapper.cpp
+++ b/drprg_amd/csrc/mapper.cpp
@@ -328,15 +328,29 @@
     Lane& lane = lanes_[b.lane];
     grow_lane(lane, std::max<uint64_t>(min_capacity_, b.batch.n_bases / FILTER_BASES_PER_ENTRY));
     if (!lane.scratch_zero) HIPCHK(hipMemsetAsync(lane.d_scratch.data(), 0, lane.d_scratch.bytes(), b.stream));
+    if (lane.small_dirty) {
+        HIPCHK(hipMemsetAsync(dev::filter_super_counts(lane.small.data()), 0, dev::filter_super_words() * sizeof(uint32_t), b.stream));
+        HIPCHK(hipMemsetAsync(dev::filter_share_words(lane.small.data()), 0, dev::filter_share_word_count() * sizeof(uint32_t), b.stream));
+    }
     lane.scratch_zero = false;
+    lane.small_dirty = true;
     dev::SketchArgs a = sketch_args(b.batch, nullptr);
     count_on_lane(a, lane);
     dev::FilterBuffers fb = filter_buffers(lane);
     fb.class_clock = lane.d_scratch.data() + L_FT_CLOCK;
     if (ft_share_[b.batch.packed ? 1 : 0][0]) fb.wave_share = ft_share_[b.batch.packed ? 1 : 0];
+    fb.counters = lane.d_scratch.data();
+    fb.counters_mirror = lane.h_scratch.device_ptr();
+    fb.n_counters = L_N;
+    fb.done = reinterpret_cast<uint32_t*>(lane.d_scratch.data() + L_DONE);
+    fb.wide_shares = reinterpret_cast<uint32_t*>(lane.d_scratch.data() + L_WIDE);
     HIPCHK(dev::launch_sketch_filter(a, tables_.bloom_tables(use_mid_), n_cus_, fb, read_cluster_args(b), lane.fw, sw_, b.stream, kernel_timer(lane.t0, lane.t1)));
-    HIPCHK(dev::launch_counters_home(lane.d_scratch.data(), lane.h_scratch.device_ptr(), L_N, b.stream, dev::filter_super_counts(lane.small.data()), dev::filter_super_words()));
+    if (!lane.fw.counters_home) {
+        HIPCHK(dev::launch_counters_home(lane.d_scratch.data(), lane.h_scratch.device_ptr(), L_N, b.stream, dev::filter_super_counts(lane.small.data()), dev::filter_super_words()));
+        HIPCHK(hipMemsetAsync(dev::filter_share_words(lane.small.data()), 0, dev::filter_share_word_count() * sizeof(uint32_t), b.stream));
+    }
     lane.scratch_zero = true;
+    lane.small_dirty = false;
 }
 
 static void wait_stream(hipStream_t stream, hipEvent_t event = nullptr)
@@ -583,6 +597,7 @@
     tot_minimizers_ += lane.h_scratch[L_MINIMIZERS];
     tot_hits_ += lane.h_scratch[L_HITS];
     tot_leftover_ += lane.h_scratch[L_COMPLEX];
+    wide_shares_ += lane.h_scratch[L_WIDE];
     tune_filter_shares(lane, b.batch.packed, b.batch.n_bases);
     leftovers(b);
     return true;
diff --git a/drprg_amd/csrc/mapper.h b/drprg_amd/csrc/mapper.h
--- a/drprg_amd/csrc/mapper.h
+++ b/drprg_amd/csrc/mapper.h
@@ -92,6 +92,7 @@
     }
     void filter_schedule(uint64_t out[20]);
     void buffer_info(uint64_t out[6]);
+    uint64_t wide_shares() const { return wide_shares_; }
     void enable_kernel_timing(bool on) { timing_ = on; }
     double sketch_ms_total() const { return sketch_ms_; }
     uint64_t sketch_launches() const { return sketch_launches_; }
@@ -109,10 +110,12 @@
         DeviceBuffer<unsigned long long> d_scratch;
         PinnedBuffer<unsigned long long> h_scratch;
         bool scratch_zero = false;
+        bool small_dirty = false;
         dev::FilterWork fw {};
         uint64_t capacity() const { return raw_pos.size(); }
     };
-    enum { L_HITS = 0, L_OVERFLOW = 1, L_MAXLEN = 2, L_UNSORTED = 3, L_COMPLEX = 4, L_CHUNK = 5, L_MINIMIZERS = 6, L_FT_CLOCK = 7 , L_N = 12 };
+    enum { L_HITS = 0, L_OVERFLOW = 1, L_MAXLEN = 2, L_UNSORTED = 3, L_COMPLEX = 4, L_CHUNK = 5, L_MINIMIZERS = 6, L_FT_CLOCK = 7 ,
+        L_DONE = 12 , L_WIDE = 13 , L_N = 14 };
     struct Batch {
         DeviceBatch batch;
         bool active = false;
@@ -199,6 +202,7 @@
     static constexpr uint64_t MIN_CAPACITY_CLAMP = 4096;
     uint64_t min_capacity_ = 1u << 20;
     uint64_t reruns_filter_ = 0, reruns_direct_ = 0, regrows_hits_ = 0;
+    uint64_t wide_shares_ = 0;
     struct TileSet {
         uint32_t slice_cap = 256, ws_tiles = 0, ws_cap = 0;
         DeviceBuffer<uint64_t> d_tile_info;
diff --git a/drprg_amd/csrc/read_cluster.hip b/drprg_amd/csrc/read_cluster.hip
--- a/drprg_amd/csrc/read_cluster.hip
+++ b/drprg_amd/csrc/read_cluster.hip
@@ -50,36 +50,21 @@
     int tid = threadIdx.x;
 #define lane (tid & 63)
 #define wave (tid >> 6)
-    if (rc.n_wg && blockIdx.x == 0) {
-        uint32_t h = 0, nm = 0, ml = 0;
-        for (uint32_t g = (uint32_t)tid; g < rc.n_wg; g += RC_THREADS) {
-            h += rc.wg_hits[g];
-            nm += rc.wg_nmin[g];
-            const uint32_t m = rc.wg_maxlen[g];
-            ml = m > ml ? m : ml;
-        }
-        const uint32_t wh = wave_inclusive_scan(h), wn = wave_inclusive_scan(nm), wm = wave_max(ml);
-        if (lane == 63) {
-            s_w[0][wave] = wh;
-            s_w[1][wave] = wn;
-            s_irr[wave] = wm;
-        }
-        __syncthreads();
-        if (tid == 0) {
-            unsigned long long th = 0, tn = 0;
-            uint32_t tm = 0;
-            for (int i = 0; i < RC_WAVES; ++i) {
-                th += s_w[0][i];
-                tn += s_w[1][i];
-                tm = s_irr[i] > tm ? s_irr[i] : tm;
-            }
-            *rc.tot_hits = th;
-            if (tn && !(*reinterpret_cast<volatile const uint32_t*>(rc.overflow_word) & 4u)) atomicAdd(rc.tot_minimizers, tn);
-            *rc.tot_max_len = (unsigned long long)tm;
-        }
-        __syncthreads();
-    }
-    if (*reinterpret_cast<volatile uint32_t*>(a.overflow) & 4u) return;
+    auto go_home = [&]() {
+        if (!rc.home_n) return;
+        if (!last_workgroup_out(rc.done, &s_n_irr)) return;
+        if ((uint32_t)tid < rc.home_n) {
+            rc.home_to[tid] = load_device(rc.home_from + tid);
+            rc.home_from[tid] = 0;
+            __threadfence_system();
+        }
+        for (uint32_t j = (uint32_t)tid; j < rc.n_zero_a4; j += RC_THREADS) rc.zero_a[j] = make_uint4(0, 0, 0, 0);
+        for (uint32_t j = (uint32_t)tid; j < rc.n_zero_b4; j += RC_THREADS) rc.zero_b[j] = make_uint4(0, 0, 0, 0);
+    };
+    if (*reinterpret_cast<volatile uint32_t*>(a.overflow) & 4u) {
+        go_home();
+        return;
+    }
     const uint32_t total = SLICES ? rc.slice_prefix[rc.n_slices] : *fw.cand_total;
     const uint32_t handled_mark = SLICES ? rc.mark_epoch : 0u;
     uint16_t* const s_minpath = reinterpret_cast<uint16_t*>(s_hist + rc.n_prgs);
@@ -539,6 +524,7 @@
         if (s_tot[1]) atomicAdd(rc.n_hits_kept, s_tot[1]);
         if (s_tot[2]) atomicAdd(rc.n_complex, s_tot[2]);
     }
+    go_home();
 }
 #undef lane
 #undef wave
diff --git a/drprg_amd/csrc/share_bounds.h b/drprg_amd/csrc/share_bounds.h
--- /dev/null
+++ b/drprg_amd/csrc/share_bounds.h
@@ -0,0 +1,54 @@
+#pragma once
+#include <cstdint>
+
+#if defined(__HIPCC__)
+#define DRPRG_SB_HD __host__ __device__
+#else
+#define DRPRG_SB_HD
+#endif
+
+namespace drprg {
+namespace dev {
+
+constexpr uint32_t VS_WINDOW = 256;
+
+struct ShareBounds {
+    uint32_t t_begin, t_end;
+    uint32_t s_lo, s_hi;
+};
+
+DRPRG_SB_HD inline void share_range(uint32_t total, uint32_t grid, uint32_t b, uint32_t& t_begin, uint32_t& t_end)
+{
+    const uint32_t per_wg = (uint32_t)(((uint64_t)total + grid - 1) / grid);
+    const uint64_t b64 = (uint64_t)b * per_wg;
+    t_begin = b64 < total ? (uint32_t)b64 : total;
+    t_end = b64 + per_wg < total ? (uint32_t)(b64 + per_wg) : total;
+}
+
+DRPRG_SB_HD inline uint32_t superblock_of(const uint32_t* prefix, uint32_t n_super, uint32_t x)
+{
+    uint32_t lo = 0, hi = n_super;
+    while (hi - lo > 1) {
+        const uint32_t mid = lo + ((hi - lo) >> 1);
+        if (prefix[mid] <= x) lo = mid;
+        else hi = mid;
+    }
+    return lo;
+}
+
+DRPRG_SB_HD inline ShareBounds share_bounds(const uint32_t* prefix, uint32_t n_super, uint32_t grid, uint32_t b)
+{
+    ShareBounds r;
+    share_range(prefix[n_super], grid, b, r.t_begin, r.t_end);
+    r.s_lo = r.s_hi = 0;
+    if (r.t_begin < r.t_end) {
+        r.s_lo = superblock_of(prefix, n_super, r.t_begin);
+        r.s_hi = superblock_of(prefix, n_super, r.t_end - 1u);
+    }
+    return r;
+}
+
+DRPRG_SB_HD inline bool share_fits_window(const ShareBounds& r) { return r.s_hi - r.s_lo + 2u <= VS_WINDOW; }
+
+}
+}
diff --git a/drprg_amd/csrc/sketch_filter.hip b/drprg_amd/csrc/sketch_filter.hip
--- a/drprg_amd/csrc/sketch_filter.hip
+++ b/drprg_amd/csrc/sketch_filter.hip
@@ -1,4 +1,5 @@
 #include "filter_common.h"
+#include "share_bounds.h"
 #include <algorithm>
 #include <cstdint>
 #include <type_traits>
@@ -86,6 +87,7 @@
     const bool dynamic = per_wg > FT_WAVES;
     if (dynamic && (t_lo != 0 || t_hi != fw.sched.n_tiles)) {
         if (tid == 0) atomicOr(a.overflow, 32u);
+        if (tid == 0 && blockIdx.x == 0) *fw.cand_count = 0;
         return;
     }
     const uint32_t tiles_per_wave = fw.sched.tpw0 ? fw.sched.tpw0 : (t_hi - t_lo + n_waves - 1) / n_waves;
@@ -476,6 +478,42 @@
     }
     close_slice();
     if (fw.class_clock && (tid & 255) == 0) atomicMax(&fw.class_clock[1 + (tid >> 8)], (unsigned long long)wall_clock64());
+
+    if (!last_workgroup_out(fw.done, s_dyn + 24)) return;
+    {
+        constexpr int PER = MAX_SLICES / FT_THREADS;
+        static_assert(PER == 8, "two 16-byte stores of prefixes per thread");
+        uint32_t* const s_pre = s_dyn + 32;
+        uint32_t cnt[PER], run = 0;
+#pragma unroll
+        for (int i = 0; i < PER; ++i) cnt[i] = load_device(fw.super_count + (size_t)tid * PER + i);
+#pragma unroll
+        for (int i = 0; i < PER; ++i) run += cnt[i];
+        uint32_t total;
+        uint32_t acc = block_exclusive_scan<FT_WAVES>(run, s_dyn, &total);
+        uint32_t pre[PER];
+#pragma unroll
+        for (int i = 0; i < PER; ++i) {
+            pre[i] = acc;
+            acc += cnt[i];
+        }
+#pragma unroll
+        for (int i = 0; i < PER / 4; ++i) {
+            const uint4 v = make_uint4(pre[4 * i], pre[4 * i + 1], pre[4 * i + 2], pre[4 * i + 3]);
+            reinterpret_cast<uint4*>(fw.super_prefix + (size_t)tid * PER)[i] = v;
+            reinterpret_cast<uint4*>(s_pre + (size_t)tid * PER)[i] = v;
+        }
+        if (tid == FT_THREADS - 1) {
+            fw.super_prefix[MAX_SLICES] = acc;
+            s_pre[MAX_SLICES] = acc;
+        }
+        if (tid == 0) *fw.cand_count = total;
+        __syncthreads();
+        for (uint32_t b = (uint32_t)tid; b < fw.verify_grid; b += FT_THREADS) {
+            const ShareBounds sb = share_bounds(s_pre, (uint32_t)MAX_SLICES, fw.verify_grid, b);
+            fw.share_bounds[b] = make_uint4(sb.t_begin, sb.t_end, sb.s_lo, sb.s_hi);
+        }
+    }
 }
 #undef DRPRG_SECOND_STAGE
 #undef DRPRG_BLOCK_TEST
@@ -498,9 +536,14 @@
 }
 
 constexpr size_t FT_SMALL_HEAD = (size_t)MAX_CHUNKS * 3 + MAX_SLICES;
-size_t filter_small_words() { return FT_SMALL_HEAD + 4 + 4 * (size_t)MAX_EX_WG; }
+constexpr size_t FT_SHARE_AT = FT_SMALL_HEAD + 4 + 4 * (size_t)MAX_EX_WG, FT_SHARE_WORDS = (size_t)MAX_SLICES + 4 + 4 * (size_t)MAX_EX_WG;
+static_assert(FT_SHARE_AT % 4 == 0 && FT_SHARE_WORDS % 4 == 0 && MAX_CHUNKS % 4 == 0, "cleared and read 16 bytes at a time");
+constexpr size_t FT_EPILOGUE_WORDS = 32 + (size_t)MAX_SLICES + 4;
+size_t filter_small_words() { return FT_SHARE_AT + FT_SHARE_WORDS; }
 uint32_t* filter_super_counts(uint32_t* small) { return small + MAX_CHUNKS; }
 uint32_t filter_super_words() { return (uint32_t)MAX_SLICES; }
+uint32_t* filter_share_words(uint32_t* small) { return small + FT_SHARE_AT; }
+uint32_t filter_share_word_count() { return (uint32_t)FT_SHARE_WORDS; }
 
 FilterSched make_filter_sched(uint32_t n_tiles, uint32_t n_wg, const uint32_t share[4], const FilterSchedKnobs& knobs)
 {
@@ -628,6 +671,12 @@
     fw.slice_cap = fw.slice_base + MAX_CHUNKS;
     fw.cand_count = b.small + FT_SMALL_HEAD;
     fw.cand_total = fw.cand_count;
+    fw.super_prefix = filter_share_words(b.small);
+    fw.share_bounds = reinterpret_cast<uint4*>(fw.super_prefix + MAX_SLICES + 4);
+    fw.done = b.done;
+    fw.wide_shares = b.wide_shares;
+    if (!b.done) return hipErrorInvalidValue;
+    fw.verify_grid = candidate_stage_grid(n_cus);
     {
         using Kernel = void (*)(SketchArgs, FilterWork);
         const int which = mid ? (bt.mid0_bits == 3 ? 3 : 4) : blk ? 5 : level0 ? 2 : (a.k < 12 ? 1 : 0);
@@ -644,7 +693,7 @@
             : which == 1                 ? &sketch_filter_kernel<true, false, false, 0, true>
                                          : &sketch_filter_kernel<false, false, false, 0, true>;
         const Kernel kernel = a.packed ? packed : ascii;
-        const size_t dyn = level0 ? (size_t)FT_L0_WORDS * 4 + (size_t)FT_WAVES * 2048 : ((size_t)4 << bt.bloom_wbits) + 16;
+        const size_t dyn = level0 ? (size_t)FT_L0_WORDS * 4 + (size_t)FT_WAVES * 2048 : std::max<size_t>(((size_t)4 << bt.bloom_wbits) + 16, FT_EPILOGUE_WORDS * 4);
         fw.sched.lds_word = (uint32_t)(dyn / 4 - 4);
         static size_t configured[12][MAX_HIP_DEVICES] = {};
         HIP_TRY(ensure_dynamic_lds(reinterpret_cast<const void*>(kernel), dyn, configured[which + (a.packed ? 6 : 0)]));
@@ -652,18 +701,27 @@
     }
     HIP_TRY(hipGetLastError());
     const bool skip_rc = sw.skip_read_cluster;
-    HIP_TRY(launch_candidate_stage(a, fw, rc, n_cus, stream, skip_rc));
-    ReadClusterArgs rct = rc;
+    ReadClusterArgs rcv = rc, rct = rc;
     if (!skip_rc) {
-        rct.wg_hits = fw.wg_hits;
-        rct.wg_nmin = fw.wg_nmin;
-        rct.wg_maxlen = fw.wg_maxlen;
-        rct.n_wg = fw.verify_grid;
-        rct.tot_hits = a.n_hits;
-        rct.tot_minimizers = a.n_minimizers;
-        rct.tot_max_len = fw.max_len;
-        rct.overflow_word = a.overflow;
-    }
+        rcv.n_wg = fw.verify_grid;
+        rcv.tot_hits = a.n_hits;
+        rcv.tot_minimizers = a.n_minimizers;
+        rcv.tot_max_len = fw.max_len;
+        rcv.overflow_word = a.overflow;
+        rcv.done = b.done;
+        if (b.counters && b.counters_mirror && b.n_counters) {
+            rct.home_from = b.counters;
+            rct.home_to = b.counters_mirror;
+            rct.home_n = b.n_counters;
+            rct.done = b.done;
+            rct.zero_a = reinterpret_cast<uint4*>(fw.super_count);
+            rct.n_zero_a4 = filter_super_words() / 4;
+            rct.zero_b = reinterpret_cast<uint4*>(fw.super_prefix);
+            rct.n_zero_b4 = filter_share_word_count() / 4;
+            fw.counters_home = 1;
+        }
+    }
+    HIP_TRY(launch_candidate_stage(a, fw, rcv, n_cus, stream, skip_rc));
     return launch_read_cluster(a, fw, rct, n_cus, skip_rc, stream);
 }
 
diff --git a/drprg_amd/pandora.py b/drprg_amd/pandora.py
--- a/drprg_amd/pandora.py
+++ b/drprg_amd/pandora.py
@@ -296,7 +296,7 @@
         out = (C.c_uint64 * 6)()
         _check(lib.drprg_hip_buffer_info(self._h, out), self._h)
         return dict(filter_reruns=int(out[0]), direct_reruns=int(out[1]), hit_regrows=int(out[2]), lane_capacity=int(out[3]),
-                    hit_capacity=int(out[4]))
+                    hit_capacity=int(out[4]), wide_shares=int(out[5]))
 
     def kernel_timing(self, enable=True, reset=False):
         ms, n = C.c_double(), C.c_uint64()
```

Result: no change. 20.83 billion (-0.4%).
